# ming71/rotate-yolov3

Hardware: AMD Instinct MI355X
Metric: images/sec fwd+bwd at 608^2 (train step, backend=hip) (higher is better)
Workload: dtype bf16; 1 GPU; configs[3]: Darknet-53 train step (fwd + riou loss + bwd + grad all-reduce + SGD), bs=64/GPU 608x608, synthetic HRSC-shaped targets; global_batch=64, parallelism=dp1, gradients=250 MB fp32 in 4 flat buckets, fp32 on the wire

## Files before the change

include/ryolo.h:

```cpp
#ifndef RYOLO_H
#define RYOLO_H

#include <stddef.h>
#include <stdint.h>

#ifdef __cplusplus
extern "C" {
#endif

#define RYOLO_OK 0
#define RYOLO_EINVAL -1
#define RYOLO_ELAUNCH -2
#define RYOLO_ETOOBIG -3

#define RYOLO_RNMS_MAX_BOXES 262144

const char *ryolo_strerror(int code);
int ryolo_abi_version(void);
const char *ryolo_build_id(void);
int ryolo_set_tuning(const char *name, const char *value);

size_t ryolo_rnms_workspace_bytes(int n);
int ryolo_rnms(const float *dets, int n, int row_stride, float thr, int64_t *keep_out, int32_t *num_keep,
               void *workspace, size_t workspace_bytes, void *stream);

size_t ryolo_rnms_segmented_workspace_bytes(int m, int num_segments, int max_seg_len);
int ryolo_rnms_segmented(const float *dets, int m, int row_stride, const int32_t *seg_offsets, int num_segments,
                         int max_seg_len, float thr, unsigned char *keep_flags, void *workspace, size_t workspace_bytes,
                         void *stream);

void ryolo_rnms_count_pairs(uint64_t *device_counter);

int ryolo_riou_pairs(const float *b1, int stride1, const float *b2, int stride2, int n, float *out, void *stream);
int ryolo_riou_matrix(const float *b1, int n1, int stride1, const float *b2, int n2, int stride2, float *out,
                      void *stream);

int ryolo_skew_iou_pairs(const float *b1, int stride1, const float *b2, int stride2, int n, float *out, void *stream);
int ryolo_skew_iou_matrix(const float *b1, int n1, int stride1, const float *b2, int n2, int stride2, float *out,
                          void *stream);

size_t ryolo_eval_match_workspace_bytes(int n_det, int n_lab);
int ryolo_eval_match(const float *det, int det_stride, const int32_t *det_off, const float *lab, int lab_stride, const int32_t *lab_off,
                     int n_img, int n_det, int n_lab, float iou_thres, uint8_t *correct, int32_t *matched , void *ws,
                     size_t ws_bytes, void *stream);


#define RYOLO_ACT_LINEAR 0
#define RYOLO_ACT_LEAKY 1
#define RYOLO_ACT_MISH 2

typedef struct ryolo_conv_desc {
    int N, H, W;
    int Cin, Cout;
    int ksize, stride, pad;
    int in_cstride, out_cstride, res_cstride;
    int act;
    float slope;
    int upsample;
    int tile;
} ryolo_conv_desc;

size_t ryolo_conv_packed_weight_bytes(int Cout, int Cin_pad, int ksize);
int ryolo_conv_pack_weights(const float *w_oihw, int Cout, int Cin, int ksize, int Cin_pad, void *packed,
                            void *stream);
int ryolo_conv2d_bn_act(const ryolo_conv_desc *desc , const void *x, const void *w_packed,
                        const float *scale, const float *shift, const void *residual , void *y,
                        void *stream);
int ryolo_conv_pair_supported(const ryolo_conv_desc *first, const ryolo_conv_desc *second, int shortcut_from_input);
int ryolo_conv2d_bn_act_pair(const ryolo_conv_desc *first, const ryolo_conv_desc *second, const void *x, const void *w_first,
                             const float *scale_first, const float *shift_first, const void *w_second, const float *scale_second,
                             const float *shift_second, int shortcut_from_input, void *y, void *stream);
#define RYOLO_CONV_KERNEL_MP256 1
#define RYOLO_CONV_KERNEL_MP192 2
#define RYOLO_CONV_KERNEL_MQ 3
#define RYOLO_CONV_KERNEL_DIRECT8 4
#define RYOLO_CONV_KERNEL_STEM 5
#define RYOLO_CONV_KERNEL_PW 6
#define RYOLO_CONV_KERNEL_STEM0 8
#define RYOLO_CONV_KERNEL_STEM_DGRAD 7
#define RYOLO_CONV_KERNEL_STEM64 11
#define RYOLO_CONV_KERNEL_MQ128 9
#define RYOLO_CONV_KERNEL_MQ64 10
#define RYOLO_CONV_KERNEL_IGEMM 16
int ryolo_conv_kernel_choice(const ryolo_conv_desc *desc, int with_residual, int with_statistics);
#define RYOLO_WGRAD_KERNEL_TAPS 1000
int ryolo_conv_dgrad_kernel_choice(const ryolo_conv_desc *forward_desc, int with_bn_reduce );
int ryolo_conv_wgrad_kernel_choice(const ryolo_conv_desc *forward_desc);
int ryolo_nchw_f32_to_nhwc_bf16(const float *x, int N, int C, int H, int W, int Cpad, void *y, void *stream);
int ryolo_nhwc_bf16_to_nchw_f32(const void *x, int N, int C, int H, int W, int cstride, float *y, void *stream);


int ryolo_yolo_decode_filter(const void *head, int head_cstride, int bs, int ny, int nx, int na, int no,
                             const float *anchors, float stride, float context_factor, int arc, float conf_thres,
                             float min_wh, long long io_rows_per_image, long long io_row_offset, float *cand,
                             long long *cand_row, int *counter, int capacity, void *stream);

int ryolo_yolo_decode(const void *head, int head_cstride, int bs, int ny, int nx, int na, int no,
                      const float *anchors, float stride, float context_factor, int arc, float *io,
                      long long io_rows_per_image, long long io_row_offset, float *p, void *stream);

int ryolo_conv_head_decode_supported(const ryolo_conv_desc *desc, int na, int no);
int ryolo_conv_head_decode(const ryolo_conv_desc *desc, const void *x, const void *w_packed, const float *scale, const float *shift,
                           const float *anchors, int na, int no, float stride, float context_factor, int arc, float *io,
                           long long io_rows_per_image, long long io_row_offset, float *p, void *stream);

int ryolo_add_nhwc(const void *a, int a_cstride, const void *b, int b_cstride, void *y, int y_cstride,
                   long long npix, int C, void *stream);
int ryolo_upsample_nhwc(const void *x, int x_cstride, void *y, int y_cstride, int N, int H, int W, int C, int scale,
                        void *stream);
int ryolo_maxpool_nhwc(const void *x, int x_cstride, void *y, int y_cstride, int N, int H, int W, int C, int ksize,
                       int stride, void *stream);

size_t ryolo_se_workspace_bytes(int N, int H, int W, int C);
int ryolo_se_nhwc(const void *x, int x_cstride, const float *w1 , const float *w2 ,
                  int hidden, void *y, int y_cstride, int N, int H, int W, int C,
                  float *gate_out , void *workspace, size_t workspace_bytes, void *stream);


int ryolo_conv0_recompute_supported(const ryolo_conv_desc *desc);
int ryolo_conv0_bn_act_fwd(const ryolo_conv_desc *desc, const void *x, const void *w_packed, const float *scale, const float *shift,
                           int act, const float *slope, void *y, void *stream);
size_t ryolo_conv0_bn_bwd_workspace_bytes(void);
int ryolo_conv0_bn_bwd(const ryolo_conv_desc *desc, const void *x, const void *w_packed, const void *dy, int dy_cstride,
                       const float *scale, const float *shift, const float *mean, const float *invstd, int act, const float *slope,
                       void *dz, int dz_cstride, float *dgamma, float *dbeta, float *dslope, void *workspace, size_t workspace_bytes,
                       int workspace_is_zero, void *stream);
size_t ryolo_conv0_bn_bwd_wgrad_workspace_bytes(void);
int ryolo_conv0_bn_bwd_wgrad(const ryolo_conv_desc *desc, const void *x, const void *w_packed, const void *dy, int dy_cstride,
                             const float *scale, const float *shift, const float *mean, const float *invstd, int act, const float *slope,
                             float *dgamma, float *dbeta, float *dslope, float *grad_oihw, int cin_real, int accumulate, void *workspace,
                             size_t workspace_bytes, void *stream);
int ryolo_conv_stat_rows(const ryolo_conv_desc *desc);
int ryolo_conv2d_bn_act_stats(const ryolo_conv_desc *desc, const void *x, const void *w_packed, const float *scale,
                              const float *shift, const void *residual, void *y,
                              double *stat_part ,
                              void *stream);
int ryolo_bn_finalize(double *stat_part, int rows, int cpad, int C, long long count, float eps, float momentum,
                      const float *gamma, const float *beta, float *mean, float *invstd, float *scale, float *shift,
                      float *running_mean , float *running_var, void *stream);
int ryolo_bn_act_fwd(const void *z, int z_cstride, const float *scale, const float *shift, int act,
                     const float *slope , const void *residual, int res_cstride, void *y,
                     int y_cstride, long long npix, int C, void *stream);
size_t ryolo_bn_act_bwd_workspace_bytes(long long npix, int C);
int ryolo_bn_act_bwd(const void *z, int z_cstride, const void *dy, int dy_cstride, const float *scale, const float *shift,
                     const float *mean, const float *invstd, int act, const float *slope, void *dz, int dz_cstride,
                     long long npix, int C, float *dgamma, float *dbeta, float *dslope, void *workspace,
                     size_t workspace_bytes, void *stream);
size_t ryolo_conv_packed_dgrad_bytes(int Cout, int Cin, int ksize, int stride);
int ryolo_conv_dgrad_tap_table(int ksize, int stride, int *host_out );
int ryolo_conv_pack_weights_dgrad(const float *w_oihw, int Cout, int Cin, int ksize, int stride, void *packed,
                                  const int *taps_table ,
                                  void *stream);
int ryolo_conv2d_dgrad(const ryolo_conv_desc *forward_desc, const void *dz, int dz_cstride, const void *packed_dgrad,
                       const float *ones, const float *zeros , void *dx, int accumulate, void *stream);
int ryolo_conv2d_dgrad_bnreduce_rows(const ryolo_conv_desc *forward_desc);
int ryolo_conv2d_dgrad_bnreduce(const ryolo_conv_desc *forward_desc, const void *dz, int dz_cstride, const void *packed_dgrad,
                                const float *ones, const float *zeros, void *dx, int accumulate,
                                const void *z , int z_cstride,
                                const float *scale, const float *shift, const float *mean, const float *invstd ,
                                const float *slope , float *part , void *stream);
int ryolo_bn_act_bwd_reduced(const void *z, int z_cstride, const void *dy, int dy_cstride, const float *scale, const float *shift,
                             const float *mean, const float *invstd, int act , const float *slope, void *dz,
                             int dz_cstride, long long npix, int C, float *dgamma, float *dbeta, float *dslope, const float *part,
                             int rows, void *workspace , size_t workspace_bytes, void *stream);
size_t ryolo_conv_wgrad_workspace_bytes(const ryolo_conv_desc *forward_desc);
int ryolo_conv2d_wgrad_partials(const ryolo_conv_desc *forward_desc, const void *x, const void *dz, int dz_cstride, int Cin_real,
                                float *grad_oihw, int accumulate, void *workspace, size_t workspace_bytes, void *stream);
int ryolo_conv2d_wgrad_reduce(const ryolo_conv_desc *forward_desc, const void *x, const void *dz, int dz_cstride, int Cin_real,
                              float *grad_oihw, int accumulate, void *workspace, size_t workspace_bytes, void *stream);

typedef struct ryolo_wgrad_reduce_job {
    const float *part;
    float *g;
    int S, Cout, Cin_real, Cin_k, ks, Kpad, Cout_pad, accumulate;
    int kind;
    int block_begin, block_end;
    int wide;
} ryolo_wgrad_reduce_job;
int ryolo_conv_wgrad_reduce_job_fill(ryolo_wgrad_reduce_job *host_job, const ryolo_conv_desc *forward_desc, int Cin_real, const void *workspace,
                                     float *grad_oihw, int accumulate);
int ryolo_conv_wgrad_reduce_batch(const ryolo_wgrad_reduce_job *device_jobs, int njobs, int total_blocks, void *stream);
int ryolo_conv2d_wgrad(const ryolo_conv_desc *forward_desc, const void *x, const void *dz, int dz_cstride, int Cin_real,
                       float *grad_oihw , int accumulate, void *workspace,
                       size_t workspace_bytes, void *stream);
int ryolo_upsample2x_bwd(const void *dy, int dy_cstride, void *dx, int dx_cstride, int N, int H, int W, int C,
                         int accumulate, void *stream);
int ryolo_pgrad_to_nhwc(const float *pgrad, int bs, int na, int ny, int nx, int no, void *out, int out_cstride,
                        void *stream);

typedef struct ryolo_pack_job {
    const void *src;
    void *dst;
    int kind, Cout, Cin, KS, Cin_pad, ntaps, Kpad, rows;
    int khs[9], kws[9];
    int block_begin, block_end;
} ryolo_pack_job;
int ryolo_conv_pack_job_fill(ryolo_pack_job *host_jobs, const float *w_oihw, int Cout, int Cin, int ksize, int stride,
                             int Cin_pad, void *packed_fwd, void *packed_dgrad);
int ryolo_conv_pack_batch(const ryolo_pack_job *device_jobs, int njobs, int total_blocks, void *stream);

#define RYOLO_MAX_HEADS 4
int ryolo_build_targets(const float *tpad, const unsigned char *valid, int NT, int nheads, int na, const float *const *ng,
                        const float *const *anchor_vec, float iou_t, float ang_t, float context_factor, float *const *w,
                        long long *const *idx, float *const *box, float *const *npos, void *stream);
size_t ryolo_yolo_loss_bitmap_bytes(long long cells);
int ryolo_yolo_loss(const float *p, int bs, int na, int ny, int nx, int no, int nc, const float *w, int NT,
                    const long long *b, const long long *gj, const long long *gi, const long long *cls, const float *txy,
                    const float *twh, const float *ta, const float *anchor_vec , const float *npos, float giou,
                    float reg_w, float cls_w, float cls_pw, float obj_w, float obj_pw,
                    int iou_mode ,
                    unsigned *bitmap, float *dp, float *items , void *stream);

int ryolo_yolo_loss_nhwc(const void *head, int head_cstride, const float *p, int bs, int na, int ny, int nx, int no, int nc,
                         const float *w, int NT, const long long *b, const long long *gj, const long long *gi,
                         const long long *cls, const float *txy, const float *twh, const float *ta, const float *anchor_vec,
                         const float *npos, float giou, float reg_w, float cls_w, float cls_pw, float obj_w, float obj_pw,
                         int iou_mode, unsigned *bitmap, float *dp_sparse, void *head_grad, int head_grad_cstride, float *items,
                         void *stream);
#define RYOLO_ARC_FOCAL 1
#define RYOLO_ARC_UBCE 2
#define RYOLO_ARC_UCE 4
size_t ryolo_yolo_loss_bitmap_bytes_arc(long long cells, int nc, int arc);
int ryolo_yolo_loss_arc(const float *p, int bs, int na, int ny, int nx, int no, int nc, const float *w, int NT,
                        const long long *b, const long long *gj, const long long *gi, const long long *cls, const float *txy,
                        const float *twh, const float *ta, const float *anchor_vec, const float *npos, float giou, float reg_w,
                        float cls_w, float cls_pw, float obj_w, float obj_pw, int iou_mode, int arc, float fl_gamma, unsigned *bitmap,
                        float *dp, float *items, void *stream);
int ryolo_yolo_loss_nhwc_arc(const void *head, int head_cstride, const float *p, int bs, int na, int ny, int nx, int no, int nc,
                             const float *w, int NT, const long long *b, const long long *gj, const long long *gi,
                             const long long *cls, const float *txy, const float *twh, const float *ta, const float *anchor_vec,
                             const float *npos, float giou, float reg_w, float cls_w, float cls_pw, float obj_w, float obj_pw,
                             int iou_mode, int arc, float fl_gamma, unsigned *bitmap, float *dp_sparse, void *head_grad,
                             int head_grad_cstride, float *items, void *stream);
int ryolo_scale_bf16_if(const float *g, void *buf, int cstride, long long npix, int C, void *stream);

int ryolo_riou_loss_pairs(const float *pbox, const float *tbox, int n, float *iou, float *grad, void *stream);

// ... 15 lines not shown
```

rotate-yolov3_amd/_lib.py:

```python
import ctypes as C
import os

_HERE = os.path.dirname(os.path.abspath(__file__))
LIB_PATH = os.environ.get("RYOLO_HIP_LIB") or os.path.join(_HERE, "libryolo_hip.so")

_lib = None

ACT_LINEAR, ACT_LEAKY, ACT_MISH = 0, 1, 2


class ConvDesc(C.Structure):
    _fields_ = [("N", C.c_int), ("H", C.c_int), ("W", C.c_int), ("Cin", C.c_int), ("Cout", C.c_int),
                ("ksize", C.c_int), ("stride", C.c_int), ("pad", C.c_int),
                ("in_cstride", C.c_int), ("out_cstride", C.c_int), ("res_cstride", C.c_int),
                ("act", C.c_int), ("slope", C.c_float), ("upsample", C.c_int), ("tile", C.c_int)]


_vp = C.c_void_p
_dp = C.POINTER(ConvDesc)
_sigs = {
    "ryolo_strerror": (C.c_char_p, [C.c_int]),
    "ryolo_abi_version": (C.c_int, []),
    "ryolo_build_id": (C.c_char_p, []),
    "ryolo_set_tuning": (C.c_int, [C.c_char_p, C.c_char_p]),
    "ryolo_rnms_workspace_bytes": (C.c_size_t, [C.c_int]),
    "ryolo_rnms": (C.c_int, [_vp, C.c_int, C.c_int, C.c_float, _vp, _vp, _vp, C.c_size_t, _vp]),
    "ryolo_rnms_segmented_workspace_bytes": (C.c_size_t, [C.c_int, C.c_int, C.c_int]),
    "ryolo_rnms_segmented": (C.c_int, [_vp, C.c_int, C.c_int, _vp, C.c_int, C.c_int, C.c_float, _vp, _vp, C.c_size_t, _vp]),
    "ryolo_riou_pairs": (C.c_int, [_vp, C.c_int, _vp, C.c_int, C.c_int, _vp, _vp]),
    "ryolo_riou_matrix": (C.c_int, [_vp, C.c_int, C.c_int, _vp, C.c_int, C.c_int, _vp, _vp]),
    "ryolo_rnms_count_pairs": (None, [_vp]),
    "ryolo_skew_iou_pairs": (C.c_int, [_vp, C.c_int, _vp, C.c_int, C.c_int, _vp, _vp]),
    "ryolo_skew_iou_matrix": (C.c_int, [_vp, C.c_int, C.c_int, _vp, C.c_int, C.c_int, _vp, _vp]),
    "ryolo_eval_match_workspace_bytes": (C.c_size_t, [C.c_int, C.c_int]),
    "ryolo_eval_match": (C.c_int, [_vp, C.c_int, _vp, _vp, C.c_int, _vp, C.c_int, C.c_int, C.c_int, C.c_float, _vp, _vp, _vp, C.c_size_t, _vp]),
    "ryolo_conv_pair_supported": (C.c_int, [_dp, _dp, C.c_int]),
    "ryolo_conv_head_decode_supported": (C.c_int, [_dp, C.c_int, C.c_int]),
    "ryolo_conv0_recompute_supported": (C.c_int, [_dp]),
    "ryolo_conv2d_dgrad_bnreduce_rows": (C.c_int, [_dp]),
    "ryolo_se_workspace_bytes": (C.c_size_t, [C.c_int, C.c_int, C.c_int, C.c_int]),
    "ryolo_se_nhwc": (C.c_int, [_vp, C.c_int, _vp, _vp, C.c_int, _vp, C.c_int, C.c_int, C.c_int, C.c_int, C.c_int, _vp, _vp, C.c_size_t, _vp]),
}


def declare(name, restype, argtypes):
    _sigs[name] = (restype, argtypes)
    if _lib is not None:
        fn = getattr(getattr(_lib, "_real", _lib), name)
        fn.restype, fn.argtypes = restype, argtypes


def lib():
    global _lib
    if _lib is None:
        if not os.path.exists(LIB_PATH):
            raise RuntimeError(
                "rotate-yolov3_amd: %s is missing -- run `python -c 'import __graft_entry__ as g; g.build()'` "
                "(hipcc --offload-arch=gfx950).  There is no CPU fallback for the HIP hot path." % LIB_PATH)
        import torch
        _lib = C.CDLL(LIB_PATH)
        for name, (restype, argtypes) in _sigs.items():
            fn = getattr(_lib, name)
            fn.restype, fn.argtypes = restype, argtypes
    return _lib


TUNING_SWITCHES = ("RYOLO_CONV3X3", "RYOLO_CONV1X1", "RYOLO_RNMS_TILES", "RYOLO_MQ_KORDER", "RYOLO_BN_REDUCE_TILES", "RYOLO_STEM_DGRAD")


def set_tuning(name, value):
    rc = getattr(lib(), "_real", lib()).ryolo_set_tuning(name.encode(), None if value is None else str(value).encode())
    if rc != 0:
        raise RuntimeError("ryolo_set_tuning(%s): unknown switch" % name)


class _CallTracer(object):

    def __init__(self, real, log):
        self._real, self._log = real, log

    def __getattr__(self, name):
        fn = getattr(self._real, name)
        if not name.startswith("ryolo_") or not callable(fn):
            return fn
        log = self._log

        def traced(*args):
            import torch
            e0, e1 = torch.cuda.Event(enable_timing=True), torch.cuda.Event(enable_timing=True)
            e0.record()
            rc = fn(*args)
            e1.record()
            log.append((name, args, e0, e1))
            return rc
        return traced


class trace_calls(object):

    def __enter__(self):
        global _lib
        lib()
        self._saved = _lib
        self.log = []
        _lib = _CallTracer(self._saved, self.log)
        return self.log

    def __exit__(self, *exc):
        global _lib
        _lib = self._saved
        return False


def check(rc, what):
    if rc != 0:
        msg = lib().ryolo_strerror(rc)
        raise RuntimeError("%s failed: %s (code %d)" % (what, msg.decode() if msg else "?", rc))


def stream_ptr(device=None):
# ... 3 lines not shown
```

rotate-yolov3_amd/csrc/conv.hip:

```cpp
#include <cstring>

#include <mutex>

#include "conv_common.h"

using namespace ryolo_detail;

namespace {

template <int KS, int BM, int BN, int WGM, int WGN, int NSTAGE, bool FAST, bool GEN, bool BNRED = false>
__global__ void __launch_bounds__(WGM *WGN * 64) conv_igemm_kernel(const ConvParams p, const BnRed br = BnRed()) {
    constexpr int NW = WGM * WGN, NT = NW * 64;
    constexpr int WPIX = BM / WGM, WCH = BN / WGN, PF = WPIX / 16, CF = WCH / 16;
    constexpr int A_BYTES = BM * BK * 2, B_BYTES = BN * BK * 2, STAGE = A_BYTES + B_BYTES;
    constexpr int A_PPW = (BM / 8) / NW, B_PPW = (BN / 8) / NW;
    static_assert(A_PPW >= 1 && B_PPW >= 1, "tile too small for the wave count");
    constexpr int SROW = BN * 2 + 16;
    static_assert(BM * SROW + WGM * 2 * BN * 4 <= NSTAGE * STAGE, "staging tile + statistics slots must fit in the operand buffers");
    constexpr int LOADS_PER_STAGE = A_PPW + B_PPW;

    extern __shared__ __attribute__((aligned(16))) char smem[];

    const int tid = threadIdx.x;
    const int lane = tid & 63;
// ... 1475 lines not shown
        unsigned nblk;
        if (!conv0_params(d, d->out_cstride, p, gpw, &nblk)) return RYOLO_EINVAL;
        p.cin_log2 = 3;
        p.stat_cpad = 128;
        const bool staged = conv0_halo_on() && !(d->tile >> 16) && y && !stat_part;
        RYOLO_CONV_DRY_RUN(lc, (staged ? RYOLO_CONV_KERNEL_STEM0 : RYOLO_CONV_KERNEL_DIRECT8));
        if (staged) return launch_conv0_halo(p, nullptr, 0, lc);
        return stat_part ? launch_c8_direct<true>(p, gpw, nblk, lc.stream) : launch_c8_direct<false>(p, gpw, nblk, lc.stream);
    }
    if (!conv_shape(d, p)) return RYOLO_EINVAL;
    p.cin_log2 = ilog2_exact(d->Cin);
    if (d->ksize == 3 && p.cin_log2 < 0 && (d->Cin % BK)) return RYOLO_EINVAL;
    p.taps2 = (d->Cin == 32 && d->ksize == 3) ? 1 : 0;
    p.fast = (d->Cin % BK == 0 || p.taps2) && !(d->tile & 0x100) && buffer_extent((unsigned long long)d->N * d->H * d->W, d->in_cstride, d->Cin, &p.x_bytes) &&
             buffer_extent((d->Cout + 127) / 128 * 128, p.Kpad, p.Kpad + 128, &p.w_bytes);
    if (!p.fast) p.taps2 = p.x_bytes = p.w_bytes = 0;
    p.no_persist = (d->tile & 0x200) ? 1 : 0;
    p.force_persist = (d->tile & 0x800) ? 1 : 0;
    p.pw_grid_cap = (d->tile & 0xff) == 13 ? (d->tile >> 16) & 0xff : 0;
#ifdef RYOLO_MP_ABLATION
    if ((d->tile & 0x400) && p.fast) p.x_bytes = p.w_bytes = 0;
#endif
    p.nt_out = (long long)p.M * d->upsample * d->upsample * d->Cout * 2 >= nt_out_min_bytes() ? 1 : 0;
    p.stat_cpad = (d->Cout + 127) / 128 * 128;
    return dispatch(p, d->ksize, pick_tile(d), lc);
}

static bool head_params(const ryolo_conv_desc *d, ConvParams &p) {
    if (conv_validate(d) != RYOLO_OK || d->ksize != 1 || d->stride != 1 || d->pad != 0 || d->upsample != 1 || (d->Cin % BK)) return false;
    if (!conv_shape(d, p)) return false;
    p.out_cs = d->Cout; p.res_cs = 0; p.Kpad = d->Cin;
    if (!buffer_extent(p.M, d->in_cstride, d->Cin, &p.x_bytes) || !buffer_extent((d->Cout + 127) / 128 * 128, p.Kpad, p.Kpad + 128, &p.w_bytes)) return false;
    p.fast = 1; p.use_magic = 1;
    return true;
}

extern "C" {

int ryolo_conv_stat_rows(const ryolo_conv_desc *d) {
    if (conv_validate(d) != RYOLO_OK) return 0;
    return STAT_ROWS;
}

int ryolo_conv2d_bn_act_stats(const ryolo_conv_desc *d, const void *x, const void *w_packed, const float *scale,
                              const float *shift, const void *residual, void *y, double *stat_part, void *stream_) {
    if (!x || !w_packed || !scale || !shift) return RYOLO_EINVAL;
    if (!y && !(stat_part && ryolo_conv0_recompute_supported(d))) return RYOLO_EINVAL;
    if (((uintptr_t)x | (uintptr_t)y | (uintptr_t)w_packed | (uintptr_t)residual | (uintptr_t)scale | (uintptr_t)shift) & 15)
        return RYOLO_EINVAL;
    ConvLaunch lc;
    lc.stream = (hipStream_t)stream_;
    return conv_forward(d, x, w_packed, scale, shift, residual, y, stat_part, lc);
}

int ryolo_conv2d_bn_act(const ryolo_conv_desc *d, const void *x, const void *w_packed, const float *scale,
                        const float *shift, const void *residual, void *y, void *stream_) {
    return ryolo_conv2d_bn_act_stats(d, x, w_packed, scale, shift, residual, y, nullptr, stream_);
}

int ryolo_conv_kernel_choice(const ryolo_conv_desc *d, int with_residual, int with_statistics) {
    int choice = -1;
    ConvLaunch lc;
    lc.choice = &choice;
    void *fake = (void *)(uintptr_t)4096;
    const int rc = conv_forward(d, fake, fake, (const float *)fake, (const float *)fake, with_residual ? fake : nullptr, fake,
                                with_statistics ? (double *)fake : nullptr, lc);
    return rc == RYOLO_OK ? choice : -1;
}

int ryolo_conv_head_decode_supported(const ryolo_conv_desc *d, int na, int no) {
    ConvParams p{};
    return head_params(d, p) && conv_pw_decode_supported(p, na, no) ? 1 : 0;
}

int ryolo_conv_head_decode(const ryolo_conv_desc *d, const void *x, const void *w_packed, const float *scale, const float *shift,
                           const float *anchors, int na, int no, float stride, float context_factor, int arc, float *io,
                           long long io_rows_per_image, long long io_row_offset, float *pout, void *stream_) {
    ConvParams p{};
    if (!x || !w_packed || !scale || !shift || !anchors || !io || !head_params(d, p) || !conv_pw_decode_supported(p, na, no)) return RYOLO_EINVAL;
    if (arc < 0 || arc > 2 || !(stride > 0.f) || !(context_factor > 0.f)) return RYOLO_EINVAL;
    if (((uintptr_t)x | (uintptr_t)w_packed) & 15) return RYOLO_EINVAL;
    p.x = (const __bf16 *)x; p.w = (const __bf16 *)w_packed; p.scale = scale; p.shift = shift;
    return launch_conv_pw_decode(p, io, io_rows_per_image, io_row_offset, pout, anchors, na, no, stride, context_factor, arc, (hipStream_t)stream_);
}

int ryolo_conv_pair_supported(const ryolo_conv_desc *first, const ryolo_conv_desc *second, int shortcut_from_input) {
    if (conv_validate(first) != RYOLO_OK || conv_validate(second) != RYOLO_OK) return 0;
    return conv_stem_pair_kind(first, second, shortcut_from_input) != 0 ? 1 : 0;
}

int ryolo_conv2d_bn_act_pair(const ryolo_conv_desc *a, const ryolo_conv_desc *b, const void *x, const void *w_first, const float *scale_first,
                             const float *shift_first, const void *w_second, const float *scale_second, const float *shift_second,
                             int shortcut_from_input, void *y, void *stream_) {
    if (conv_validate(a) != RYOLO_OK || conv_validate(b) != RYOLO_OK || !x || !w_first || !scale_first || !shift_first || !w_second || !scale_second ||
        !shift_second || !y)
        return RYOLO_EINVAL;
    const int kind = conv_stem_pair_kind(a, b, shortcut_from_input);
    if (!kind) return RYOLO_EINVAL;
    if (((uintptr_t)x | (uintptr_t)y | (uintptr_t)w_first | (uintptr_t)w_second) & 15) return RYOLO_EINVAL;
    ConvParams p{};
    if (!conv_shape(b, p)) return RYOLO_EINVAL;
    p.w = (const __bf16 *)w_second; p.scale = scale_second; p.shift = shift_second; p.y = (__bf16 *)y;
    p.in_cs = b->Cin; p.res_cs = 0;
    p.nt_out = (long long)p.M * b->Cout * 2 >= nt_out_min_bytes() ? 1 : 0;
    const unsigned long long xb = (((unsigned long long)a->N * a->H * a->W - 1) * a->in_cstride + a->Cin) * 2ull;
    const int kpad_first = (a->ksize * a->ksize * a->Cin + BK - 1) / BK * BK;
    return launch_conv_stem_pair(kind, p, x, (unsigned)xb, a->in_cstride, a->H, a->W, w_first, kpad_first, scale_first, shift_first, a->act,
                                 a->slope, (hipStream_t)stream_);
}

int ryolo_conv0_recompute_supported(const ryolo_conv_desc *d) {
    return conv_validate(d) == RYOLO_OK && conv0_shape(d, d->out_cstride) ? 1 : 0;
}

int ryolo_conv0_bn_act_fwd(const ryolo_conv_desc *d, const void *x, const void *w_packed, const float *scale, const float *shift,
                           int act, const float *slope, void *y, void *stream_) {
    if (!ryolo_conv0_recompute_supported(d) || !x || !w_packed || !scale || !shift || !y) return RYOLO_EINVAL;
    if (act < 0 || act > 2 || (act == RYOLO_ACT_LEAKY && !slope)) return RYOLO_EINVAL;
    if (((uintptr_t)x | (uintptr_t)y | (uintptr_t)w_packed) & 15) return RYOLO_EINVAL;
    ConvParams p{};
    const int gpw = 32;
    unsigned nblk;
    if (!conv0_params(d, d->out_cstride, p, gpw, &nblk)) return RYOLO_EINVAL;
    p.x = (const __bf16 *)x; p.w = (const __bf16 *)w_packed; p.scale = scale; p.shift = shift; p.y = (__bf16 *)y;
    p.act = act; p.slope = 0.f;
    C8Bwd bw;
    bw.slope = act == RYOLO_ACT_LEAKY ? slope : nullptr;
    bw.round_z = 1;
    ConvLaunch lc;
    lc.stream = (hipStream_t)stream_;
    if (conv0_halo_on()) return launch_conv0_halo(p, bw.slope, 1, lc);
    return launch_c8_mode(act, p, gpw, nblk, bw, 0, lc.stream);
}

size_t ryolo_conv0_bn_bwd_workspace_bytes(void) { return (size_t)STAT_ROWS * 96 * 8 + 64 * 4; }

int ryolo_conv0_bn_bwd(const ryolo_conv_desc *d, const void *x, const void *w_packed, const void *dy, int dy_cstride,
                       const float *scale, const float *shift, const float *mean, const float *invstd, int act, const float *slope,
                       void *dz, int dz_cstride, float *dgamma, float *dbeta, float *dslope, void *workspace, size_t workspace_bytes,
                       int workspace_is_zero, void *stream_) {
    if (!ryolo_conv0_recompute_supported(d) || !x || !w_packed || !dy || !scale || !shift || !mean || !invstd || !dz || !workspace)
        return RYOLO_EINVAL;
    if (workspace_bytes < ryolo_conv0_bn_bwd_workspace_bytes() || (dy_cstride & 7) || (dz_cstride & 7) || dy_cstride < 32 || dz_cstride < 32)
        return RYOLO_EINVAL;
    if (act < 0 || act > 2 || (act == RYOLO_ACT_LEAKY && !slope)) return RYOLO_EINVAL;
    if (((uintptr_t)x | (uintptr_t)dy | (uintptr_t)dz | (uintptr_t)w_packed | (uintptr_t)workspace) & 15) return RYOLO_EINVAL;
    hipStream_t stream = (hipStream_t)stream_;
    ConvParams p{};
    const int gpw = 32;
    unsigned nblk;
    C8Bwd bw;
    if (!conv0_params(d, dz_cstride, p, gpw, &nblk) || !buffer_extent(p.M, dy_cstride, 32, &bw.dy_bytes)) return RYOLO_EINVAL;
    p.x = (const __bf16 *)x; p.w = (const __bf16 *)w_packed; p.scale = scale; p.shift = shift; p.y = (__bf16 *)dz;
    p.act = act; p.slope = 0.f;
    bw.slope = act == RYOLO_ACT_LEAKY ? slope : nullptr;
    bw.dy = (const __bf16 *)dy; bw.dy_cs = dy_cstride; bw.mean = mean;
    double *part = (double *)workspace;
    float *kb = (float *)(part + (size_t)STAT_ROWS * 96), *kd = kb + 32;
    bw.part = part; bw.kb = kb; bw.kd = kd;
    if (!workspace_is_zero && hipMemsetAsync(part, 0, (size_t)STAT_ROWS * 96 * 8, stream) != hipSuccess) return RYOLO_ELAUNCH;
    int rc = launch_c8_mode(act, p, gpw, nblk, bw, 2, stream);
    if (rc != RYOLO_OK) return rc;
    rc = launch_kernel<conv0_bwd_finalize_kernel>(dim3(1), dim3(32), 0, stream, part, scale, mean, invstd, 1.0f / (float)p.M, kb, kd, dgamma, dbeta,
                                                  act == RYOLO_ACT_LEAKY ? dslope : nullptr);
    if (rc != RYOLO_OK) return rc;
    return launch_c8_mode(act, p, gpw, nblk, bw, 3, stream);
// ... 4 lines not shown
```

rotate-yolov3_amd/csrc/conv_common.h:

```cpp
#pragma once
#include <hip/hip_runtime.h>
#include <stdint.h>
#include <stdlib.h>

#include "../../include/ryolo.h"

namespace ryolo_detail {

typedef __attribute__((ext_vector_type(8))) __bf16 bf16x8;
typedef __attribute__((ext_vector_type(4))) __bf16 bf16x4;
typedef __attribute__((ext_vector_type(2))) __bf16 bf16x2;
typedef __attribute__((ext_vector_type(4))) float f32x4;
typedef __attribute__((ext_vector_type(4))) unsigned int u32x4;
typedef __attribute__((address_space(3))) void *lds_vp;
typedef const __attribute__((address_space(1))) void *glb_vp;

constexpr int BK = 64;
constexpr long long NT_OUT_MIN_BYTES = 128ll << 20;
constexpr int STAT_ROWS = 128;

struct ConvParams {
    const __bf16 *x;
    const __bf16 *w;
    const float *scale;
// ... 135 lines not shown
        }                             \
    } while (0)

inline int cu_count() {
    static const int cus = [] {
        int dev = 0, n = 0;
        return hipGetDevice(&dev) == hipSuccess && hipDeviceGetAttribute(&n, hipDeviceAttributeMultiprocessorCount, dev) == hipSuccess && n > 0 ? n : 256;
    }();
    return cus;
}

template <auto KFN, typename... Args>
int launch_kernel(dim3 grid, dim3 block, size_t smem, hipStream_t stream, Args... args) {
    if (smem > 64 * 1024) {
        static const hipError_t raised = hipFuncSetAttribute((const void *)KFN, hipFuncAttributeMaxDynamicSharedMemorySize, (int)smem);
        if (raised != hipSuccess) return RYOLO_ELAUNCH;
    }
    hipLaunchKernelGGL(KFN, grid, block, smem, stream, args...);
    return hipGetLastError() == hipSuccess ? RYOLO_OK : RYOLO_ELAUNCH;
}

inline bool buffer_extent(unsigned long long npix, long long cs, long long c, unsigned *bytes = nullptr) {
    const unsigned long long b = ((npix - 1) * (unsigned long long)cs + (unsigned long long)c) * 2ull;
    if (b >= 0x7fffff00ull) return false;
    if (bytes) *bytes = (unsigned)b;
    return true;
}

struct PersistGrid {
    int grid, nt;
    long long tiles;
    bool deep, exact;
};
inline PersistGrid persist_grid(long long M, int BM, int Cout, int BN, int Ho, int Wo, bool force = false, int rounds2 = 5) {
    const long long mt = (M + BM - 1) / BM, nt = (Cout + BN - 1) / BN, dmax = Wo > Ho ? Wo : Ho;
    PersistGrid g;
    g.grid = (2 * cu_count()) & ~7;
    g.nt = (int)nt;
    g.tiles = mt * nt;
    g.deep = force ? g.tiles > g.grid : 2 * g.tiles >= (long long)rounds2 * g.grid;
    g.exact = g.grid >= 8 && mt * BM * dmax < 0x100000000ll && g.tiles * nt < 0x100000000ll;
    return g;
}

inline int grid_for(long long total, int tb = 256, int cap = 32768) {
    long long nb = (total + tb - 1) / tb;
    return (int)(nb < 1 ? 1 : (nb > cap ? cap : nb));
}

inline int ilog2_exact(int v) {
    int l = 0;
    while ((1 << l) < v) l++;
    return (1 << l) == v ? l : -1;
}

int conv_validate(const ryolo_conv_desc *d);
int dispatch(ConvParams &p, int ksize, int pick, const ConvLaunch &lc);
long long nt_out_min_bytes();
bool conv_pw_disabled();
int mq128_knob();

int launch_conv_mp(ConvParams &p, int bm , int variant, const ConvLaunch &lc);
int conv_mp_pick_bm(const ConvParams &p);
bool conv_mp_eligible(const ConvParams &p);
int launch_conv_mq(ConvParams &p, int variant, const ConvLaunch &lc);
bool conv_mq128_eligible(const ConvParams &p);
int conv_mq128_grid(const ConvParams &p, int bm);
int launch_conv_mq128(ConvParams &p, int bm, const ConvLaunch &lc);
bool conv_stem_eligible(const ConvParams &p, int ksize);
int launch_conv_stem(ConvParams &p, const ConvLaunch &lc);
bool conv_stem64_eligible(const ConvParams &p, int ksize);
int launch_conv_stem64(ConvParams &p, const ConvLaunch &lc);
int launch_conv0_halo(ConvParams &p, const float *slope_dev, int round_z, const ConvLaunch &lc);
int launch_conv_stem_dgrad(int cdz, int stride, const void *dz, int dz_cs, const void *w_classes, void *dx, int dx_cs, int accumulate, int N,
                           int H, int W, int nt_out, const ConvLaunch &lc);
int conv_stem_pair_kind(const ryolo_conv_desc *first, const ryolo_conv_desc *second, int shortcut_from_input);
int launch_conv_stem_pair(int kind, ConvParams &p , const void *x, unsigned x_bytes, int in_cs, int H, int W,
                          const void *w_first, int kpad_first, const float *scale_first, const float *shift_first, int act_first,
                          float slope_first, hipStream_t stream);
bool conv_pw_eligible(const ConvParams &p, int ksize);
bool conv_pw_preferred(const ConvParams &p);
int conv_pw_grid(const ConvParams &p);
int launch_conv_pw(ConvParams &p, const ConvLaunch &lc);
bool conv_pw_decode_supported(const ConvParams &p, int na, int no);
int launch_conv_pw_decode(ConvParams &p, float *io, long long io_img_rows, long long io_row0, float *pout, const float *anchors, int na, int no,
                          float stride, float cf, int arc, hipStream_t stream);
#ifdef RYOLO_MP_ABLATION
int ryolo_mp_ablation_variant(int slot);
#endif

enum TuneKey { TUNE_CONV3X3 = 0, TUNE_CONV1X1, TUNE_RNMS_TILES, TUNE_MQ_KORDER, TUNE_BN_REDUCE_TILES, TUNE_STEM_DGRAD, TUNE_COUNT };
const char *tune(TuneKey k);
#ifdef RYOLO_MP_ABLATION
inline const char *abl_env(const char *name) { return getenv(name); }
#else
inline const char *abl_env(const char *) { return nullptr; }
#endif

}
```

rotate-yolov3_amd/csrc/conv_dgrad.hip:

```cpp
#include <cstring>

#include "conv_common.h"

using namespace ryolo_detail;

extern "C" {

static int dgrad_classes(int ks, int stride, int pad, int cls, int *dy, int *dx, int *khs, int *kws) {
    if (stride == 1) {
        int n = 0;
        for (int kh = 0; kh < ks; kh++)
            for (int kw = 0; kw < ks; kw++) {
                dy[n] = kh; dx[n] = kw; khs[n] = ks - 1 - kh; kws[n] = ks - 1 - kw;
                n++;
            }
        return n;
    }
    const int a = cls >> 1, b = cls & 1;
    int n = 0;
    for (int kh = ks - 1; kh >= 0; kh--) {
        if (((a + pad - kh) & 1) != 0) continue;
        for (int kw = ks - 1; kw >= 0; kw--) {
            if (((b + pad - kw) & 1) != 0) continue;
            dy[n] = (a + pad - kh) / 2; dx[n] = (b + pad - kw) / 2; khs[n] = kh; kws[n] = kw;
// ... 246 lines not shown
        for (int cls = 0; cls < (stride == 1 ? 1 : 4); cls++) {
            int dy[9], dx[9], khs[9], kws[9];
            const int nt = dgrad_classes(ksize, stride, (ksize - 1) / 2, cls, dy, dx, khs, kws);
            ryolo_pack_job &j = host_jobs[n++];
            j = ryolo_pack_job{};
            j.src = w_oihw; j.dst = dst; j.kind = 1; j.Cout = Cout; j.Cin = Cin; j.KS = ksize; j.ntaps = nt;
            for (int t = 0; t < nt; t++) { j.khs[t] = khs[t]; j.kws[t] = kws[t]; }
            j.Kpad = (nt * Cout + BK - 1) / BK * BK;
            j.rows = (Cin + 127) / 128 * 128;
            j.block_begin = 0; j.block_end = (j.rows / PK_CI) * ((Cout + PK_CO - 1) / PK_CO);
            dst += ((size_t)j.rows * j.Kpad + 128) * 2;
        }
        if (dgrad_xfusable(Cin, ksize, stride)) {
            for (int a = 0; a < 2; a++) {
                int dy[9], dx[9], khs[9], k0[9], k1[9];
                const int nt = dgrad_xfused_class(a, dy, dx, khs, k0, k1);
                ryolo_pack_job &j = host_jobs[n++];
                j = ryolo_pack_job{};
                j.src = w_oihw; j.dst = dst; j.kind = 2; j.Cout = Cout; j.Cin = Cin; j.KS = ksize; j.ntaps = nt;
                for (int t = 0; t < nt; t++) { j.khs[t] = khs[t]; j.kws[t] = (k0[t] + 1) | ((k1[t] + 1) << 4); }
                j.Kpad = (nt * Cout + BK - 1) / BK * BK;
                j.rows = (2 * Cin + 127) / 128 * 128;
                j.block_begin = 0; j.block_end = (j.rows / PK_CI) * ((Cout + PK_CO - 1) / PK_CO);
                dst += ((size_t)j.rows * j.Kpad + 128) * 2;
            }
        }
    }
    return n;
}

int ryolo_conv_pack_batch(const ryolo_pack_job *device_jobs, int njobs, int total_blocks, void *stream) {
    if (!device_jobs || njobs <= 0 || total_blocks <= 0) return RYOLO_EINVAL;
    hipLaunchKernelGGL(pack_batch_kernel, dim3((unsigned)total_blocks), dim3(256), 0, (hipStream_t)stream, device_jobs, njobs);
    return hipGetLastError() == hipSuccess ? RYOLO_OK : RYOLO_ELAUNCH;
}

int ryolo_conv_dgrad_tap_table(int ksize, int stride, int *host_out ) {
    if (!host_out || (ksize != 1 && ksize != 3) || (stride != 1 && stride != 2)) return RYOLO_EINVAL;
    for (int i = 0; i < 72; i++) host_out[i] = 0;
    for (int cls = 0; cls < (stride == 1 ? 1 : 4); cls++) {
        int dy[9], dx[9];
        dgrad_classes(ksize, stride, (ksize - 1) / 2, cls, dy, dx, host_out + cls * 18, host_out + cls * 18 + 9);
    }
    return RYOLO_OK;
}

int ryolo_conv_pack_weights_dgrad(const float *w_oihw, int Cout, int Cin, int ksize, int stride, void *packed,
                                  const int *taps_table , void *stream_) {
    if (!w_oihw || !packed || !taps_table || ryolo_conv_packed_dgrad_bytes(Cout, Cin, ksize, stride) == 0) return RYOLO_EINVAL;
    hipStream_t stream = (hipStream_t)stream_;
    const int rows = (Cin + 127) / 128 * 128;
    char *dst = (char *)packed;
    for (int cls = 0; cls < (stride == 1 ? 1 : 4); cls++) {
        int dy[9], dx[9], kk[18];
        const int nt = dgrad_classes(ksize, stride, (ksize - 1) / 2, cls, dy, dx, kk, kk + 9);
        const int Kpad = (nt * Cout + BK - 1) / BK * BK;
        const size_t total = (size_t)rows * Kpad + 128;
        const int nb = (int)((total + 255) / 256 < 4096 ? (total + 255) / 256 : 4096);
        hipLaunchKernelGGL(pack_dgrad_kernel, dim3(nb), dim3(256), 0, stream, w_oihw, Cout, Cin, ksize, nt,
                           taps_table + cls * 18, Kpad, rows, (__bf16 *)dst);
        dst += total * 2;
    }
    if (dgrad_xfusable(Cin, ksize, stride)) {
        const int rows2 = (2 * Cin + 127) / 128 * 128;
        for (int a = 0; a < 2; a++) {
            int dy[9], dx[9];
            XfTaps tp;
            const int nt = dgrad_xfused_class(a, dy, dx, tp.khs, tp.kw0, tp.kw1);
            for (int t = nt; t < 9; t++) { tp.khs[t] = 0; tp.kw0[t] = -1; tp.kw1[t] = -1; }
            const int Kpad = (nt * Cout + BK - 1) / BK * BK;
            const size_t total = (size_t)rows2 * Kpad + 128;
            const int nb = (int)((total + 255) / 256 < 4096 ? (total + 255) / 256 : 4096);
            hipLaunchKernelGGL(pack_dgrad_xfused_kernel, dim3(nb), dim3(256), 0, stream, w_oihw, Cout, Cin, nt, tp, Kpad, rows2,
                               (__bf16 *)dst);
            dst += total * 2;
        }
    }
    return hipGetLastError() == hipSuccess ? RYOLO_OK : RYOLO_ELAUNCH;
}

}

static int conv_dgrad(const ryolo_conv_desc *d , const void *dz, int dz_cstride, const void *packed_dgrad, const float *ones,
                      const float *zeros, void *dx, int accumulate, const ConvLaunch &lc) {
    if (conv_validate(d) != RYOLO_OK) return RYOLO_EINVAL;
    if (d->stride != 1 && !(d->stride == 2 && d->ksize == 3 && d->pad == 1)) return RYOLO_EINVAL;
    if ((dz_cstride & 7) || dz_cstride < d->Cout) return RYOLO_EINVAL;
    const int Ho = (d->H + 2 * d->pad - d->ksize) / d->stride + 1, Wo = (d->W + 2 * d->pad - d->ksize) / d->stride + 1;
    const int rows = (d->Cin + 127) / 128 * 128;
    const unsigned long long dz_pix = (unsigned long long)d->N * Ho * Wo;
    const int nt_out = (long long)d->N * d->H * d->W * d->Cin * 2 >= nt_out_min_bytes() ? 1 : 0;
    const char *wsrc = (const char *)packed_dgrad;
    const bool xfuse = dgrad_xfusable(d->Cin, d->ksize, d->stride) && d->pad == 1 && (d->W & 1) == 0 &&
                       d->in_cstride == d->Cin && !(d->tile & 0x8000);
    if (xfuse) wsrc += dgrad_classic_bytes(d->Cout, d->Cin, d->ksize, d->stride);
    if (!lc.bnred && d->ksize == 3 && d->pad == 1 && ((d->Cin == 32 && d->Cout == 64) || (d->Cin == 64 && d->Cout == 128 && d->stride == 2)) &&
        !(d->tile & 0x80ff)) {
        const char *e = tune(TUNE_STEM_DGRAD);
        const int knob = e ? atoi(e) : 3;
        if (knob & (d->Cout == 64 ? 1 : 2)) {
            if (buffer_extent(dz_pix, dz_cstride, d->Cout) && buffer_extent((unsigned long long)d->N * d->H * d->W, d->in_cstride, d->Cin)) {
                RYOLO_CONV_DRY_RUN(lc, RYOLO_CONV_KERNEL_STEM_DGRAD);
                const int rc = launch_conv_stem_dgrad(d->Cout, d->stride, dz, dz_cstride, packed_dgrad, dx, d->in_cstride, accumulate, d->N, d->H,
                                                      d->W, nt_out, lc);
                if (rc != RYOLO_EINVAL) return rc;
            }
        }
    }
    const int ncls = d->stride == 1 ? 1 : (xfuse ? 2 : 4);
    const int wrows = xfuse ? (2 * d->Cin + 127) / 128 * 128 : rows;
    for (int cls = 0; cls < ncls; cls++) {
        int dy[9], dxx[9], khs[9], kws[9];
        const int nt = xfuse ? dgrad_xfused_class(cls, dy, dxx, khs, kws, kws)
                             : dgrad_classes(d->ksize, d->stride, d->pad, cls, dy, dxx, khs, kws);
        ConvParams p{};
        p.x = (const __bf16 *)dz;
        p.w = (const __bf16 *)wsrc;
        p.scale = ones; p.shift = zeros;
        p.res = accumulate ? (const __bf16 *)dx : nullptr;
        p.y = (__bf16 *)dx;
        p.N = d->N; p.H = Ho; p.W = Wo; p.Cin = d->Cout; p.in_cs = dz_cstride;
        p.Cout = d->Cin; p.out_cs = d->in_cstride; p.res_cs = d->in_cstride;
        p.K = nt * d->Cout;
        p.Kpad = (p.K + BK - 1) / BK * BK;
        p.act = RYOLO_ACT_LINEAR; p.ups = 1;
        p.cin_log2 = ilog2_exact(d->Cout);
        p.ntaps = nt;
        for (int t = 0; t < nt; t++) { p.tap_dy[t] = dy[t]; p.tap_dx[t] = dxx[t]; }
        p.stride = 1; p.OH = d->H;
        if (d->stride == 1) {
            p.pad = d->ksize - 1 - d->pad;
            p.Ho = d->H; p.Wo = d->W;
            p.os = 1; p.osx = 1; p.OW = d->W;
        } else if (xfuse) {
            p.Cout = 2 * d->Cin; p.out_cs = 2 * d->in_cstride; p.res_cs = 2 * d->in_cstride;
            p.Ho = (d->H - cls + 1) / 2; p.Wo = d->W / 2;
            p.os = 2; p.osx = 1; p.ooy = cls; p.OW = d->W / 2;
        } else {
            const int a = cls >> 1, b = cls & 1;
            p.Ho = (d->H - a + 1) / 2; p.Wo = (d->W - b + 1) / 2;
            p.os = 2; p.osx = 2; p.ooy = a; p.oox = b; p.OW = d->W;
        }
        const size_t wbytes = ((size_t)wrows * p.Kpad + 128) * 2;
        wsrc += wbytes;
        if (p.Ho <= 0 || p.Wo <= 0) continue;
        p.M = (int)((long long)d->N * p.Ho * p.Wo);
        p.fast = (d->Cout % BK == 0) && buffer_extent(dz_pix, dz_cstride, d->Cout, &p.x_bytes) && buffer_extent(wrows, p.Kpad, p.Kpad + 128, &p.w_bytes);
        if (!p.fast) p.x_bytes = p.w_bytes = 0;
        if (!p.fast && (d->stride != 1 || (d->ksize == 3 && p.cin_log2 < 0))) return RYOLO_EINVAL;
        p.no_persist = (d->tile & 0x200) ? 1 : 0;
        p.pw_grid_cap = (d->tile & 0xff) == 13 ? (d->tile >> 16) & 0xff : 0;
        p.nt_out = nt_out;
        const int pick = (d->tile & 0xff);
        const int rc = dispatch(p, d->ksize, pick, lc);
        if (rc != RYOLO_OK) return rc;
    }
    return RYOLO_OK;
}

static int dgrad_choice(const ryolo_conv_desc *d, const BnRed *bnred = nullptr, int mode = 0) {
    int choice = -1;
    ConvLaunch lc;
    lc.bnred = bnred; lc.bnred_mode = mode; lc.choice = &choice;
    void *fake = (void *)(uintptr_t)4096;
    return conv_dgrad(d, fake, d ? d->Cout : 0, fake, (const float *)fake, (const float *)fake, fake, 1, lc) == RYOLO_OK ? choice : -1;
}

static int bnreduce_plan_tiles(const ryolo_conv_desc *d) {
    if (d->stride != 1 || (d->tile & 0xff) || d->in_cstride != d->Cin || (d->Cin & 7)) return 0;
    int knob = 1;
    {
        const char *e = tune(TUNE_BN_REDUCE_TILES);
        if (e) knob = atoi(e);
        if (knob == 0) return 0;
    }
    const BnRed br{};
    const int natural = dgrad_choice(d), fused = natural < 0 ? -1 : dgrad_choice(d, &br, 3);
    if (fused < 0 || natural != fused) return 0;
    const int tile = fused - RYOLO_CONV_KERNEL_IGEMM;
    const int bm = tile == 1 ? 128 : ((tile == 2 || tile == 3) ? 256 : 0);
    if (!bm) return 0;
    if (tile == 3) return 0;
    if (tile == 1 && knob == 2) return 0;
    const long long M = (long long)d->N * d->H * d->W;
    return (int)((M + bm - 1) / bm);
}

static int bnreduce_plan_mq128(const ryolo_conv_desc *d) {
    if (d->stride != 1 || (d->tile & 0xff) || d->in_cstride != d->Cin || (d->Cin & 127) || mq128_knob() <= 0) return 0;
    const int natural = dgrad_choice(d);
    if (natural != RYOLO_CONV_KERNEL_MQ128 && natural != RYOLO_CONV_KERNEL_MQ64) return 0;
    ConvParams q{};
    q.M = (int)((long long)d->N * d->H * d->W);
    q.Cout = d->Cin;
    return conv_mq128_grid(q, natural == RYOLO_CONV_KERNEL_MQ128 ? 128 : 64);
}

static int bnreduce_plan(const ryolo_conv_desc *d, int *mode) {
    *mode = 0;
    if (conv_validate(d) != RYOLO_OK) return 0;
    {
        const int r = bnreduce_plan_mq128(d);
        if (r > 0) {
            *mode = 4;
            return r;
        }
    }
    auto tiles = [&]() {
        const int r = bnreduce_plan_tiles(d);
        if (r > 0) *mode = 3;
        return r;
    };
    if (d->ksize != 1 || d->stride != 1 || d->pad != 0) return tiles();
    if ((d->Cin & 127) || (d->Cout & 63) || (d->tile & 0xff)) return tiles();
    const long long M = (long long)d->N * d->H * d->W;
    int g_pw = 0;
    {
        ConvParams q{};
        q.Cin = d->Cout; q.Kpad = (d->Cout + BK - 1) / BK * BK; q.Cout = d->Cin;
        const int g = conv_pw_disabled() ? 0 : conv_pw_grid(q);
        if (g > 0 && d->in_cstride == d->Cin && buffer_extent(M + 1024 * 128, d->Cout, d->Cout) && buffer_extent(M, d->Cin, d->Cin)) g_pw = g;
    }
    const PersistGrid pg = persist_grid(M, 128, d->Cin, 128, d->H, d->W);
    const bool persist_ok = pg.deep && pg.exact && buffer_extent(M, d->Cout, d->Cout);
    if (g_pw > 0 && (d->Cout == 128 || !persist_ok)) {
        *mode = 1;
        return g_pw;
    }
    if (persist_ok) {
        *mode = 2;
        return pg.grid;
    }
    return tiles();
}

extern "C" {

int ryolo_conv2d_dgrad_bnreduce_rows(const ryolo_conv_desc *d) {
    int mode;
    return bnreduce_plan(d, &mode);
}

int ryolo_conv2d_dgrad(const ryolo_conv_desc *d , const void *dz, int dz_cstride,
                       const void *packed_dgrad, const float *ones, const float *zeros, void *dx, int accumulate,
                       void *stream_) {
    if (!dz || !packed_dgrad || !ones || !zeros || !dx) return RYOLO_EINVAL;
    ConvLaunch lc;
    lc.stream = (hipStream_t)stream_;
    return conv_dgrad(d, dz, dz_cstride, packed_dgrad, ones, zeros, dx, accumulate, lc);
}

int ryolo_conv2d_dgrad_bnreduce(const ryolo_conv_desc *d, const void *dz, int dz_cstride, const void *packed_dgrad, const float *ones,
                                const float *zeros, void *dx, int accumulate, const void *z, int z_cstride, const float *scale,
                                const float *shift, const float *mean, const float *invstd, const float *slope, float *part,
                                void *stream_) {
    ConvLaunch lc;
    if (!bnreduce_plan(d, &lc.bnred_mode) || !z || (z_cstride & 7) || z_cstride < d->Cin || !scale || !shift || !mean || !invstd ||
        !slope || !part || d->in_cstride != d->Cin || !dz || !packed_dgrad || !ones || !zeros || !dx)
        return RYOLO_EINVAL;
    BnRed br;
    br.z = (const __bf16 *)z; br.z_cs = z_cstride; br.scale = scale; br.shift = shift; br.mean = mean; br.invstd = invstd;
    br.slope = slope; br.part = part;
    lc.bnred = &br;
    lc.stream = (hipStream_t)stream_;
    return conv_dgrad(d, dz, dz_cstride, packed_dgrad, ones, zeros, dx, accumulate, lc);
}

int ryolo_conv_dgrad_kernel_choice(const ryolo_conv_desc *d, int with_bn_reduce) {
    if (!with_bn_reduce) return dgrad_choice(d);
    const BnRed br{};
    int mode = 0;
    return bnreduce_plan(d, &mode) ? dgrad_choice(d, &br, mode) : -1;
}

}
```

rotate-yolov3_amd/csrc/conv_pw.hip:

```cpp
#include <type_traits>
#include <utility>

#include "conv_common.h"
#include "yolo_decode.h"

using namespace ryolo_detail;

namespace {

template <int N> using ic = std::integral_constant<int, N>;

template <class F, int... I>
__device__ __forceinline__ void static_for_impl(F &&f, std::integer_sequence<int, I...>) {
    (f(ic<I>{}), ...);
}
template <int N, class F>
__device__ __forceinline__ void static_for(F &&f) {
    static_for_impl(f, std::make_integer_sequence<int, N>{});
}

__device__ __forceinline__ void issue_order_fence() { asm volatile("" ::: "memory"); }

template <int N>
__device__ __forceinline__ void wait_vmcnt() {
    asm volatile("s_waitcnt vmcnt(%0)" ::"n"(N > 63 ? 63 : (N < 0 ? 0 : N)) : "memory");
}

constexpr int pw_first_block_younger(int kt, int KT, int RING, int LPU, int WL, int NREQ, int D) {
    int after = 0;
    bool seen = false;
    for (int u = 0; u < RING - 1; u++) {
        if (seen) after += LPU;
        if (u == kt) seen = true;
    }
    for (int j = 0; j < D && j < KT; j++)
        if (seen) after += WL;
    for (int t = 0; t < kt; t++) {
        if (t == 0 && seen) after += NREQ;
        if (seen) after += LPU;
        if (t + RING - 1 == kt) seen = true;
        if (t + D < KT && seen) after += WL;
    }
    return after;
}

struct PwBnRed {
    const __bf16 *z;
    int z_cs;
    unsigned z_bytes;
    const float *scale, *shift, *mean, *invstd, *slope;
    float *part;
};

#ifdef RYOLO_MP_ABLATION
#define PW_DBG(bit) ((p.dbg0 >> (bit)) & 1)
#else
#define PW_DBG(bit) 0
#endif

struct PwDecode {
    float *io, *p;
    const float *anchors;
    long long io_img_rows, io_row0;
    int na, no, ny, nx;
    float stride, cf;
    int arc;
    int apb;
};

template <int KT, int NW, int CF, int PF, int RING, int MODE>
__global__ void __launch_bounds__(NW * 64, 2) conv_pw_kernel(const ConvParams p, const PwBnRed br, const PwDecode dc) {
    constexpr int BMS = PF * 16;
    constexpr int UNIT = BMS * 128;
    constexpr int LPU = (BMS / 8) / NW;
    constexpr int NCB = NW * CF * 16;
    constexpr bool HAS_RES = MODE == 2 || MODE == 3, BNRED = MODE == 3, STATS = MODE == 1, DEC = MODE == 4;
    constexpr int TROW = NCB * 2 + 16;
    constexpr int NSTG = DEC ? 0 : (CF == 2 ? PF : PF / 2);
    constexpr int NREQ = (HAS_RES ? NSTG : 0) + (BNRED ? NSTG : 0);
    static_assert(LPU >= 1 && (BMS / 8) % NW == 0, "a unit must split into whole pieces per wave");
    static_assert(CF == 1 || CF == 2, "one or two channel fragments per wave");
    static_assert(PF % 2 == 0, "row fragments are paired by the CF == 1 epilogue");
    static_assert(RING >= 3, "at least one unit in flight behind the one being read");
    static_assert((RING - 2) * LPU + 2 * (NSTG + NREQ) <= 63, "the counted waits must be encodable");
    extern __shared__ __attribute__((aligned(16))) char smem[];

    if (PW_DBG(6)) return;
    const int tid = threadIdx.x, lane = tid & 63;
    const int wave = __builtin_amdgcn_readfirstlane(tid >> 6);
    const int fr = lane & 15, g = lane >> 4;
#ifdef RYOLO_MP_ABLATION
    unsigned *trace_row = nullptr;
    if (PW_DBG(9) && p.trace && (wave == 0 || wave == NW - 1) && (blockIdx.x == 0 || blockIdx.x == 8 || blockIdx.x == 1001 % gridDim.x))
        trace_row = p.trace + ((blockIdx.x == 0 ? 0 : (blockIdx.x == 8 ? 1 : 2)) * 2 + (wave == 0 ? 0 : 1)) * 64;
    int trace_n = 0;
#define PW_STAMP()                                                                                              \
    do {                                                                                                        \
        if (trace_row && trace_n < 64) {                                                                        \
            if (lane == 0) trace_row[trace_n] = (unsigned)__builtin_readcyclecounter();                         \
            trace_n++;                                                                                          \
        }                                                                                                       \
    } while (0)
#else
#define PW_STAMP() do { } while (0)
#endif
    PW_STAMP();

    const int xcd = blockIdx.x & 7, loc = blockIdx.x >> 3, nloc = gridDim.x >> 3;
    const int NB = p.pw_nb;
    const int nb = loc % NB, ms = loc / NB, nms = nloc / NB;
    const int MB = p.pw_mb, q = MB >> 3, r = MB & 7;
    const int start = xcd < r ? xcd * (q + 1) : r * (q + 1) + (xcd - r) * q;
    const int len = q + (xcd < r ? 1 : 0);
    const int n0 = DEC ? nb * dc.apb * dc.no : nb * NCB;
    if constexpr (BNRED) {
        for (int t = tid; t < 3 * p.Cout; t += NW * 64) br.part[(size_t)blockIdx.x * 3 * p.Cout + t] = 0.f;
        __syncthreads();
    }
    if (ms >= len) return;
    const int cnt = (len - ms + nms - 1) / nms;
    const int rb0 = start + ms;

    int iss_off[LPU];
#pragma unroll
    for (int j = 0; j < LPU; j++) {
        const int row = (wave * LPU + j) * 8 + (lane >> 3);
        const int slot = (lane & 7) ^ ((row >> 1) & 7);
        iss_off[j] = ((rb0 * BMS + row) * p.in_cs) * 2 + slot * 16;
    }
    const int iss_delta = nms * BMS * p.in_cs * 2;
    int iss_i = 0, iss_kt = 0, iss_slot = 0;
    auto fill = [&]() __attribute__((always_inline)) {
        const bool live = iss_i < cnt && !PW_DBG(1);
        char *dst = smem + iss_slot * UNIT + wave * LPU * 1024;
#pragma unroll
        for (int j = 0; j < LPU; j++)
            buffer_load_lds16(p.x, p.x_bytes, dst + j * 1024, live ? iss_off[j] : (int)0x80000000, iss_kt * 128);
        iss_slot = iss_slot + 1 == RING ? 0 : iss_slot + 1;
        if (++iss_kt == KT) {
            iss_kt = 0;
            iss_i++;
            if (iss_i < cnt) {
#pragma unroll
                for (int j = 0; j < LPU; j++) iss_off[j] += iss_delta;
            }
        }
    };

    int a_rd[2];
#pragma unroll
    for (int ks = 0; ks < 2; ks++) a_rd[ks] = fr * 128 + (((ks * 4 + g) ^ ((fr >> 1) & 7)) << 4);

    f32x4 sc[CF], sh[CF];
#pragma unroll
    for (int cf = 0; cf < CF; cf++) {
        const int ch = n0 + wave * CF * 16 + cf * 16 + g * 4;
        if constexpr (DEC) {
            sc[cf] = *(const f32x4_u4 *)(p.scale + ch);
            sh[cf] = *(const f32x4_u4 *)(p.shift + ch);
// ... 61 lines not shown
    constexpr int I0 = (RING - 1 + KT - 1) / KT;

    auto row_block = [&](int i, auto FIRSTc) __attribute__((always_inline)) {
        constexpr bool FIRST = decltype(FIRSTc)::value != 0;
        const int m0 = (rb0 + i * nms) * BMS;
#pragma unroll
        for (int cf = 0; cf < CF; cf++)
#pragma unroll
            for (int f = 0; f < PF; f++) acc[cf][f] = f32x4{0.f, 0.f, 0.f, 0.f};
        const bool steady = !FIRST && i >= I0;
        static_for<KT>([&](auto ktc) __attribute__((always_inline)) {
            constexpr int kt = decltype(ktc)::value;
            constexpr int BASE = (RING - 2) * LPU;
            constexpr int own_rq = (kt >= 1 && kt <= RING - 2) ? NREQ : 0;
            constexpr int ALL_ST = []() { int n = 0; for (int d = 1; d <= RING - 1; d++) if ((((kt - d) % KT) + KT) % KT == KT - 1) n++; return n; }();
            constexpr int ALL_RQ = []() { int n = 0; for (int d = 1; d <= RING - 2; d++) if ((((kt - d) % KT) + KT) % KT == 0) n++; return n; }();
            if constexpr (FIRST) wait_vmcnt<pw_first_block_younger(kt, KT, RING, LPU, WL, NREQ, WD)>();
            else if (steady) wait_vmcnt<BASE + ALL_ST * NSTG + ALL_RQ * NREQ>();
            else wait_vmcnt<BASE + own_rq>();
            PW_STAMP();
            if (!PW_DBG(4)) __builtin_amdgcn_s_barrier();
            PW_STAMP();
            if constexpr (kt == 0 && NREQ > 0) {
#if defined(__HIP_DEVICE_COMPILE__)
#pragma unroll
                for (int s = 0; s < NSTG; s++) {
                    const int m = m0 + (CF == 2 ? s : 2 * s + (g & 1)) * 16 + fr;
                    const bool ok = m < p.M && och_ok;
                    if constexpr (HAS_RES) rv[s] = __builtin_amdgcn_raw_buffer_load_b128(rrs, ok ? (m * p.res_cs + och) * 2 : (int)0x80000000, 0, 0);
                    if constexpr (BNRED) zv[s] = __builtin_amdgcn_raw_buffer_load_b128(zrs, ok ? (m * br.z_cs + och) * 2 : (int)0x80000000, 0, 0);
                }
#endif
            }
            issue_order_fence();
            fill();
            issue_order_fence();
            if constexpr (FIRST && kt + WD < KT) {
                load_w(ic<kt + WD>{});
                issue_order_fence();
            }
            const char *ub = smem + rd_slot * UNIT;
#pragma unroll
            for (int ks = 0; ks < 2; ks++) {
                bf16x8 xf[PF];
#pragma unroll
                for (int f = 0; f < PF; f++) xf[f] = PW_DBG(5) ? wreg[kt][ks][0] : *(const bf16x8 *)(ub + a_rd[ks] + f * 2048);
                if (!PW_DBG(2)) {
#pragma unroll
                    for (int cf = 0; cf < CF; cf++)
#pragma unroll
                        for (int f = 0; f < PF; f++)
                            acc[cf][f] = __builtin_amdgcn_mfma_f32_16x16x32_bf16(wreg[kt][ks][cf], xf[f], acc[cf][f], 0, 0, 0);
                }
            }
            rd_slot = rd_slot + 1 == RING ? 0 : rd_slot + 1;
#ifdef RYOLO_MP_ABLATION
            if (trace_row) asm volatile("s_nop 0" ::"v"(acc[0][0]), "v"(acc[CF - 1][PF - 1]));
#endif
            PW_STAMP();
        });

        auto run_epilogue = [&](auto ACTc) __attribute__((always_inline)) {
            constexpr int ACT = decltype(ACTc)::value;
            if constexpr (DEC) {
                char *tile = smem + RING * UNIT;
#pragma unroll
                for (int cf = 0; cf < CF; cf++)
#pragma unroll
                    for (int f = 0; f < PF; f++) {
                        bf16x4 o;
#pragma unroll
                        for (int rr = 0; rr < 4; rr++) {
                            float v = acc[cf][f][rr] * sc[cf][rr] + sh[cf][rr];
                            if constexpr (ACT == RYOLO_ACT_LEAKY) v = v > 0.f ? v : v * slope;
                            else if constexpr (ACT == RYOLO_ACT_MISH) v = mish(v);
                            o[rr] = (__bf16)v;
                        }
                        *(bf16x4 *)(tile + (f * 16 + fr) * TROW + (wave * CF * 16 + cf * 16 + g * 4) * 2) = o;
                    }
                __syncthreads();
                const int a0 = nb * dc.apb, na_here = min(dc.apb, dc.na - a0);
                const int nrows = BMS * na_here;
                const long long hw = (long long)dc.ny * dc.nx;
                for (int rw = tid; rw < nrows; rw += NW * 64) {
                    const int al = rw / BMS, pxl = rw - al * BMS;
                    const int a = a0 + al;
                    const int m = m0 + pxl;
                    if (m >= p.M) continue;
                    const int t1 = udiv_magic(m, p.magic_wo);
                    const int x = m - t1 * p.Wo;
                    const int n = udiv_magic(t1, p.magic_ho);
                    const int y = t1 - n * p.Ho;
                    const __bf16 *src = (const __bf16 *)(tile + pxl * TROW) + al * dc.no;
                    float v[8];
#pragma unroll
                    for (int k = 0; k < 8; k++)
                        if (k < dc.no) v[k] = (float)src[k];
                    const long long row = (long long)a * hw + (long long)y * dc.nx + x;
                    if (dc.p) store_row(dc.p + (((long long)n * dc.na * hw) + row) * dc.no, v, dc.no);
                    const float aw = dc.anchors[a * 3 + 0] / dc.stride, ah = dc.anchors[a * 3 + 1] / dc.stride, aa = dc.anchors[a * 3 + 2];
                    decode_row<8>(v, dc.no, x, y, aw, ah, aa, dc.stride, dc.cf, dc.arc, dc.io + (((long long)n * dc.io_img_rows) + dc.io_row0 + row) * dc.no);
                }
                return;
            }
            unsigned R[CF][PF][2];
#pragma unroll
            for (int cf = 0; cf < CF; cf++)
#pragma unroll
                for (int f = 0; f < PF; f++) {
                    const bool ok = m0 + f * 16 + fr < p.M;
                    bf16x4 o;
#pragma unroll
                    for (int rr = 0; rr < 4; rr++) {
                        float v = acc[cf][f][rr] * sc[cf][rr] + sh[cf][rr];
                        if constexpr (ACT == RYOLO_ACT_LEAKY) v = v > 0.f ? v : v * slope;
                        else if constexpr (ACT == RYOLO_ACT_MISH) v = mish(v);
                        o[rr] = (__bf16)v;
                        if constexpr (STATS) {
                            const float qv = ok ? (float)o[rr] : 0.f;
                            st_sum[cf][rr] += qv;
                            st_sq[cf][rr] += qv * qv;
                        }
                    }
                    const uint2 u2 = __builtin_bit_cast(uint2, o);
                    R[cf][f][0] = u2.x;
                    R[cf][f][1] = u2.y;
                }
#if defined(__HIP_DEVICE_COMPILE__)
#pragma unroll
            for (int s = 0; s < (DEC ? 0 : NSTG); s++) {
                unsigned a0, a1, b0, b1;
                if constexpr (CF >= 2) { a0 = R[0][s][0]; a1 = R[0][s][1]; b0 = R[1][s][0]; b1 = R[1][s][1]; }
                else { a0 = R[0][2 * s][0]; a1 = R[0][2 * s][1]; b0 = R[0][2 * s + 1][0]; b1 = R[0][2 * s + 1][1]; }
                auto s0 = __builtin_amdgcn_permlane16_swap(a0, b0, false, false);
                auto s1 = __builtin_amdgcn_permlane16_swap(a1, b1, false, false);
                u32x4 out = u32x4{s0[0], s1[0], s0[1], s1[1]};
                const int m = m0 + (CF == 2 ? s : 2 * s + (g & 1)) * 16 + fr;
                const bool ok = m < p.M && och_ok;
                if constexpr (HAS_RES) {
                    bf16x8 a = __builtin_bit_cast(bf16x8, out);
                    const bf16x8 b = __builtin_bit_cast(bf16x8, rv[s]);
#pragma unroll
                    for (int e = 0; e < 8; e++) a[e] = (__bf16)((float)a[e] + (float)b[e]);
                    out = __builtin_bit_cast(u32x4, a);
                }
                if constexpr (BNRED) {
                    const bf16x8 dv = __builtin_bit_cast(bf16x8, out), zq = __builtin_bit_cast(bf16x8, zv[s]);
                    if (ok) {
#pragma unroll
                        for (int e = 0; e < 8; e++) {
                            const float zf = (float)zq[e], d = (float)dv[e];
                            const float u = zf * bn_sc[e] + bn_sh[e];
                            float gg = d;
                            if (u <= 0.f) { gg = d * bn_slope; bs3[e] += d * u; }
                            bs2[e] += gg * (zf - bn_mu[e]);
                            bs1[e] += gg;
                        }
                    }
                }
                if (PW_DBG(3)) {
                    asm volatile("" ::"v"(out));
                } else if (p.ups == 1) {
                    const int voff = ok ? (m * p.out_cs + och) * 2 : (int)0x80000000;
                    if (p.nt_out) __builtin_amdgcn_raw_buffer_store_b128(out, yrs, voff, 0, 2);
                    else __builtin_amdgcn_raw_buffer_store_b128(out, yrs, voff, 0, 0);
                } else {
                    const int mm = m < p.M ? m : 0;
                    const int t = udiv_magic(mm, p.magic_wo);
                    const int wo = mm - t * p.Wo;
                    const int img = udiv_magic(t, p.magic_ho);
                    const int ho = t - img * p.Ho;
                    const int W2 = p.Wo * 2;
                    const int o00 = ok ? ((((img * p.Ho * 2 + ho * 2) * W2 + wo * 2) * p.out_cs) + och) * 2 : (int)0x80000000;
                    buffer_store16_soff<0>(out, yrs, o00, 0);
                    buffer_store16_soff<0>(out, yrs, o00, p.out_cs * 2);
                    buffer_store16_soff<0>(out, yrs, o00, W2 * p.out_cs * 2);
                    buffer_store16_soff<0>(out, yrs, o00, (W2 + 1) * p.out_cs * 2);
                }
            }
#endif
        };
        if (p.act == RYOLO_ACT_LEAKY) run_epilogue(ic<RYOLO_ACT_LEAKY>{});
        else if (p.act == RYOLO_ACT_MISH) run_epilogue(ic<RYOLO_ACT_MISH>{});
        else run_epilogue(ic<RYOLO_ACT_LINEAR>{});
        PW_STAMP();
    };
    PW_STAMP();
    if (PW_DBG(7)) {
        asm volatile("s_waitcnt vmcnt(0)" ::: "memory");
        return;
    }
    row_block(0, ic<1>{});
    if (!PW_DBG(8))
        for (int i = 1; i < cnt; i++) row_block(i, ic<0>{});
    asm volatile("s_waitcnt vmcnt(0)" ::: "memory");
    PW_STAMP();

    if constexpr (STATS) {
        float ta = 0.f, tb = 0.f;
#pragma unroll
        for (int cf = 0; cf < CF; cf++)
#pragma unroll
            for (int rr = 0; rr < 4; rr++) {
                const float a = row16_sum(st_sum[cf][rr]), b = row16_sum(st_sq[cf][rr]);
                if (fr == cf * 4 + rr) {
                    ta = a;
                    tb = b;
                }
            }
        if (fr < CF * 4) {
            const int ch = n0 + wave * CF * 16 + (fr >> 2) * 16 + g * 4 + (fr & 3);
            if (ch < p.Cout) {
                double *row = p.stat_part + (size_t)(blockIdx.x % STAT_ROWS) * 2 * p.stat_cpad;
                atomicAdd(row + ch, (double)ta);
                atomicAdd(row + p.stat_cpad + ch, (double)tb);
            }
        }
    }
    if constexpr (BNRED) {
        float t1 = 0.f, t2 = 0.f, t3 = 0.f;
#pragma unroll
        for (int e = 0; e < 8; e++) {
            float a = row16_sum(bs1[e]), b = row16_sum(bs2[e]), d = row16_sum(bs3[e]);
            if constexpr (CF == 1) {
                a += __shfl_xor(a, 16); b += __shfl_xor(b, 16); d += __shfl_xor(d, 16);
            }
            if (fr == e) { t1 = a; t2 = b; t3 = d; }
        }
        const bool writer = fr < 8 && (CF == 2 || (g & 1) == 0);
        const int ch = och + fr;
        if (writer && ch < p.Cout) {
            float *row = br.part + (size_t)blockIdx.x * 3 * p.Cout;
            row[ch] = t1;
            row[p.Cout + ch] = t2 * br.invstd[ch];
            row[2 * p.Cout + ch] = t3;
        }
    }
}

struct PwCfg { int kt, ncb, nw, cf, pf, ring; };

static thread_local const PwDecode *g_pw_decode = nullptr;

template <int KT, int NW, int CF, int PF, int RING, int MODE>
int pw_launch(ConvParams &p, const PwBnRed &br, int grid, hipStream_t stream) {
    constexpr int LDS = RING * PF * 16 * 128 + (MODE == 4 ? PF * 16 * (NW * CF * 16 * 2 + 16) : 0);
    const PwDecode dc = g_pw_decode ? *g_pw_decode : PwDecode{};
    return launch_kernel<conv_pw_kernel<KT, NW, CF, PF, RING, MODE>>(dim3((unsigned)grid), dim3(NW * 64), LDS, stream, p, br, dc);
}

template <int KT, int NW, int CF, int PF, int RING, int MODES>
int pw_launch_mode(ConvParams &p, const PwBnRed *br, int grid, hipStream_t stream) {
    PwBnRed none{};
    const int mode = g_pw_decode ? 4 : (br ? 3 : (p.stat_part ? 1 : (p.res ? 2 : 0)));
    if constexpr ((MODES & 16) != 0) if (mode == 4) return pw_launch<KT, NW, CF, PF, RING, 4>(p, none, grid, stream);
    if constexpr ((MODES & 8) != 0) if (mode == 3) return pw_launch<KT, NW, CF, PF, RING, 3>(p, *br, grid, stream);
    if constexpr ((MODES & 2) != 0) if (mode == 1) return pw_launch<KT, NW, CF, PF, RING, 1>(p, none, grid, stream);
    if constexpr ((MODES & 4) != 0) if (mode == 2) return pw_launch<KT, NW, CF, PF, RING, 2>(p, none, grid, stream);
    if constexpr ((MODES & 1) != 0) if (mode == 0) return pw_launch<KT, NW, CF, PF, RING, 0>(p, none, grid, stream);
    return RYOLO_EINVAL;
}

inline unsigned pw_magic_u32(int d) { return d <= 1 ? 0u : (unsigned)((0x100000000ull + (unsigned)d - 1) / (unsigned)d); }

bool pw_pick(const ConvParams &p, bool bnred, PwCfg &c, int &NB, int &grid) {
    if (p.Kpad != p.Cin || (p.Cin & 63)) return false;
    const int kt = p.Cin / 64;
    const int cus = cu_count() & ~7;
    if (cus < 8) return false;
    int wgpc;
    if (g_pw_decode) {
        if (bnred) return false;
        if (kt == 4) c = PwCfg{4, 256, 8, 2, 4, 12};
        else if (kt == 8) c = PwCfg{8, 256, 8, 2, 4, 12};
        else if (kt == 16) c = PwCfg{16, 128, 8, 1, 4, 12};
        else return false;
        NB = (g_pw_decode->na + g_pw_decode->apb - 1) / g_pw_decode->apb;
        grid = cus;
        return NB >= 1 && (grid / 8) % NB == 0;
    }
    else if (kt == 4 && p.Cout <= 128 && !bnred) { c = PwCfg{4, 128, 4, 2, 8, 4}; wgpc = 2; }
    else if (kt == 6 && p.Cout <= 128 && !bnred) { c = PwCfg{6, 128, 4, 2, 4, 8}; wgpc = 2; }
    else if (kt == 2 && p.Cout % 256 == 0) { c = PwCfg{2, 256, 8, 2, 4, 12}; wgpc = 1; }
    else if (kt == 4 && bnred) { c = PwCfg{4, 128, 8, 1, 4, 12}; wgpc = 1; }
    else if (kt == 4) { c = PwCfg{4, 256, 8, 2, 4, 12}; wgpc = 1; }
    else if (kt == 8 && bnred) { c = PwCfg{8, 128, 8, 1, 4, 12}; wgpc = 1; }
    else if (kt == 8) { c = PwCfg{8, 256, 8, 2, 4, 12}; wgpc = 1; }
    else if (kt == 12 && !bnred) { c = PwCfg{12, 128, 8, 1, 4, 12}; wgpc = 1; }
    else if (kt == 16 && !bnred) { c = PwCfg{16, 128, 8, 1, 4, 12}; wgpc = 1; }
    else return false;
    NB = (p.Cout + c.ncb - 1) / c.ncb;
    grid = wgpc * cus;
    if (p.pw_grid_cap > 0 && p.pw_grid_cap * 8 < grid) grid = p.pw_grid_cap * 8;
    const int nloc = grid / 8;
    if (NB < 1 || nloc % NB) return false;
    if (NB * c.ncb > ((p.Cout + 127) / 128) * 128) return false;
    return true;
}

}

namespace ryolo_detail {

bool conv_pw_eligible(const ConvParams &p, int ksize) {
    if (ksize != 1 || !p.fast || p.os != 1 || p.stride != 1 || p.taps2) return false;
    if (p.stat_part && (p.res || p.ups != 1)) return false;
    if (p.res && p.ups != 1) return false;
    PwCfg c;
    int NB, grid;
    if (!pw_pick(p, false, c, NB, grid)) return false;
    return !(p.res && c.kt == 4 && c.nw == 4);
}

bool conv_pw_preferred(const ConvParams &p) {
    PwCfg c;
    int NB, grid;
    if (!pw_pick(p, false, c, NB, grid)) return false;
    const long long mb = ((long long)p.M + c.pf * 16 - 1) / (c.pf * 16);
    return c.kt <= 12 && 2 * p.Cout <= 3 * p.Cin && mb * NB >= 2ll * grid;
}

int conv_pw_grid(const ConvParams &p) {
    PwCfg c;
    int NB, grid;
    return pw_pick(p, true, c, NB, grid) ? grid : 0;
}

static int pw_decode_apb(int na, int no, int ncb = 256) {
    const int apb = ncb / no;
    return apb < na ? apb : na;
}

int launch_conv_pw_decode(ConvParams &p, float *io, long long io_img_rows, long long io_row0, float *pout, const float *anchors, int na, int no,
                          float stride, float cf, int arc, hipStream_t stream) {
    if (!io || !anchors || na <= 0 || no < 7 || no > 8 || na * no != p.Cout || p.ups != 1 || p.res || p.stat_part) return RYOLO_EINVAL;
    const long long dmax = p.Wo > p.Ho ? p.Wo : p.Ho;
    if (((long long)p.M + 64) * dmax >= 0x100000000ll) return RYOLO_EINVAL;
    PwDecode dc;
    dc.io = io; dc.p = pout; dc.anchors = anchors; dc.io_img_rows = io_img_rows; dc.io_row0 = io_row0;
    dc.na = na; dc.no = no; dc.ny = p.Ho; dc.nx = p.Wo; dc.stride = stride; dc.cf = cf; dc.arc = arc;
    dc.apb = pw_decode_apb(na, no, p.Cin == 1024 ? 128 : 256);
    g_pw_decode = &dc;
    ConvLaunch lc;
    lc.stream = stream;
    const int rc = launch_conv_pw(p, lc);
    g_pw_decode = nullptr;
    return rc;
}

bool conv_pw_decode_supported(const ConvParams &p, int na, int no) {
    if (no < 7 || no > 8 || na * no != p.Cout || p.Kpad != p.Cin || (p.Cin != 256 && p.Cin != 512 && p.Cin != 1024)) return false;
    const int ncb = p.Cin == 1024 ? 128 : 256;
    const int apb = pw_decode_apb(na, no, ncb);
    const int nb = apb > 0 ? (na + apb - 1) / apb : 0;
    if (!(apb > 0 && (nb == 1 || nb == 2 || nb == 4) && (nb - 1) * apb * no + ncb <= ((p.Cout + 127) / 128) * 128)) return false;
    PwDecode dc{};
    dc.na = na; dc.no = no; dc.apb = apb;
    const PwDecode *saved = g_pw_decode;
    g_pw_decode = &dc;
    PwCfg c;
    int NB, grid;
    const bool ok = pw_pick(p, false, c, NB, grid);
    g_pw_decode = saved;
    return ok;
}

#ifdef RYOLO_MP_ABLATION
static int g_pw_dbg = 0;
static unsigned *g_pw_trace = nullptr;
#endif

int launch_conv_pw(ConvParams &p, const ConvLaunch &lc) {
#ifdef RYOLO_MP_ABLATION
    p.dbg0 = g_pw_dbg;
    p.trace = g_pw_trace;
#endif
    PwCfg c;
    int NB, grid;
    if (!pw_pick(p, lc.bnred != nullptr, c, NB, grid)) return RYOLO_EINVAL;
    const int bms = c.pf * 16;
    const long long mb = ((long long)p.M + bms - 1) / bms;
    const unsigned long long yb = (((unsigned long long)p.M * p.ups * p.ups - 1) * p.out_cs + p.Cout) * 2ull;
    const unsigned long long rb = p.res ? (((unsigned long long)p.M - 1) * p.res_cs + p.Cout) * 2ull : 0ull;
    const unsigned long long xmax = ((unsigned long long)(mb + grid) * bms) * p.in_cs * 2ull + 4096;
    if (yb >= 0x7fffff00ull || rb >= 0x7fffff00ull || xmax >= 0x7fffff00ull || mb > 0x7fffffffll) return RYOLO_EINVAL;
    if (p.ups != 1 && (long long)mb * bms * (p.Wo > p.Ho ? p.Wo : p.Ho) >= 0x100000000ll) return RYOLO_EINVAL;
    p.y_bytes = (unsigned)yb;
    p.res_bytes = (unsigned)rb;
    p.pw_nb = NB;
    p.pw_mb = (int)mb;
    p.magic_wo = pw_magic_u32(p.Wo);
    p.magic_ho = pw_magic_u32(p.Ho);
    PwBnRed br{};
    const PwBnRed *brp = nullptr;
    if (const BnRed *b = lc.bnred) {
        if (p.stat_part || p.ups != 1) return RYOLO_EINVAL;
        br.z = b->z; br.z_cs = b->z_cs; br.scale = b->scale; br.shift = b->shift; br.mean = b->mean; br.invstd = b->invstd;
        br.slope = b->slope; br.part = b->part;
        const unsigned long long zb = (((unsigned long long)p.M - 1) * b->z_cs + p.Cout) * 2ull;
        if (zb >= 0x7fffff00ull) return RYOLO_EINVAL;
        br.z_bytes = (unsigned)zb;
        brp = &br;
    }
    RYOLO_CONV_DRY_RUN(lc, RYOLO_CONV_KERNEL_PW);
#define PW_CASE(KT_, NW_, CF_, PF_, RING_, MODES_)                                               \
    if (c.kt == KT_ && c.nw == NW_ && c.cf == CF_ && c.pf == PF_ && c.ring == RING_)              \
        return pw_launch_mode<KT_, NW_, CF_, PF_, RING_, MODES_>(p, brp, grid, lc.stream);
    PW_CASE(4, 4, 2, 8, 4, 3)
    PW_CASE(6, 4, 2, 4, 8, 7)
    PW_CASE(2, 8, 2, 4, 12, 15)
    PW_CASE(4, 8, 2, 4, 12, 23)
    PW_CASE(4, 8, 1, 4, 12, 8)
    PW_CASE(8, 8, 2, 4, 12, 23)
    PW_CASE(8, 8, 1, 4, 12, 8)
    PW_CASE(12, 8, 1, 4, 12, 7)
    PW_CASE(16, 8, 1, 4, 12, 23)
#undef PW_CASE
    return RYOLO_EINVAL;
}

}

#ifdef RYOLO_MP_ABLATION
extern "C" void ryolo_debug_convpw_set(int flags) { ryolo_detail::g_pw_dbg = flags; }
extern "C" void ryolo_debug_convpw_trace(void *buf ) { ryolo_detail::g_pw_trace = (unsigned *)buf; }
#endif
```

rotate-yolov3_amd/csrc/train.hip:

```cpp
#include "conv_common.h"

using namespace ryolo_detail;

namespace {

__global__ void __launch_bounds__(1024) bn_finalize_kernel(double *__restrict__ part, int R, int cpad, int C, float count, float eps,
                                   float momentum, const float *__restrict__ gamma, const float *__restrict__ beta,
                                   float *__restrict__ mean, float *__restrict__ invstd, float *__restrict__ scale,
                                   float *__restrict__ shift, float *__restrict__ run_mean, float *__restrict__ run_var) {
    __shared__ double red[2][32][33];
    const int cx = threadIdx.x & 31, ry = threadIdx.x >> 5;
    const int c = blockIdx.x * 32 + cx;
    double s = 0.0, q = 0.0;
    if (c < C) {
        for (int r0 = ry; r0 < R; r0 += 32 * 8) {
            double a[8], b[8];
#pragma unroll
            for (int u = 0; u < 8; u++) {
                const int r = r0 + 32 * u;
                a[u] = r < R ? part[(size_t)r * 2 * cpad + c] : 0.0;
                b[u] = r < R ? part[(size_t)r * 2 * cpad + cpad + c] : 0.0;
            }
#pragma unroll
            for (int u = 0; u < 8; u++) {
// ... 20 lines not shown
    invstd[c] = is;
    scale[c] = gamma[c] * is;
    shift[c] = beta[c] - (float)mu * gamma[c] * is;
    if (run_mean) {
        const double unb = count > 1.f ? var * count / (count - 1.0) : var;
        run_mean[c] = (1.f - momentum) * run_mean[c] + momentum * (float)mu;
        run_var[c] = (1.f - momentum) * run_var[c] + momentum * (float)unb;
    }
}

__device__ __forceinline__ float mish_f(float x) {
    const float e = __expf(fminf(x, 20.f));
    const float n = (1.f + e) * (1.f + e);
    return x * (n - 1.f) / (n + 1.f);
}
__device__ __forceinline__ float mish_grad(float x) {
    const float e = __expf(fminf(x, 20.f));
    const float n = (1.f + e) * (1.f + e);
    const float t = (n - 1.f) / (n + 1.f);
    return t + x * (1.f - t * t) * (e / (1.f + e));
}

constexpr long long NT_MIN_BYTES = 128ll << 20;
#ifdef RYOLO_MP_ABLATION
static int g_nt[3] = {-1, -1, -1};
inline bool nt_pass(int kind, long long npix, int C) { return g_nt[kind] < 0 ? npix * C * 2 >= NT_MIN_BYTES : g_nt[kind] != 0; }
#else
inline bool nt_pass(int, long long npix, int C) { return npix * C * 2 >= NT_MIN_BYTES; }
#endif
template <bool NTL>
__device__ __forceinline__ bf16x8 ld8(const __bf16 *p) {
    if constexpr (NTL) return __builtin_nontemporal_load((const bf16x8 *)p);
    else return *(const bf16x8 *)p;
}
template <bool NTL>
__device__ __forceinline__ void st8(__bf16 *p, const bf16x8 &v) {
    if constexpr (NTL) __builtin_nontemporal_store(v, (bf16x8 *)p);
    else *(bf16x8 *)p = v;
}

template <int ACT, bool NTL = false>
__global__ void bn_act_fwd_kernel(const __bf16 *__restrict__ z, int z_cs, const float *__restrict__ scale,
                                  const float *__restrict__ shift, const float *__restrict__ slope_p,
                                  const __bf16 *__restrict__ res, int res_cs, __bf16 *__restrict__ y, int y_cs,
                                  long long npix, int C) {
    const int cpr = C / 8;
    const long long total = npix * cpr;
    const float slope = slope_p ? slope_p[0] : 0.f;
    for (long long i = (long long)blockIdx.x * blockDim.x + threadIdx.x; i < total;
         i += (long long)gridDim.x * blockDim.x) {
        const long long pix = i / cpr;
        const int c = (int)(i % cpr) * 8;
        const bf16x8 v = ld8<NTL>(z + pix * z_cs + c);
        bf16x8 o;
#pragma unroll
        for (int e = 0; e < 8; e++) {
            float u = (float)v[e] * scale[c + e] + shift[c + e];
            if (ACT == 1) u = u > 0.f ? u : u * slope;
            else if (ACT == 2) u = mish_f(u);
            o[e] = (__bf16)u;
        }
        if (res) {
            const bf16x8 r = ld8<NTL>(res + pix * res_cs + c);
#pragma unroll
            for (int e = 0; e < 8; e++) o[e] = (__bf16)((float)o[e] + (float)r[e]);
        }
        st8<NTL>(y + pix * y_cs + c, o);
    }
}

constexpr int BWD_SLAB_MIN = 128;
#ifdef RYOLO_MP_ABLATION
static int g_bwd_slabs = 1024, g_bwd_slab_min = BWD_SLAB_MIN;
inline long long bwd_slab(long long npix) {
    long long s = (npix + g_bwd_slabs - 1) / g_bwd_slabs;
    return s < g_bwd_slab_min ? g_bwd_slab_min : s;
}
#else
inline long long bwd_slab(long long npix) {
    const long long s = (npix + 1023) / 1024;
    return s < BWD_SLAB_MIN ? BWD_SLAB_MIN : s;
}
#endif
template <int ACT, bool NTL = false>
__global__ void __launch_bounds__(256)
bn_act_bwd_reduce_kernel(const __bf16 *__restrict__ z, int z_cs, const __bf16 *__restrict__ dy, int dy_cs,
                         const float *__restrict__ scale, const float *__restrict__ shift,
                         const float *__restrict__ mean, const float *__restrict__ invstd,
                         const float *__restrict__ slope_p, long long npix, int C, int CT, float *__restrict__ part, long long SL) {
    __shared__ float red[256][25];
    const int cl = threadIdx.x % CT, pl = threadIdx.x / CT, npl = 256 / CT;
    const int c = (blockIdx.x * CT + cl) * 8;
    const int slab = blockIdx.y;
    const long long p0 = (long long)slab * SL;
    const long long p1 = p0 + SL < npix ? p0 + SL : npix;
    const float slope = slope_p ? slope_p[0] : 0.f;
    float s1[8], s2[8], s3[8];
#pragma unroll
    for (int e = 0; e < 8; e++) s1[e] = s2[e] = s3[e] = 0.f;
    if (c < C) {
        float sc[8], sh[8], mu[8], is[8];
#pragma unroll
        for (int e = 0; e < 8; e++) {
            sc[e] = scale ? scale[c + e] : 1.f; sh[e] = scale ? shift[c + e] : 0.f;
            mu[e] = scale ? mean[c + e] : 0.f; is[e] = scale ? invstd[c + e] : 0.f;
        }
        auto accum = [&](const bf16x8 &zv, const bf16x8 &gv) {
#pragma unroll
            for (int e = 0; e < 8; e++) {
                const float zf = (float)zv[e], d = (float)gv[e];
                float g = d;
                if (scale) {
                    const float u = zf * sc[e] + sh[e];
                    if (ACT == 1 && u <= 0.f) { g = d * slope; s3[e] += d * u; }
                    else if (ACT == 2) g = d * mish_grad(u);
                    s2[e] += g * (zf - mu[e]);
                }
                s1[e] += g;
            }
        };
        long long pix = p0 + pl;
        for (; pix + 3 * npl < p1; pix += 4 * npl) {
            bf16x8 zv[4], gv[4];
#pragma unroll
            for (int k = 0; k < 4; k++) {
                zv[k] = ld8<NTL>(z + (pix + k * npl) * z_cs + c);
                gv[k] = ld8<NTL>(dy + (pix + k * npl) * dy_cs + c);
            }
#pragma unroll
            for (int k = 0; k < 4; k++) accum(zv[k], gv[k]);
        }
        for (; pix < p1; pix += npl) accum(*(const bf16x8 *)(z + pix * z_cs + c), *(const bf16x8 *)(dy + pix * dy_cs + c));
#pragma unroll
        for (int e = 0; e < 8; e++) s2[e] *= is[e];
    }
#pragma unroll
    for (int e = 0; e < 8; e++) { red[threadIdx.x][e] = s1[e]; red[threadIdx.x][8 + e] = s2[e]; red[threadIdx.x][16 + e] = s3[e]; }
    __syncthreads();
    for (int t = threadIdx.x; t < CT * 24; t += 256) {
        const int l = t / 24, k = t % 24;
        float v = 0.f;
        for (int q = 0; q < npl; q++) v += red[q * CT + l][k];
        const int ch = (blockIdx.x * CT + l) * 8 + (k & 7);
        if (ch < C) part[((size_t)slab * 3 + (k >> 3)) * C + ch] = v;
    }
}

__global__ void __launch_bounds__(1024)
bn_act_bwd_finalize_kernel(const float *__restrict__ part, int nslab, int C, float *__restrict__ s1o,
                           float *__restrict__ s2o, float *__restrict__ dgamma, float *__restrict__ dbeta,
                           float *__restrict__ s3o) {
    __shared__ float red[3][32][33];
    const int cx = threadIdx.x & 31, ry = threadIdx.x >> 5;
    const int c = blockIdx.x * 32 + cx;
    float a = 0.f, b = 0.f, d = 0.f;
    if (c < C) {
        for (int s0 = ry; s0 < nslab; s0 += 32 * 8) {
            float va[8], vb[8], vd[8];
#pragma unroll
            for (int u = 0; u < 8; u++) {
                const int s = s0 + 32 * u;
                va[u] = s < nslab ? part[((size_t)s * 3 + 0) * C + c] : 0.f;
                vb[u] = s < nslab ? part[((size_t)s * 3 + 1) * C + c] : 0.f;
                vd[u] = s < nslab ? part[((size_t)s * 3 + 2) * C + c] : 0.f;
            }
#pragma unroll
            for (int u = 0; u < 8; u++) { a += va[u]; b += vb[u]; d += vd[u]; }
        }
    }
    red[0][ry][cx] = a; red[1][ry][cx] = b; red[2][ry][cx] = d;
    __syncthreads();
    if (ry != 0) return;
    for (int k = 1; k < 32; k++) { a += red[0][k][cx]; b += red[1][k][cx]; d += red[2][k][cx]; }
    if (c < C) {
        s1o[c] = a;
        s2o[c] = b;
        if (dgamma) dgamma[c] += b;
        if (dbeta) dbeta[c] += a;
        if (s3o) s3o[c] = d;
    }
}

constexpr int BWD_FOLD = 64, BWD_FOLD_MIN_ROWS = 2048;
__global__ void __launch_bounds__(1024)
bn_act_bwd_fold_kernel(const float *__restrict__ part, int nrows, int C, int per, float *__restrict__ out) {
    __shared__ float red[3][32][33];
    const int cx = threadIdx.x & 31, ry = threadIdx.x >> 5;
    const int c = blockIdx.x * 32 + cx, g = blockIdx.y;
    const int r0 = g * per, r1 = min(nrows, r0 + per);
    float a = 0.f, b = 0.f, d = 0.f;
    if (c < C) {
        for (int s0 = r0 + ry; s0 < r1; s0 += 32 * 4) {
            float va[4], vb[4], vd[4];
#pragma unroll
            for (int u = 0; u < 4; u++) {
                const int s = s0 + 32 * u;
                va[u] = s < r1 ? part[((size_t)s * 3 + 0) * C + c] : 0.f;
                vb[u] = s < r1 ? part[((size_t)s * 3 + 1) * C + c] : 0.f;
                vd[u] = s < r1 ? part[((size_t)s * 3 + 2) * C + c] : 0.f;
            }
#pragma unroll
            for (int u = 0; u < 4; u++) { a += va[u]; b += vb[u]; d += vd[u]; }
        }
    }
    red[0][ry][cx] = a; red[1][ry][cx] = b; red[2][ry][cx] = d;
    __syncthreads();
    if (ry != 0 || c >= C) return;
    for (int k = 1; k < 32; k++) { a += red[0][k][cx]; b += red[1][k][cx]; d += red[2][k][cx]; }
    out[((size_t)g * 3 + 0) * C + c] = a;
    out[((size_t)g * 3 + 1) * C + c] = b;
    out[((size_t)g * 3 + 2) * C + c] = d;
}

template <int ACT, bool NTL = false>
__global__ void __launch_bounds__(256) bn_act_bwd_apply_kernel(const __bf16 *__restrict__ z, int z_cs, const __bf16 *__restrict__ dy, int dy_cs,
// ... 155 lines not shown
extern "C" {

int ryolo_bn_finalize(double *stat_part, int rows, int cpad, int C, long long count, float eps, float momentum,
                      const float *gamma, const float *beta, float *mean, float *invstd, float *scale, float *shift,
                      float *running_mean, float *running_var, void *stream) {
    if (!stat_part || !gamma || !beta || !mean || !invstd || !scale || !shift || rows <= 0 || C <= 0 || count <= 0)
        return RYOLO_EINVAL;
    hipLaunchKernelGGL(bn_finalize_kernel, dim3((C + 31) / 32), dim3(1024), 0, (hipStream_t)stream, stat_part, rows, cpad, C,
                       (float)count, eps, momentum, gamma, beta, mean, invstd, scale, shift, running_mean, running_var);
    return ok_launch();
}

int ryolo_bn_act_fwd(const void *z, int z_cstride, const float *scale, const float *shift, int act, const float *slope,
                     const void *residual, int res_cstride, void *y, int y_cstride, long long npix, int C, void *stream) {
    if (!z || !scale || !shift || !y || npix <= 0 || C <= 0 || (C & 7) || (z_cstride & 7) || (y_cstride & 7))
        return RYOLO_EINVAL;
    if (act < 0 || act > 2) return RYOLO_EINVAL;
    const bool ntl = nt_pass(0, npix, C);
#define RYOLO_BN_FWD(A)                                                                                                   \
    hipLaunchKernelGGL((ntl ? bn_act_fwd_kernel<A, true> : bn_act_fwd_kernel<A, false>), dim3(grid_for(npix * (C / 8))), dim3(256), 0, (hipStream_t)stream,           \
                       (const __bf16 *)z, z_cstride, scale, shift, slope, (const __bf16 *)residual, res_cstride,          \
                       (__bf16 *)y, y_cstride, npix, C)
    if (act == 0) RYOLO_BN_FWD(0); else if (act == 1) RYOLO_BN_FWD(1); else RYOLO_BN_FWD(2);
#undef RYOLO_BN_FWD
    return ok_launch();
}

size_t ryolo_bn_act_bwd_workspace_bytes(long long npix, int C) {
    const long long nslab = (npix + bwd_slab(npix) - 1) / bwd_slab(npix);
    return (size_t)nslab * 3 * C * 4 + (size_t)3 * C * 4;
}

static int bn_act_bwd_impl(const void *z, int z_cstride, const void *dy, int dy_cstride, const float *scale, const float *shift,
                           const float *mean, const float *invstd, int act, const float *slope, void *dz, int dz_cstride,
                           long long npix, int C, float *dgamma, float *dbeta, float *dslope, void *workspace,
                           size_t workspace_bytes, const float *pre_part, int pre_rows, void *stream_);

int ryolo_bn_act_bwd(const void *z, int z_cstride, const void *dy, int dy_cstride, const float *scale, const float *shift,
                     const float *mean, const float *invstd, int act, const float *slope, void *dz, int dz_cstride,
                     long long npix, int C, float *dgamma, float *dbeta, float *dslope, void *workspace,
                     size_t workspace_bytes, void *stream_) {
    return bn_act_bwd_impl(z, z_cstride, dy, dy_cstride, scale, shift, mean, invstd, act, slope, dz, dz_cstride, npix, C, dgamma, dbeta,
                           dslope, workspace, workspace_bytes, nullptr, 0, stream_);
}

int ryolo_bn_act_bwd_reduced(const void *z, int z_cstride, const void *dy, int dy_cstride, const float *scale, const float *shift,
                             const float *mean, const float *invstd, int act, const float *slope, void *dz, int dz_cstride,
                             long long npix, int C, float *dgamma, float *dbeta, float *dslope, const float *part, int rows,
                             void *workspace, size_t workspace_bytes, void *stream_) {
    if (!part || rows <= 0 || !scale || act != 1) return RYOLO_EINVAL;
    return bn_act_bwd_impl(z, z_cstride, dy, dy_cstride, scale, shift, mean, invstd, act, slope, dz, dz_cstride, npix, C, dgamma, dbeta,
                           dslope, workspace, workspace_bytes, part, rows, stream_);
}

static int bn_act_bwd_impl(const void *z, int z_cstride, const void *dy, int dy_cstride, const float *scale, const float *shift,
                           const float *mean, const float *invstd, int act, const float *slope, void *dz, int dz_cstride,
                           long long npix, int C, float *dgamma, float *dbeta, float *dslope, void *workspace,
                           size_t workspace_bytes, const float *pre_part, int pre_rows, void *stream_) {
    if (!z || !dy || npix <= 0 || C <= 0 || (C & 7) || (z_cstride & 7) || (dy_cstride & 7) || !workspace) return RYOLO_EINVAL;
    if (workspace_bytes < (pre_part ? (size_t)3 * C * 4 : ryolo_bn_act_bwd_workspace_bytes(npix, C))) return RYOLO_EINVAL;
    if (scale && (!shift || !mean || !invstd || !dz || (dz_cstride & 7))) return RYOLO_EINVAL;
    hipStream_t stream = (hipStream_t)stream_;
    int nslab = pre_part ? pre_rows : (int)((npix + bwd_slab(npix) - 1) / bwd_slab(npix));
    float *part = pre_part ? const_cast<float *>(pre_part) : (float *)workspace;
    float *s1 = pre_part ? (float *)workspace : part + (size_t)nslab * 3 * C, *s2 = s1 + C, *s3 = s2 + C;
    if (pre_part && pre_rows >= BWD_FOLD_MIN_ROWS && workspace_bytes >= (size_t)(3 + 3 * BWD_FOLD) * C * 4) {
        float *folded = s3 + C;
        const int per = (pre_rows + BWD_FOLD - 1) / BWD_FOLD;
        hipLaunchKernelGGL(bn_act_bwd_fold_kernel, dim3((C + 31) / 32, BWD_FOLD), dim3(1024), 0, stream, part, pre_rows, C, per, folded);
        part = folded;
        nslab = (pre_rows + per - 1) / per;
    }
    float *dsl = (scale && act == 1) ? dslope : nullptr;
    int CT = 32;
    while (CT > 1 && CT > C / 8) CT >>= 1;
    if (act < 0 || act > 2) return RYOLO_EINVAL;
    const bool nt_red = nt_pass(1, npix, C), nt_app = nt_pass(2, npix, C);
#define RYOLO_BN_REDK(A) (nt_red ? bn_act_bwd_reduce_kernel<A, true> : bn_act_bwd_reduce_kernel<A, false>)
#define RYOLO_BN_RED(A)                                                                                                   \
    hipLaunchKernelGGL(RYOLO_BN_REDK(A), dim3((C / 8 + CT - 1) / CT, nslab), dim3(256), 0, stream,             \
                       (const __bf16 *)z, z_cstride, (const __bf16 *)dy, dy_cstride, scale, shift, mean, invstd, slope,   \
                       npix, C, CT, part, bwd_slab(npix))
    if (pre_part) {  }
    else if (act == 0) RYOLO_BN_RED(0); else if (act == 1) RYOLO_BN_RED(1); else RYOLO_BN_RED(2);
#undef RYOLO_BN_RED
    hipLaunchKernelGGL(bn_act_bwd_finalize_kernel, dim3((C + 31) / 32), dim3(1024), 0, stream, part, nslab, C, s1, s2,
                       scale ? dgamma : nullptr, dbeta, dsl ? s3 : nullptr);
#define RYOLO_BN_APP(A)                                                                                                   \
    hipLaunchKernelGGL((nt_app ? bn_act_bwd_apply_kernel<A, true> : bn_act_bwd_apply_kernel<A, false>), dim3(grid_for(npix * (C / 8), 256, ELEM_BLOCKS)), dim3(256), 0, stream,                  \
                       (const __bf16 *)z, z_cstride, (const __bf16 *)dy, dy_cstride, scale, shift, mean, invstd, s1, s2,  \
                       1.0f / (float)npix, slope, (__bf16 *)dz, dz_cstride, npix, C, s3, dsl)
    if (scale) {
        if (act == 0) RYOLO_BN_APP(0); else if (act == 1) RYOLO_BN_APP(1); else RYOLO_BN_APP(2);
    }
#undef RYOLO_BN_APP
    return ok_launch();
}

#ifdef RYOLO_MP_ABLATION
void ryolo_debug_bn_set(int slabs, int slab_min, int nt_fwd, int nt_red, int nt_app) {
    g_bwd_slabs = slabs; g_bwd_slab_min = slab_min; g_nt[0] = nt_fwd; g_nt[1] = nt_red; g_nt[2] = nt_app;
}
#endif

int ryolo_upsample2x_bwd(const void *dy, int dy_cstride, void *dx, int dx_cstride, int N, int H, int W, int C,
                         int accumulate, void *stream) {
    if (!dy || !dx || N <= 0 || H <= 0 || W <= 0 || C <= 0 || (C & 7) || (dy_cstride & 7) || (dx_cstride & 7))
        return RYOLO_EINVAL;
    hipLaunchKernelGGL(upsample2x_bwd_kernel, dim3(grid_for((long long)N * H * W * (C / 8))), dim3(256), 0,
                       (hipStream_t)stream, (const __bf16 *)dy, dy_cstride, (__bf16 *)dx, dx_cstride, N, H, W, C, accumulate);
    return ok_launch();
}

int ryolo_pgrad_to_nhwc(const float *pgrad, int bs, int na, int ny, int nx, int no, void *out, int out_cstride,
                        void *stream) {
    if (!pgrad || !out || bs <= 0 || na <= 0 || ny <= 0 || nx <= 0 || no <= 0 || out_cstride < na * no) return RYOLO_EINVAL;
    const long long npix = (long long)bs * ny * nx;
    const size_t smem = (size_t)PG_PIX * na * no * 2;
    if ((na * no) % 8 == 0 && (out_cstride & 7) == 0 && (((uintptr_t)out) & 15) == 0 && smem <= 64 * 1024 && npix < 0x7fffffffll) {
        hipLaunchKernelGGL(pgrad_to_nhwc_tiled_kernel, dim3((unsigned)((npix + PG_PIX - 1) / PG_PIX)), dim3(256), smem,
                           (hipStream_t)stream, pgrad, na, ny * nx, no, (__bf16 *)out, out_cstride, (int)npix);
        return ok_launch();
    }
    hipLaunchKernelGGL(pgrad_to_nhwc_kernel, dim3(grid_for((long long)bs * na * ny * nx * no)), dim3(256), 0,
                       (hipStream_t)stream, pgrad, bs, na, ny, nx, no, (__bf16 *)out, out_cstride);
    return ok_launch();
}

}
```

rotate-yolov3_amd/model/hip_train_ops.py:

```python
import ctypes as C

import torch

from .. import _lib
from .hip_ops import ConvDesc, _check_nhwc, cpad

_vp = C.c_void_p
_P = C.POINTER(ConvDesc)
_lib.declare("ryolo_conv_stat_rows", C.c_int, [_P])
_lib.declare("ryolo_conv2d_bn_act_stats", C.c_int, [_P, _vp, _vp, _vp, _vp, _vp, _vp, _vp, _vp])
_lib.declare("ryolo_bn_finalize", C.c_int, [_vp, C.c_int, C.c_int, C.c_int, C.c_longlong, C.c_float, C.c_float, _vp, _vp, _vp,
                                            _vp, _vp, _vp, _vp, _vp, _vp])
_lib.declare("ryolo_bn_act_fwd", C.c_int, [_vp, C.c_int, _vp, _vp, C.c_int, _vp, _vp, C.c_int, _vp, C.c_int, C.c_longlong,
                                           C.c_int, _vp])
_lib.declare("ryolo_bn_act_bwd_workspace_bytes", C.c_size_t, [C.c_longlong, C.c_int])
_lib.declare("ryolo_bn_act_bwd", C.c_int, [_vp, C.c_int, _vp, C.c_int, _vp, _vp, _vp, _vp, C.c_int, _vp, _vp, C.c_int,
                                           C.c_longlong, C.c_int, _vp, _vp, _vp, _vp, C.c_size_t, _vp])
_lib.declare("ryolo_conv_packed_dgrad_bytes", C.c_size_t, [C.c_int, C.c_int, C.c_int, C.c_int])
_lib.declare("ryolo_conv_pack_weights_dgrad", C.c_int, [_vp, C.c_int, C.c_int, C.c_int, C.c_int, _vp, _vp, _vp])
_lib.declare("ryolo_conv_dgrad_tap_table", C.c_int, [C.c_int, C.c_int, _vp])
_lib.declare("ryolo_conv2d_dgrad", C.c_int, [_P, _vp, C.c_int, _vp, _vp, _vp, _vp, C.c_int, _vp])
_lib.declare("ryolo_conv2d_dgrad_bnreduce", C.c_int, [_P, _vp, C.c_int, _vp, _vp, _vp, _vp, C.c_int, _vp, C.c_int, _vp, _vp, _vp, _vp, _vp,
                                                      _vp, _vp])
_lib.declare("ryolo_bn_act_bwd_reduced", C.c_int, [_vp, C.c_int, _vp, C.c_int, _vp, _vp, _vp, _vp, C.c_int, _vp, _vp, C.c_int,
                                                   C.c_longlong, C.c_int, _vp, _vp, _vp, _vp, C.c_int, _vp, C.c_size_t, _vp])
_lib.declare("ryolo_conv_wgrad_workspace_bytes", C.c_size_t, [_P])
_lib.declare("ryolo_conv2d_wgrad", C.c_int, [_P, _vp, _vp, C.c_int, C.c_int, _vp, C.c_int, _vp, C.c_size_t, _vp])
_lib.declare("ryolo_conv2d_wgrad_partials", C.c_int, [_P, _vp, _vp, C.c_int, C.c_int, _vp, C.c_int, _vp, C.c_size_t, _vp])
_lib.declare("ryolo_conv2d_wgrad_reduce", C.c_int, [_P, _vp, _vp, C.c_int, C.c_int, _vp, C.c_int, _vp, C.c_size_t, _vp])
_lib.declare("ryolo_upsample2x_bwd", C.c_int, [_vp, C.c_int, _vp, C.c_int, C.c_int, C.c_int, C.c_int, C.c_int, C.c_int, _vp])
_lib.declare("ryolo_pgrad_to_nhwc", C.c_int, [_vp, C.c_int, C.c_int, C.c_int, C.c_int, C.c_int, _vp, C.c_int, _vp])


_lib.declare("ryolo_yolo_loss_bitmap_bytes", C.c_size_t, [C.c_longlong])
_lib.declare("ryolo_yolo_loss", C.c_int, [_vp, C.c_int, C.c_int, C.c_int, C.c_int, C.c_int, C.c_int, _vp, C.c_int, _vp, _vp, _vp,
                                          _vp, _vp, _vp, _vp, _vp, _vp, C.c_float, C.c_float, C.c_float, C.c_float, C.c_float,
                                          C.c_float, C.c_int, _vp, _vp, _vp, _vp])
_lib.declare("ryolo_yolo_loss_nhwc", C.c_int, [_vp, C.c_int, _vp, C.c_int, C.c_int, C.c_int, C.c_int, C.c_int, C.c_int, _vp, C.c_int, _vp,
                                               _vp, _vp, _vp, _vp, _vp, _vp, _vp, _vp, C.c_float, C.c_float, C.c_float, C.c_float,
                                               C.c_float, C.c_float, C.c_int, _vp, _vp, _vp, C.c_int, _vp, _vp])
_lib.declare("ryolo_scale_bf16_if", C.c_int, [_vp, _vp, C.c_int, C.c_longlong, C.c_int, _vp])
_lib.declare("ryolo_yolo_loss_bitmap_bytes_arc", C.c_size_t, [C.c_longlong, C.c_int, C.c_int])
_lib.declare("ryolo_yolo_loss_arc", C.c_int, [_vp] + [C.c_int] * 6 + [_vp, C.c_int] + [_vp] * 9 + [C.c_float] * 6 +
             [C.c_int, C.c_int, C.c_float] + [_vp] * 4)
_lib.declare("ryolo_yolo_loss_nhwc_arc", C.c_int, [_vp, C.c_int, _vp] + [C.c_int] * 6 + [_vp, C.c_int] + [_vp] * 9 + [C.c_float] * 6 +
             [C.c_int, C.c_int, C.c_float] + [_vp, _vp, _vp, C.c_int, _vp, _vp])
ARC_FOCAL, ARC_UBCE, ARC_UCE = 1, 2, 4


def arc_flags(arc):
    f = ARC_FOCAL if 'F' in arc else 0
    if 'default' in arc:
        return f
    if 'BCE' in arc:
        return f | ARC_UBCE
    if 'CE' in arc:
        return f | ARC_UCE
    raise ValueError("unknown arc %r" % (arc,))
_lib.declare("ryolo_riou_loss_pairs", C.c_int, [_vp, _vp, C.c_int, _vp, _vp, _vp])


class PackJob(C.Structure):
    _fields_ = [("src", C.c_void_p), ("dst", C.c_void_p), ("kind", C.c_int), ("Cout", C.c_int), ("Cin", C.c_int),
                ("KS", C.c_int), ("Cin_pad", C.c_int), ("ntaps", C.c_int), ("Kpad", C.c_int), ("rows", C.c_int),
                ("khs", C.c_int * 9), ("kws", C.c_int * 9), ("block_begin", C.c_int), ("block_end", C.c_int)]


_lib.declare("ryolo_conv_pack_job_fill", C.c_int, [C.POINTER(PackJob), _vp, C.c_int, C.c_int, C.c_int, C.c_int, C.c_int, _vp, _vp])
_lib.declare("ryolo_conv_pack_batch", C.c_int, [_vp, C.c_int, C.c_int, _vp])


class WgradReduceJob(C.Structure):
    _fields_ = [("part", C.c_void_p), ("g", C.c_void_p), ("S", C.c_int), ("Cout", C.c_int), ("Cin_real", C.c_int), ("Cin_k", C.c_int),
                ("ks", C.c_int), ("Kpad", C.c_int), ("Cout_pad", C.c_int), ("accumulate", C.c_int), ("kind", C.c_int),
                ("block_begin", C.c_int), ("block_end", C.c_int), ("wide", C.c_int)]


_lib.declare("ryolo_conv_wgrad_reduce_job_fill", C.c_int, [C.POINTER(WgradReduceJob), _P, C.c_int, _vp, _vp, C.c_int])
_lib.declare("ryolo_conv_wgrad_reduce_batch", C.c_int, [_vp, C.c_int, C.c_int, _vp])


class WgradReduceBatch(object):

    def __init__(self, device):
        self.device = device
        self.jobs = []
        self.keep = []

    def add(self, d, cin_real, ws, grad, accumulate):
        j = WgradReduceJob()
        n = _lib.lib().ryolo_conv_wgrad_reduce_job_fill(C.byref(j), C.byref(d), cin_real, ws.data_ptr(), grad.data_ptr(), 1 if accumulate else 0)
        if n <= 0:
            raise RuntimeError("ryolo_conv_wgrad_reduce_job_fill failed")
        self.jobs.append(j)
        self.keep.append((ws, grad))

    def finalize(self):
        arr = (WgradReduceJob * len(self.jobs))()
        blk = 0
        for q, j in enumerate(self.jobs):
            nb = j.block_end
            j.block_begin, j.block_end = blk, blk + nb
            blk += nb
            arr[q] = j
# ... 54 lines not shown

def stat_rows():
    d = ConvDesc(1, 8, 8, 8, 8, 1, 1, 0, 8, 8, 0, 0, 0.0, 1, 0)
    rows = _lib.lib().ryolo_conv_stat_rows(C.byref(d))
    if rows <= 0:
        raise RuntimeError("ryolo_conv_stat_rows failed")
    return rows


def conv_fwd_stats(d, x, packed_w, ones, shift, z, part=None, clear=True):
    L = _lib.lib()
    rows = L.ryolo_conv_stat_rows(C.byref(d))
    cp = cpad(d.Cout)
    if part is None:
        part = torch.zeros((rows, 2, cp), dtype=torch.float64, device=x.device)
    else:
        part = part.view(-1)[:rows * 2 * cp].view(rows, 2, cp)
        if clear:
            part.zero_()
    if z is not None:
        d.out_cstride = _check_nhwc(z, "z")
    _lib.check(L.ryolo_conv2d_bn_act_stats(C.byref(d), x.data_ptr(), packed_w.data_ptr(), ones.data_ptr(), shift.data_ptr(),
                                           None, z.data_ptr() if z is not None else None, part.data_ptr(), _s(x.device)),
               "ryolo_conv2d_bn_act_stats")
    return part


_lib.declare("ryolo_conv0_bn_act_fwd", C.c_int, [C.POINTER(ConvDesc), _vp, _vp, _vp, _vp, C.c_int, _vp, _vp, _vp])
_lib.declare("ryolo_conv0_bn_bwd_workspace_bytes", C.c_size_t, [])
_lib.declare("ryolo_conv0_bn_bwd", C.c_int, [C.POINTER(ConvDesc), _vp, _vp, _vp, C.c_int, _vp, _vp, _vp, _vp, C.c_int, _vp, _vp, C.c_int,
                                             _vp, _vp, _vp, _vp, C.c_size_t, C.c_int, _vp])


def conv0_recompute_supported(d):
    return bool(_lib.lib().ryolo_conv0_recompute_supported(C.byref(d)))


def conv0_bn_act_fwd(d, x, packed_w, scale, shift, act, slope, y):
    d.out_cstride = _check_nhwc(y, "y")
    _lib.check(_lib.lib().ryolo_conv0_bn_act_fwd(C.byref(d), x.data_ptr(), packed_w.data_ptr(), scale.data_ptr(), shift.data_ptr(), act,
                                                 slope.data_ptr() if slope is not None else None, y.data_ptr(), _s(x.device)),
               "ryolo_conv0_bn_act_fwd")
    return y


def conv0_bn_bwd_ws(device):
    return torch.zeros(_lib.lib().ryolo_conv0_bn_bwd_workspace_bytes(), dtype=torch.uint8, device=device)


def conv0_bn_bwd(d, x, packed_w, dy, stats, act, slope, dz, dgamma, dbeta, dslope, ws, ws_is_zero=True):
    mean, invstd, scale, shift = stats
    _lib.check(_lib.lib().ryolo_conv0_bn_bwd(C.byref(d), x.data_ptr(), packed_w.data_ptr(), dy.data_ptr(), dy.stride(2),
                                             scale.data_ptr(), shift.data_ptr(), mean.data_ptr(), invstd.data_ptr(), act,
                                             slope.data_ptr() if slope is not None else None, dz.data_ptr(), dz.stride(2),
                                             dgamma.data_ptr(), dbeta.data_ptr(), dslope.data_ptr() if dslope is not None else None,
                                             ws.data_ptr(), ws.numel(), 1 if ws_is_zero else 0, _s(x.device)), "ryolo_conv0_bn_bwd")
    return dz


_lib.declare("ryolo_conv0_bn_bwd_wgrad_workspace_bytes", C.c_size_t, [])
_lib.declare("ryolo_conv0_bn_bwd_wgrad", C.c_int, [C.POINTER(ConvDesc), _vp, _vp, _vp, C.c_int, _vp, _vp, _vp, _vp, C.c_int, _vp, _vp, _vp, _vp,
                                                  _vp, C.c_int, C.c_int, _vp, C.c_size_t, _vp])


def conv0_bn_bwd_wgrad_ws(device):
    return torch.empty(_lib.lib().ryolo_conv0_bn_bwd_wgrad_workspace_bytes(), dtype=torch.uint8, device=device)


def conv0_bn_bwd_wgrad(d, x, packed_w, dy, stats, act, slope, dgamma, dbeta, dslope, grad_w, cin_real, accumulate, ws):
    mean, invstd, scale, shift = stats
    _lib.check(_lib.lib().ryolo_conv0_bn_bwd_wgrad(C.byref(d), x.data_ptr(), packed_w.data_ptr(), dy.data_ptr(), dy.stride(2),
                                                   scale.data_ptr(), shift.data_ptr(), mean.data_ptr(), invstd.data_ptr(), act,
                                                   slope.data_ptr() if slope is not None else None, dgamma.data_ptr(), dbeta.data_ptr(),
                                                   dslope.data_ptr() if dslope is not None else None, grad_w.data_ptr(), int(cin_real),
                                                   1 if accumulate else 0, ws.data_ptr(), ws.numel(), _s(x.device)), "ryolo_conv0_bn_bwd_wgrad")


def conv_fwd_plain(d, x, packed_w, ones, shift, z):
    d.out_cstride = _check_nhwc(z, "z")
    _lib.check(_lib.lib().ryolo_conv2d_bn_act(C.byref(d), x.data_ptr(), packed_w.data_ptr(), ones.data_ptr(), shift.data_ptr(),
                                              None, z.data_ptr(), _s(x.device)), "ryolo_conv2d_bn_act")


def bn_finalize(part, C_, count, gamma, beta, eps=1e-5, momentum=0.1, running_mean=None, running_var=None, out=None):
    dev = part.device
    if out is None:
        out = [torch.empty(C_, dtype=torch.float32, device=dev) for _ in range(4)]
    _lib.check(_lib.lib().ryolo_bn_finalize(part.data_ptr(), part.shape[0], part.shape[2], C_, int(count), eps, momentum,
                                            gamma.data_ptr(), beta.data_ptr(), out[0].data_ptr(), out[1].data_ptr(),
                                            out[2].data_ptr(), out[3].data_ptr(),
                                            running_mean.data_ptr() if running_mean is not None else None,
                                            running_var.data_ptr() if running_var is not None else None, _s(dev)),
               "ryolo_bn_finalize")
    return out


def bn_act_fwd(z, scale, shift, act, slope, y, residual=None):
    n, h, w, c = z.shape
    _lib.check(_lib.lib().ryolo_bn_act_fwd(z.data_ptr(), z.stride(2), scale.data_ptr(), shift.data_ptr(), act,
                                           slope.data_ptr() if slope is not None else None,
                                           residual.data_ptr() if residual is not None else None,
                                           residual.stride(2) if residual is not None else 0, y.data_ptr(), y.stride(2),
                                           n * h * w, c, _s(z.device)), "ryolo_bn_act_fwd")
    return y


def bn_act_bwd(z, dy, stats, act, slope, dz, dgamma, dbeta, dslope, ws):
    n, h, w, c = z.shape
    mean, invstd, scale, shift = stats if stats is not None else (None, None, None, None)
    p = lambda t: t.data_ptr() if t is not None else None
    _lib.check(_lib.lib().ryolo_bn_act_bwd(z.data_ptr(), z.stride(2), dy.data_ptr(), dy.stride(2), p(scale), p(shift), p(mean),
                                           p(invstd), act, p(slope), p(dz), dz.stride(2) if dz is not None else 0,
                                           n * h * w, c, p(dgamma), p(dbeta), p(dslope), ws.data_ptr(), ws.numel(),
                                           _s(z.device)), "ryolo_bn_act_bwd")


def bn_bwd_ws_bytes(npix, c):
    return _lib.lib().ryolo_bn_act_bwd_workspace_bytes(npix, c)


_tap_tables = {}


def dgrad_tap_table(ksize, stride, device):
    key = (ksize, stride, device.index)
    t = _tap_tables.get(key)
    if t is None:
        host = (C.c_int * 72)()
        _lib.check(_lib.lib().ryolo_conv_dgrad_tap_table(ksize, stride, host), "ryolo_conv_dgrad_tap_table")
        t = torch.tensor(list(host), dtype=torch.int32, device=device)
        _tap_tables[key] = t
    return t


def pack_weights_dgrad(weight, stride, out=None):
    cout, cin, k, _ = weight.shape
    L = _lib.lib()
    nbytes = L.ryolo_conv_packed_dgrad_bytes(cout, cin, k, stride)
    if out is None:
        out = torch.empty(nbytes, dtype=torch.uint8, device=weight.device)
    w = weight.contiguous()
    table = dgrad_tap_table(k, stride, weight.device)
    _lib.check(L.ryolo_conv_pack_weights_dgrad(w.data_ptr(), cout, cin, k, stride, out.data_ptr(), table.data_ptr(),
                                               _s(weight.device)), "ryolo_conv_pack_weights_dgrad")
    return out


def conv_dgrad(d, dz, packed_dgrad, ones, zeros, dx, accumulate):
    _lib.check(_lib.lib().ryolo_conv2d_dgrad(C.byref(d), dz.data_ptr(), dz.stride(2), packed_dgrad.data_ptr(), ones.data_ptr(),
                                             zeros.data_ptr(), dx.data_ptr(), 1 if accumulate else 0, _s(dz.device)),
               "ryolo_conv2d_dgrad")


def dgrad_bnreduce_rows(d):
    return _lib.lib().ryolo_conv2d_dgrad_bnreduce_rows(C.byref(d))


def conv_dgrad_bnreduce(d, dz, packed_dgrad, ones, zeros, dx, accumulate, z, stats, slope, part):
    mean, invstd, scale, shift = stats
    _lib.check(_lib.lib().ryolo_conv2d_dgrad_bnreduce(C.byref(d), dz.data_ptr(), dz.stride(2), packed_dgrad.data_ptr(), ones.data_ptr(),
                                                      zeros.data_ptr(), dx.data_ptr(), 1 if accumulate else 0, z.data_ptr(), z.stride(2),
                                                      scale.data_ptr(), shift.data_ptr(), mean.data_ptr(), invstd.data_ptr(),
                                                      slope.data_ptr(), part.data_ptr(), _s(dz.device)), "ryolo_conv2d_dgrad_bnreduce")


def bn_act_bwd_reduced(z, dy, stats, act, slope, dz, dgamma, dbeta, dslope, part, ws):
    n, h, w, c = z.shape
    mean, invstd, scale, shift = stats
    p = lambda t: t.data_ptr() if t is not None else None
    _lib.check(_lib.lib().ryolo_bn_act_bwd_reduced(z.data_ptr(), z.stride(2), dy.data_ptr(), dy.stride(2), scale.data_ptr(), shift.data_ptr(),
                                                   mean.data_ptr(), invstd.data_ptr(), act, p(slope), dz.data_ptr(), dz.stride(2), n * h * w, c,
                                                   p(dgamma), p(dbeta), p(dslope), part.data_ptr(), part.shape[0], ws.data_ptr(), ws.numel(),
                                                   _s(z.device)), "ryolo_bn_act_bwd_reduced")


def wgrad_ws_bytes(d):
    return _lib.lib().ryolo_conv_wgrad_workspace_bytes(C.byref(d))


def conv_wgrad(d, x, dz, cin_real, grad, accumulate, ws):
    L = _lib.lib()
    args = (C.byref(d), x.data_ptr(), dz.data_ptr(), dz.stride(2), cin_real, grad.data_ptr(), 1 if accumulate else 0, ws.data_ptr(),
            ws.numel(), _s(x.device))
    if isinstance(L, _lib._CallTracer):
        _lib.check(L.ryolo_conv2d_wgrad_partials(*args), "ryolo_conv2d_wgrad_partials")
        _lib.check(L.ryolo_conv2d_wgrad_reduce(*args), "ryolo_conv2d_wgrad_reduce")
        return
    _lib.check(L.ryolo_conv2d_wgrad(*args), "ryolo_conv2d_wgrad")


def conv_wgrad_partials(d, x, dz, cin_real, grad, accumulate, ws):
    _lib.check(_lib.lib().ryolo_conv2d_wgrad_partials(C.byref(d), x.data_ptr(), dz.data_ptr(), dz.stride(2), cin_real, grad.data_ptr(),
                                                      1 if accumulate else 0, ws.data_ptr(), ws.numel(), _s(x.device)),
               "ryolo_conv2d_wgrad_partials")


def upsample2x_bwd(dy, dx, accumulate):
    n, h, w, c = dx.shape
    _lib.check(_lib.lib().ryolo_upsample2x_bwd(dy.data_ptr(), dy.stride(2), dx.data_ptr(), dx.stride(2), n, h, w, c,
                                               1 if accumulate else 0, _s(dy.device)), "ryolo_upsample2x_bwd")


def pgrad_to_nhwc(pgrad, out):
    bs, na, ny, nx, no = pgrad.shape
    g = pgrad.contiguous()
    _lib.check(_lib.lib().ryolo_pgrad_to_nhwc(g.data_ptr(), bs, na, ny, nx, no, out.data_ptr(), out.stride(2), _s(g.device)),
               "ryolo_pgrad_to_nhwc")


def yolo_loss_bitmap(p, nc=1, arc=0):
    cells = p.numel() // p.shape[-1]
    return torch.zeros(_lib.lib().ryolo_yolo_loss_bitmap_bytes_arc(cells, nc, arc) // 4, dtype=torch.int32, device=p.device)


def yolo_loss_head(p, hd, nc, h, bitmap, dp, items, arc=0):
    bs, na, ny, nx, no = p.shape
    w = hd['w'].contiguous()
    n = hd['npos'] if 'npos' in hd else w.sum()
    c = lambda t: t.contiguous()
    b, gj, gi, cls = c(hd['b']), c(hd['gj']), c(hd['gi']), c(hd['cls'])
    txy, twh, ta, av = c(hd['gxy']), c(hd['gwh']), c(hd['ga']), c(hd['av'].float())
    _lib.check(_lib.lib().ryolo_yolo_loss_arc(p.data_ptr(), bs, na, ny, nx, no, nc, w.data_ptr(), w.shape[1], b.data_ptr(),
                                              gj.data_ptr(), gi.data_ptr(), cls.data_ptr(), txy.data_ptr(), twh.data_ptr(),
                                              ta.data_ptr(), av.data_ptr(), n.data_ptr(), float(h['giou']), float(h['reg']),
                                              float(h['cls']), float(h['cls_pw']), float(h['obj']), float(h['obj_pw']),
                                              1 if h.get('riou', 0) else 0, int(arc), float(h.get('fl_gamma', 0.0)),
                                              bitmap.data_ptr(), dp.data_ptr(), items.data_ptr(), _s(p.device)),
               "ryolo_yolo_loss_arc")


def yolo_loss_head_nhwc(head, p, hd, nc, h, bitmap, dp_sparse, head_g, items, arc=0):
    bs, na, ny, nx, no = p.shape
    w = hd['w'].contiguous()
    n = hd['npos'] if 'npos' in hd else w.sum()
# ... 75 lines not shown
```

rotate-yolov3_amd/model/plan.py:

```python
import ctypes as C
from collections import namedtuple

from .. import _lib
from .._lib import ACT_LINEAR, ConvDesc

View = namedtuple('View', 'buf off C H W cs')
EvalPlan = namedtuple('EvalPlan', 'shapes buffers x views ops')
TrainPlan = namedtuple('TrainPlan', 'shapes buffers x act grd forward blocks backward')


class Refused(RuntimeError):
    """the configuration is refused at plan time (as opposed to a bug in the planner)"""


def _abs(i, l):
    return l if l > 0 else i + l


def _sources(i, d):
    return [_abs(i, int(v)) for v in d['layers'].split(',')]


def _new(buffers, c, h, w):
    buffers.append((c, h, w))
# ... 115 lines not shown
        return home[i] if i in home else _new(buffers, *shp[i])

    ops = []
    pending = None
    pending_head = None
    for i, d in enumerate(defs):
        t = d['type']
        if i in fused_into:
            views[i] = views[fused_into[i]]
            continue
        if t == 'convolutional':
            cv = convs[i]
            if cv.get('refuse'):
                raise Refused(cv['refuse'])
            xin = x if i == 0 else views[i - 1]
            cin_k = convs[pending['layer']]['cout'] if pending is not None else xin.C
            res = views[conv_res[i]] if i in conv_res else None
            ups = 2 if i in conv_ups else 1
            final = i + 1 if (i in conv_res or i in conv_ups) else i
            if cv['cout'] % 8 or cin_k % 8:
                raise Refused("conv %d: channel counts must be multiples of 8 for the HIP path" % i)
            if pending is not None:
                first, pending = pending, None
                fc = convs[first['layer']]
                views[i] = out = view_for(final)
                ops.append(dict(kind='pair', layer=i, first=first['layer'], xin=first['xin'], out=out, shortcut=res is not None,
                                descs=pair_descs(N, first['xin'], fc, cv, out.cs),
                                name='conv_stem_pair<k%ds%d+k%ds%d%s>' % (fc['k'], fc['s'], cv['k'], cv['s'], '+res' if res is not None else '')))
                continue
            alone = readers[i] == [i + 1] and i not in home and res is None and ups == 1
            if (head_decode and alone and not cv['bn'] and cv['act'] == ACT_LINEAR and cv['k'] == 1 and cv['s'] == 1 and
                    defs[i + 1]['type'] == 'yolo'):
                na, no = yolos[i + 1]
                ht = (N, xin.H, xin.W, xin.C, cv['cout'], 1, 1, 0, xin.cs, cv['cout'], 0, ACT_LINEAR, 0.0, 1, 0)
                if _query('ryolo_conv_head_decode_supported', ht, int(na), int(no)):
                    pending_head = dict(kind='head', conv=i, xin=xin, desc=ht, na=na, no=no, name='conv_pw<k1,K%d>+decode' % xin.C)
                    continue
            if (stem_pair and alone and i not in conv_res and defs[i + 1]['type'] == 'convolutional' and (i + 1) not in conv_ups
                    and convs[i + 1]['bn']):
                nx = convs[i + 1]
                if nx.get('refuse'):
                    raise Refused(nx['refuse'])
                if (i + 1) not in conv_res or views[conv_res[i + 1]] == xin:
                    a, b = pair_descs(N, xin, cv, nx)
                    if _query('ryolo_conv_pair_supported', a, b, 1 if (i + 1) in conv_res else 0):
                        pending = dict(layer=i, xin=xin)
                        continue
            views[i] = out = view_for(final)
            desc = (N, xin.H, xin.W, xin.C, cv['cout'], cv['k'], cv['s'], cv['pad'], xin.cs, out.cs, res.cs if res is not None else 0,
                    cv['act'], cv['slope'], ups, 0)
            ops.append(dict(kind='conv', layer=i, xin=xin, out=out, res=res, res_layer=conv_res.get(i), ups=ups, desc=desc))
        elif t == 'shortcut':
            views[i] = view_for(i)
            ops.append(dict(kind='add', layer=i, a=views[i - 1], b=views[_abs(i, int(d['from']))], out=views[i]))
        elif t == 'upsample':
            views[i] = view_for(i)
            ops.append(dict(kind='upsample', layer=i, xin=views[i - 1], out=views[i], stride=int(d['stride'])))
        elif t == 'maxpool':
            views[i] = view_for(i)
            ops.append(dict(kind='maxpool', layer=i, xin=views[i - 1], out=views[i], size=int(d['size']), stride=int(d['stride'])))
        elif t == 'se':
            c = shp[i][0]
            if c % 8 or c < 16 or c > 2048:
                raise Refused("se %d: %d channels (the HIP path serves multiples of 8 from 16 to 2048)" % (i, c))
            views[i] = view_for(i)
            ops.append(dict(kind='se', layer=i, xin=views[i - 1], out=views[i], C=c))
        elif t == 'route':
            if i in alias:
                views[i] = views[alias[i]]
            for src, off in copies.get(i, ()):
                ops.append(dict(kind='copy', layer=i, xin=views[src], out=_slice(views[i], off, shp[src][0])))
        elif t == 'yolo':
            if pending_head is not None:
                ops.append(dict(pending_head, layer=i))
                pending_head = None
            else:
                views[i] = views[i - 1]
                ops.append(dict(kind='decode', layer=i, xin=views[i]))
        elif t == 'reorg3d':
            views[i] = views[i - 1]
    return EvalPlan(shp, buffers, x, views, ops)


def plan_train(defs, convs, N, H, W, conv0_recompute=True, conv0_one_pass=True, cin=3):
    n = len(defs)
    shp = _shapes(defs, convs, cin, H, W)
    for i, d in enumerate(defs):
        if d['type'] == 'upsample' and int(d['stride']) != 2:
            raise Refused("training path: only x2 upsampling")
        if d['type'] == 'se':
            raise Refused("training path: se layers have no HIP training kernels (use model.backend = 'torch')")
        if d['type'] == 'maxpool':
            raise Refused("training path: maxpool graphs (yolov3-tiny) cannot train in the reference either "
                          "(model/loss.py:248 hard-codes three heads)")
    readers = _readers(defs)
    fused_into, conv_res = {}, {}
    for i, d in enumerate(defs):
        if d['type'] == 'shortcut' and i > 0 and defs[i - 1]['type'] == 'convolutional' and readers[i - 1] == [i] \
                and _abs(i, int(d['from'])) != i - 1 and convs[i - 1]['bn']:
            fused_into[i] = i - 1
            conv_res[i - 1] = _abs(i, int(d['from']))

    buffers = []
    x = _new(buffers, 8, H, W)

    def new_pair(c, h, w):
        return _new(buffers, c, h, w), _new(buffers, c, h, w)

    act, grd = [None] * n, [None] * n
    alias, concat = _routes(defs, shp)
    home = {}
    children = {}
    for i, srcs in concat.items():
        act[i], grd[i] = new_pair(*shp[i])
        for src, off in srcs:
            if src in home or defs[src]['type'] not in ('convolutional', 'shortcut', 'upsample') or shp[src][0] % 8 or off % 8:
                raise Refused("training path: route %d needs a copy (unsupported graph)" % i)
            home[src] = (_slice(act[i], off, shp[src][0]), _slice(grd[i], off, shp[src][0]))
            children.setdefault(grd[i], []).append(home[src][1])

    def pair_for(i):
        return home[i] if i in home else new_pair(*shp[i])

    forward, blocks = [], []
    for i, d in enumerate(defs):
        t = d['type']
        if i in fused_into:
            act[i], grd[i] = act[fused_into[i]], grd[fused_into[i]]
            continue
        if t == 'convolutional':
            cv = convs[i]
            if cv.get('refuse'):
                raise Refused(cv['refuse'])
            xin, xin_g = (x, None) if i == 0 else (act[i - 1], grd[i - 1])
            final = i + 1 if i in conv_res else i
            y, dy = pair_for(final)
            res_alias = False
            if i in conv_res and final not in home:
                rg = grd[conv_res[i]]
                if rg is not None and rg[2:5] == dy[2:5] and rg.cs == rg.C:
                    dy, res_alias = rg, True
            act[i], grd[i] = y, dy
            c, h, w = shp[i]
            desc = (N, xin.H, xin.W, xin.C, c, cv['k'], cv['s'], cv['pad'], xin.cs, c, 0, 0, 0.0, 1, 0)
            recompute = bool(i == 0 and cv['bn'] and i not in conv_res and conv0_recompute
                             and _query('ryolo_conv0_recompute_supported', desc))
            blk = dict(layer=i, desc=desc, xin=xin, xin_g=xin_g, y=y, dy=dy, res=act[conv_res[i]] if i in conv_res else None,
                       res_g=grd[conv_res[i]] if i in conv_res else None, res_alias=res_alias, bn=cv['bn'], act=cv['act'], shape=shp[i],
                       recompute=recompute, one_pass=bool(recompute and xin_g is None and conv0_one_pass))
            blocks.append(blk)
            forward.append(('conv', i, blk))
        elif t == 'shortcut':
            a, b = i - 1, _abs(i, int(d['from']))
            act[i], grd[i] = pair_for(i)
            forward.append(('add', i, (act[a], act[b], act[i], grd[a], grd[b], grd[i])))
        elif t == 'upsample':
            act[i], grd[i] = pair_for(i)
            forward.append(('up', i, (act[i - 1], act[i], grd[i - 1], grd[i])))
        elif t == 'route':
            if i in alias:
                act[i], grd[i] = act[alias[i]], grd[alias[i]]
        elif t == 'yolo':
            act[i], grd[i] = act[i - 1], grd[i - 1]
            forward.append(('yolo', i, (act[i], grd[i])))

    init = set()

    def first(g):
        if g in init:
            return False
        init.add(g)
        init.update(children.get(g, ()))
        return True

    heads = [i for kind, i, _ in forward if kind == 'yolo']
    backward = []
    for kind, i, pl in reversed(forward):
        if kind == 'yolo':
            first(pl[1])
            backward.append((kind, i, heads.index(i)))
        elif kind == 'conv':
            res_first = first(pl['res_g']) if (pl['res_g'] is not None and not pl['res_alias']) else None
            backward.append((kind, i, (res_first, first(pl['xin_g']) if pl['xin_g'] is not None else None)))
        elif kind == 'add':
            backward.append((kind, i, (first(pl[3]), first(pl[4]))))
        elif kind == 'up':
            backward.append((kind, i, first(pl[2])))
    return TrainPlan(shp, buffers, x, act, grd, forward, blocks, backward)


def reduce_fusion_pairs(tp):
    by = {b['layer']: b for b in tp.blocks}
    pairs = []
    for (k0, i0, _), (k1, i1, _) in zip(tp.backward[:-1], tp.backward[1:]):
        if k0 != 'conv' or k1 != 'conv':
            continue
        x, y = by[i0], by[i1]
        g, dy = x['xin_g'], y['dy']
        if g is None or not y['bn'] or y['recompute'] or g != dy or dy[2:5] != y['shape'] or g.cs != g.C:
            continue
        rows = _query('ryolo_conv2d_dgrad_bnreduce_rows', x['desc'])
        if rows > 0:
            pairs.append((x, y, rows))
    return pairs
```

rotate-yolov3_amd/model/train_engine.py:

```python
import ctypes as C
import os

import torch
import torch.nn as nn

from .. import _lib
from . import hip_ops as ops
from . import hip_train_ops as tr
from . import plan
from .engine import HipEngine


class _Fn(torch.autograd.Function):
    @staticmethod
    def forward(ctx, engine, x, anchor):
        ctx.engine = engine
        outs = engine.forward(x)
        return tuple(outs)

    @staticmethod
    def backward(ctx, *grads):
        ctx.engine.backward(grads)
        return None, None, None


class TrainEngine(object):
    def __init__(self, model, x_shape, device, use_graph=True):
        _lib.lib()
        self.model = model
        self.no_graph_env = os.environ.get('RYOLO_NO_GRAPH', '0') == '1'
        self.use_graph = use_graph and not self.no_graph_env
        self.graph_fallback = None
        self.reduce_fallback = None
        self.force_eager = False
        self.g_fwd = self.g_bwd = None
        self._segs = None
        self._red_planned = False
        self.nbt = None
        self.packs = None
        self.steps = 0
        self.device = device
        self.bs, cin, self.H, self.W = [int(v) for v in x_shape]
        defs, mods = model.module_defs, model.module_list
        self.defs, self.mods = defs, mods

        convs = {i: self._conv_attrs(mods[i]) for i, d in enumerate(defs) if d['type'] == 'convolutional'}
        tp = self._tplan = plan.plan_train(defs, convs, self.bs, self.H, self.W,
                                           conv0_recompute=os.environ.get('RYOLO_CONV0_RECOMPUTE', '1') != '0',
                                           conv0_one_pass=os.environ.get('RYOLO_CONV0_ONE_PASS', '1') != '0', cin=cin)
        self.shp = tp.shapes

        def new_buf(c, h, w):
            return torch.empty((self.bs, h, w, c), dtype=torch.bfloat16, device=device)

        bufs = [new_buf(*b) for b in tp.buffers]
        tensors = {None: None}

        def tv(v):
            if v not in tensors:
                tensors[v] = bufs[v.buf][..., v.off:v.off + v.C]
            return tensors[v]

        self.x_nhwc = tv(tp.x)
        cmax = max(ops.cpad(max(c.out_channels, c.in_channels)) for c in (HipEngine._conv_of(mods[i]) for i in convs))
        self.ones = torch.ones(cmax, device=device)
        self.zeros = torch.zeros(cmax, device=device)
        self.stat_part = torch.zeros((tr.stat_rows(), 2, cmax), dtype=torch.float64, device=device)
        self.blocks = []
        self.p, self.p_src = [], []
        self.static_grad = {}
        self.direct = False
        self.static_flat = None
        wgrad_ws, bn_ws = 0, 0
        self.plan = fwd = []
        for kind, i, rec in tp.forward:
            if kind == 'conv':
                conv = HipEngine._conv_of(mods[i])
                bn = HipEngine._bn_of(mods[i])
                actmod = [s_ for s_ in mods[i] if isinstance(s_, (nn.PReLU, nn.LeakyReLU))]
                xin, y, dy = tv(rec['xin']), tv(rec['y']), tv(rec['dy'])
                c, h, w = rec['shape']
                desc = ops.ConvDesc(*rec['desc'])
                if bn is not None:
                    z = None if rec['recompute'] else new_buf(c, h, w)
                    dz = None if rec['one_pass'] else new_buf(c, h, w)
                else:
                    z, dz = y, dy
                blk = dict(i=i, conv=conv, bn=bn, act=actmod[-1] if actmod else None, mish=any(type(s_).__name__ == 'Mish' for s_ in mods[i]),
                           xin=xin, xin_g=tv(rec['xin_g']), z=z, dz=dz, y=y, dy=dy, desc=desc, res=tv(rec['res']), res_g=tv(rec['res_g']),
                           res_alias=rec['res_alias'], cin_k=xin.shape[-1], k=desc.ksize, s=desc.stride, pad=desc.pad,
                           npix=self.bs * h * w, C=c, recompute=rec['recompute'])
                wgrad_ws = max(wgrad_ws, tr.wgrad_ws_bytes(desc))
                bn_ws = max(bn_ws, tr.bn_bwd_ws_bytes(blk['npix'], c))
                self.blocks.append(blk)
                fwd.append(('conv', i, blk))
            elif kind in ('add', 'up'):
                fwd.append((kind, i, tuple(tv(v) for v in rec)))
            elif kind == 'yolo':
                m = mods[i]
                c, h, w = tp.shapes[i]
                anchors = m.anchors.to(device=device, dtype=torch.float32).contiguous()
                pbuf = torch.empty((self.bs, m.na, h, w, model.nc + 6), dtype=torch.float32, device=device)
                io = None
                if model.nc + 6 > 96 or m.na * (model.nc + 6) > 1024:
                    io = torch.empty((self.bs, m.na * h * w, model.nc + 6), dtype=torch.float32, device=device)
                self.p.append(pbuf)
                fwd.append(('yolo', i, (tv(rec[0]), tv(rec[1]), m, anchors, pbuf, io, h, w)))
        self.head_pairs = [(pl[0], pl[1]) for kind, _, pl in fwd if kind == 'yolo']
        self.fused_nhwc = False
        self.head_g_ready = False
        self.batch_reduce = os.environ.get('RYOLO_WGRAD_BATCH_REDUCE', '1') != '0'
        self._wr_batches = {}
        self._ws_w_bytes = max(wgrad_ws, 256)
        self._ws_w = None
        self.ws_b = torch.empty(max(bn_ws, 256), dtype=torch.uint8, device=device)

        self.bplan = [(kind, i, pl, flags) for (kind, i, pl), (_, _, flags) in zip(reversed(fwd), tp.backward)]

    @staticmethod
    def _conv_attrs(m):
        conv = HipEngine._conv_of(m)
        other = [type(s_).__name__ for s_ in m if not isinstance(s_, (nn.Conv2d, nn.BatchNorm2d, nn.PReLU, nn.LeakyReLU))
                 and type(s_).__name__ != 'Mish']
        return dict(cout=conv.out_channels, k=conv.kernel_size[0], s=conv.stride[0], pad=conv.padding[0],
                    bn=HipEngine._bn_of(m) is not None, act=None,
                    refuse="activation %s has no HIP training kernels (use model.backend = 'torch')" % other[0] if other else None)

    def _build_grad_sink(self):
        plist = [q for q in self.model.parameters()]
        views = getattr(self.model, '_dp_grad_views', None)
        ok = views is not None and os.environ.get("RYOLO_DIRECT_GRADS", "1") != "0"
        if ok:
            for q in plist:
                v = views.get(q)
                if (v is None or v.dtype != torch.float32 or not v.is_contiguous() or v.device != q.device or v.shape != q.shape
                        or q.grad is None or q.grad.data_ptr() != v.data_ptr()):
                    ok = False
                    break
        self.direct = bool(ok)
        if ok:
            self.static_flat = None
            self.static_grad = {q: views[q] for q in plist}
        else:
            self.static_flat = torch.zeros(sum(q.numel() for q in plist), dtype=torch.float32, device=self.device)
            off = 0
            for q in plist:
                self.static_grad[q] = self.static_flat[off:off + q.numel()].view_as(q)
                off += q.numel()

    def _reset_grad_sink(self):
        self.static_grad, self.static_flat, self.direct = {}, None, False
        self._segs, self.g_bwd = None, None
        self._wr_batches = {}

    def _check_direct_sink(self):
        if not self.direct:
            return
        rebound = 0
        for q, v in self.static_grad.items():
            g = q.grad
            if g is None:
                v.zero_()
            elif g.data_ptr() != v.data_ptr():
                v.copy_(g)
            else:
                continue
            q.grad = v
            rebound += 1
        if rebound and not getattr(self, '_warned_rebind', False):
            self._warned_rebind = True
            import warnings
            warnings.warn("TrainEngine: %d param.grad tensors had been replaced (zero_grad(set_to_none=True)?) while a GradientAllReducer "
                          "owns them; they were re-bound to the reducer's buckets.  Use reducer.zero_grad() to clear gradients." % rebound)

    def _grad_of(self, p):
        g = self.static_grad.get(p)
        if g is None:
            self._build_grad_sink()
            g = self.static_grad[p]
        return g

    def _flush_param_grads(self, params=None):
        add_to, add_from = [], []
        plist = list(self.static_grad.keys()) if params is None else params
        if not self.direct:
            views = getattr(self.model, '_dp_grad_views', None) or {}
            for p in plist:
                g = self.static_grad[p]
                v = views.get(p)
                if v is not None and (p.grad is None or p.grad.data_ptr() != v.data_ptr()):
# ... 86 lines not shown
            n, c, h, w = x.shape
            _lib.check(_lib.lib().ryolo_nchw_f32_to_nhwc_bf16(x.data_ptr(), n, c, h, w, 8, self.x_nhwc.data_ptr(), _lib.stream_ptr(dev)),
                       "ryolo_nchw_f32_to_nhwc_bf16")
            if not self.use_graph or self.steps < 2 or self.force_eager:
                self._forward_launch()
            else:
                if self.g_fwd is None:
                    self.g_fwd = self._capture(self._forward_launch)
                if self.g_fwd is not None:
                    self.g_fwd.replay()
        return [p for p in self.p]

    def _capture(self, launch):
        dev = self.device
        torch.cuda.synchronize(dev)
        g = torch.cuda.CUDAGraph()
        try:
            with torch.cuda.graph(g, capture_error_mode="thread_local"):
                launch()
            return g
        except Exception as e:
            self.use_graph = False
            self.graph_fallback = "%s: %s" % (type(e).__name__, str(e).splitlines()[0][:200] if str(e) else "")
            import warnings
            warnings.warn("TrainEngine: hipGraph capture failed (%s); continuing with eager launches" % self.graph_fallback)
            try:
                torch.cuda.synchronize(dev)
            except Exception:
                pass
            launch()
            return None

    def _forward_launch(self):
        dev = self.device
        L = _lib.lib()
        if self.nbt is None:
            self.nbt = [pl['bn'].num_batches_tracked for kind, i, pl in self.plan if kind == 'conv' and pl['bn'] is not None]
        if self.nbt:
            torch._foreach_add_(self.nbt, 1)
        if self.packs is None:
            self.packs = tr.WeightPackBatch(dev)
            for kind, i, pl in self.plan:
                if kind != 'conv':
                    continue
                w = pl['conv'].weight
                if w.dtype != torch.float32 or not w.is_contiguous():
                    raise RuntimeError("TrainEngine expects contiguous fp32 conv weights")
                cout, cin, k, _ = w.shape
                pl['packed'] = torch.empty(L.ryolo_conv_packed_weight_bytes(cout, pl['cin_k'], k), dtype=torch.uint8, device=dev)
                pl['packed_d'] = torch.empty(L.ryolo_conv_packed_dgrad_bytes(cout, cin, k, pl['s']), dtype=torch.uint8,
                                             device=dev) if pl['xin_g'] is not None else None
                self.packs.add(w.detach(), pl['s'], pl['cin_k'], pl['packed'], pl['packed_d'])
            self.packs.finalize()
        self.packs.run()
        for kind, i, pl in self.plan:
            if kind == 'conv':
                b = pl
                conv, bn = b['conv'], b['bn']
                if bn is not None:
                    part = tr.conv_fwd_stats(b['desc'], b['xin'], b['packed'], self.ones, self.zeros, b['z'], part=self.stat_part,
                                             clear=False)
                    b['stats'] = tr.bn_finalize(part, b['C'], b['npix'], bn.weight.detach(), bn.bias.detach(), eps=bn.eps,
                                                momentum=bn.momentum, running_mean=bn.running_mean,
                                                running_var=bn.running_var, out=b.get('stats'))
                    slope = b['act'].weight.detach() if isinstance(b['act'], nn.PReLU) else None
                    if isinstance(b['act'], nn.LeakyReLU):
                        if 'leaky' not in b:
                            b['leaky'] = torch.full((1,), b['act'].negative_slope, device=dev)
                        slope = b['leaky']
                    b['slope'] = slope
                    b['actcode'] = 2 if b['mish'] else (1 if slope is not None else 0)
                    if b['recompute']:
                        tr.conv0_bn_act_fwd(b['desc'], b['xin'], b['packed'], b['stats'][2], b['stats'][3], b['actcode'], slope, b['y'])
                    else:
                        tr.bn_act_fwd(b['z'], b['stats'][2], b['stats'][3], b['actcode'], slope, b['y'], residual=b['res'])
                else:
                    if conv.bias is not None:
                        if 'bias_pad' not in b:
                            b['bias_pad'] = torch.zeros(ops.cpad(b['C']), device=dev)
                        b['bias_pad'][:b['C']].copy_(conv.bias.detach())
                        bias = b['bias_pad']
                    else:
                        bias = self.zeros
                    tr.conv_fwd_plain(b['desc'], b['xin'], b['packed'], self.ones, bias, b['z'])
                    b['stats'] = None
            elif kind == 'add':
                a, bb, y = pl[0], pl[1], pl[2]
                nn_, hh, ww, cc = y.shape
                _lib.check(L.ryolo_add_nhwc(a.data_ptr(), a.stride(2), bb.data_ptr(), bb.stride(2), y.data_ptr(), y.stride(2),
                                            nn_ * hh * ww, cc, _lib.stream_ptr(dev)), "ryolo_add_nhwc")
            elif kind == 'up':
                xin, y = pl[0], pl[1]
                nn_, hh, ww, cc = xin.shape
                _lib.check(L.ryolo_upsample_nhwc(xin.data_ptr(), xin.stride(2), y.data_ptr(), y.stride(2), nn_, hh, ww, cc, 2,
                                                 _lib.stream_ptr(dev)), "ryolo_upsample_nhwc")
            elif kind == 'yolo':
                head, _, m, anchors, pbuf, io, hh, ww = pl
                stride = float(max(self.H, self.W)) / float(max(hh, ww))
                _lib.check(L.ryolo_yolo_decode(head.data_ptr(), head.stride(2), self.bs, hh, ww, m.na, self.model.nc + 6,
                                               anchors.data_ptr(), stride, 1.0, 0, io.data_ptr() if io is not None else None, m.na * hh * ww, 0,
                                               pbuf.data_ptr(), _lib.stream_ptr(dev)), "ryolo_yolo_decode")
                if (m.nx, m.ny) != (ww, hh):
                    from .models import create_grids
                    create_grids(m, (self.H, self.W), (ww, hh), dev)

    def backward(self, pgrads):
        dev = self.device
        with torch.cuda.device(dev), torch.no_grad():
            if not hasattr(self, "static_pg"):
                self.static_pg = [torch.zeros_like(p) for p in self.p]
            ready = self.head_g_ready
            self.head_g_ready = False
            for k, (buf, g) in enumerate(zip(self.static_pg, pgrads)):
                if g is not None and ready and g.data_ptr() == buf.data_ptr():
                    continue
                if g is None:
                    buf.zero_()
                elif g.data_ptr() != buf.data_ptr():
                    buf.copy_(g)
                tr.pgrad_to_nhwc(buf, self.head_pairs[k][1])
                if self.fused_nhwc and g is not None:
                    buf.zero_()
            self._check_direct_sink()
            self._grad_of(next(self.model.parameters()))
            segs = self._segments()
            if self.batch_reduce:
                self._ensure_reduce_batches(segs)
            if self.g_bwd is None:
                self.g_bwd = [None] * len(segs)
            for k, (lo, hi, params) in enumerate(segs):
                if not self.use_graph or self.steps < 2 or self.force_eager:
                    self._backward_launch(lo, hi)
                else:
                    if self.g_bwd[k] is None:
                        self.g_bwd[k] = self._capture(lambda lo=lo, hi=hi: self._backward_launch(lo, hi))
                    if self.g_bwd[k] is not None:
                        self.g_bwd[k].replay()
                self._flush_param_grads(params)
            self.steps += 1

    def _backward_launch(self, lo=0, hi=None):
        dev = self.device
        L = _lib.lib()
        pgrads = self.static_pg
        if lo == 0 and self.static_flat is not None:
            self.static_flat.zero_()
        if not self._red_planned:
            self._plan_reduce_fusion()
        hook = getattr(self, 'backward_hook', None)

        def entry(kind, i, pl, flags):
            if kind == 'yolo':
                pass
            elif kind == 'conv':
                b = pl
                conv, bn = b['conv'], b['bn']
                res_first, in_first = flags
                dy = b['dy']
                if b['res_g'] is not None and not b['res_alias']:
                    self._passthrough(dy, b['res_g'], res_first)
                if bn is not None:
                    dsl = self._grad_of(b['act'].weight) if isinstance(b['act'], nn.PReLU) else None
                    if b['recompute'] and b['xin_g'] is None and b['dz'] is None:
                        if 'ws0f' not in b:
                            b['ws0f'] = tr.conv0_bn_bwd_wgrad_ws(dev)
                        tr.conv0_bn_bwd_wgrad(b['desc'], b['xin'], b['packed'], dy, b['stats'], b['actcode'], b['slope'],
                                              self._grad_of(bn.weight), self._grad_of(bn.bias), dsl, self._grad_of(conv.weight),
                                              conv.in_channels, True, b['ws0f'])
                        return
                    elif b['recompute']:
                        if 'ws0' not in b:
                            b['ws0'] = tr.conv0_bn_bwd_ws(dev)
                        tr.conv0_bn_bwd(b['desc'], b['xin'], b['packed'], dy, b['stats'], b['actcode'], b['slope'], b['dz'],
                                        self._grad_of(bn.weight), self._grad_of(bn.bias), dsl, b['ws0'])
                    elif b.get('red_part') is not None:
                        tr.bn_act_bwd_reduced(b['z'], dy, b['stats'], 1, b['slope'], b['dz'],
                                              self._grad_of(bn.weight), self._grad_of(bn.bias), dsl, b['red_part'], self.ws_b)
                    else:
                        tr.bn_act_bwd(b['z'], dy, b['stats'], b['actcode'], b['slope'], b['dz'],
                                      self._grad_of(bn.weight), self._grad_of(bn.bias), dsl, self.ws_b)
                elif conv.bias is not None:
                    tr.bn_act_bwd(b['z'], dy, None, 0, None, None, None, self._grad_of(conv.bias), None, self.ws_b)
                if self.batch_reduce:
                    tr.conv_wgrad_partials(b['desc'], b['xin'], b['dz'], conv.in_channels, self._grad_of(conv.weight), True, b['ws_w'])
                else:
                    tr.conv_wgrad(b['desc'], b['xin'], b['dz'], conv.in_channels, self._grad_of(conv.weight), True, self.ws_w)
                if b['xin_g'] is not None:
                    y = b.get('red_for')
                    if y is not None:
                        tr.conv_dgrad_bnreduce(b['desc'], b['dz'], b['packed_d'], self.ones, self.zeros, b['xin_g'], not in_first,
                                               y['z'], y['stats'], y['slope'], y['red_part'])
                    else:
                        tr.conv_dgrad(b['desc'], b['dz'], b['packed_d'], self.ones, self.zeros, b['xin_g'], not in_first)
            elif kind == 'add':
                dyv = pl[5]
                self._passthrough(dyv, pl[3], flags[0])
                self._passthrough(dyv, pl[4], flags[1])
            elif kind == 'up':
                tr.upsample2x_bwd(pl[3], pl[2], not flags)

        for kind, i, pl, flags in self.bplan[lo:hi]:
            if hook is not None:
                hook('pre', kind, i, pl, flags)
            entry(kind, i, pl, flags)
            if hook is not None:
                hook('post', kind, i, pl, flags)
        if self.batch_reduce:
            wb = self._wr_batches[(lo, len(self.bplan) if hi is None else hi)]
            if wb is not None:
                wb.run()

    def _plan_reduce_fusion(self):
        self._red_planned = True
        if os.environ.get("RYOLO_BN_REDUCE_FUSION", "1") == "0":
            return
        blk = {b['i']: b for b in self.blocks}
        pairs = []
        for xr, yr, rows in plan.reduce_fusion_pairs(self._tplan):
            x, y = blk[xr['layer']], blk[yr['layer']]
            if y.get('actcode') == 1 and y.get('slope') is not None and y.get('stats') is not None:
                pairs.append((x, y, rows, x['xin_g'].shape[3]))
        if not pairs:
            return
        part = torch.empty(max(rows * 3 * c for _, _, rows, c in pairs), dtype=torch.float32, device=self.device)
        for x, y, rows, c in pairs:
            x['red_for'] = y
            y['red_part'] = part[:rows * 3 * c].view(rows, 3, c)

    def _passthrough(self, src, dst, is_first):
        L = _lib.lib()
        n, h, w, c = dst.shape
        if is_first:
            _lib.check(L.ryolo_upsample_nhwc(src.data_ptr(), src.stride(2), dst.data_ptr(), dst.stride(2), n, h, w, c, 1,
                                             _lib.stream_ptr(self.device)), "ryolo_upsample_nhwc")
        else:
            _lib.check(L.ryolo_add_nhwc(src.data_ptr(), src.stride(2), dst.data_ptr(), dst.stride(2), dst.data_ptr(),
                                        dst.stride(2), n * h * w, c, _lib.stream_ptr(self.device)), "ryolo_add_nhwc")

    def __call__(self, x):
        anchor = next(self.model.parameters())
        return list(_Fn.apply(self, x, anchor))
```

Baseline: 1349 images/s.

## Fuse YOLO head conv with raw-prediction write and pad head channels for dgrad

Adds a training-mode head kernel (new pointwise mode 5) that writes both the bf16 conv output and the fp32 per-anchor prediction buffer in one pass, so the separate yolo_decode launch and its re-read of the head tensor are skipped when fused. Head conv outputs are also allocated with a channel stride rounded up to 64 and zero-filled, so the head's 1x1 dgrad can take the fast path with K a multiple of BK. The cost is extra zeroed padding memory and extra template instantiations, and it relies on the padded lanes of dy staying zero.

```diff
diff --git a/include/ryolo.h b/include/ryolo.h
--- a/include/ryolo.h
+++ b/include/ryolo.h
@@ -103,6 +103,10 @@
 int ryolo_conv_head_decode(const ryolo_conv_desc *desc, const void *x, const void *w_packed, const float *scale, const float *shift,
                            const float *anchors, int na, int no, float stride, float context_factor, int arc, float *io,
                            long long io_rows_per_image, long long io_row_offset, float *p, void *stream);
+
+int ryolo_conv_head_train_supported(const ryolo_conv_desc *desc, int na, int no);
+int ryolo_conv_head_train(const ryolo_conv_desc *desc, const void *x, const void *w_packed, const float *scale, const float *shift,
+                          int na, int no, void *y, float *p, void *stream);
 
 int ryolo_add_nhwc(const void *a, int a_cstride, const void *b, int b_cstride, void *y, int y_cstride,
                    long long npix, int C, void *stream);
@@ -153,6 +157,9 @@
                                   void *stream);
 int ryolo_conv2d_dgrad(const ryolo_conv_desc *forward_desc, const void *dz, int dz_cstride, const void *packed_dgrad,
                        const float *ones, const float *zeros , void *dx, int accumulate, void *stream);
+int ryolo_conv2d_dgrad_zpad(const ryolo_conv_desc *forward_desc, const void *dz, int dz_cstride, const void *packed_dgrad,
+                            const float *ones, const float *zeros, void *dx, int accumulate, void *stream);
+int ryolo_conv_dgrad_zpad_kernel_choice(const ryolo_conv_desc *forward_desc);
 int ryolo_conv2d_dgrad_bnreduce_rows(const ryolo_conv_desc *forward_desc);
 int ryolo_conv2d_dgrad_bnreduce(const ryolo_conv_desc *forward_desc, const void *dz, int dz_cstride, const void *packed_dgrad,
                                 const float *ones, const float *zeros, void *dx, int accumulate,
diff --git a/rotate-yolov3_amd/_lib.py b/rotate-yolov3_amd/_lib.py
--- a/rotate-yolov3_amd/_lib.py
+++ b/rotate-yolov3_amd/_lib.py
@@ -36,6 +36,7 @@
     "ryolo_eval_match": (C.c_int, [_vp, C.c_int, _vp, _vp, C.c_int, _vp, C.c_int, C.c_int, C.c_int, C.c_float, _vp, _vp, _vp, C.c_size_t, _vp]),
     "ryolo_conv_pair_supported": (C.c_int, [_dp, _dp, C.c_int]),
     "ryolo_conv_head_decode_supported": (C.c_int, [_dp, C.c_int, C.c_int]),
+    "ryolo_conv_head_train_supported": (C.c_int, [_dp, C.c_int, C.c_int]),
     "ryolo_conv0_recompute_supported": (C.c_int, [_dp]),
     "ryolo_conv2d_dgrad_bnreduce_rows": (C.c_int, [_dp]),
     "ryolo_se_workspace_bytes": (C.c_size_t, [C.c_int, C.c_int, C.c_int, C.c_int]),
diff --git a/rotate-yolov3_amd/csrc/conv.hip b/rotate-yolov3_amd/csrc/conv.hip
--- a/rotate-yolov3_amd/csrc/conv.hip
+++ b/rotate-yolov3_amd/csrc/conv.hip
@@ -1581,6 +1581,21 @@
     if (((uintptr_t)x | (uintptr_t)w_packed) & 15) return RYOLO_EINVAL;
     p.x = (const __bf16 *)x; p.w = (const __bf16 *)w_packed; p.scale = scale; p.shift = shift;
     return launch_conv_pw_decode(p, io, io_rows_per_image, io_row_offset, pout, anchors, na, no, stride, context_factor, arc, (hipStream_t)stream_);
+}
+
+int ryolo_conv_head_train_supported(const ryolo_conv_desc *d, int na, int no) {
+    ConvParams p{};
+    return head_params(d, p) && d->act == RYOLO_ACT_LINEAR && conv_pw_decode_supported(p, na, no, true) ? 1 : 0;
+}
+
+int ryolo_conv_head_train(const ryolo_conv_desc *d, const void *x, const void *w_packed, const float *scale, const float *shift, int na, int no,
+                          void *y, float *pout, void *stream_) {
+    ConvParams p{};
+    if (!x || !w_packed || !scale || !shift || !y || !pout || !ryolo_conv_head_train_supported(d, na, no) || !head_params(d, p)) return RYOLO_EINVAL;
+    if (((uintptr_t)x | (uintptr_t)w_packed | (uintptr_t)y | (uintptr_t)pout) & 15) return RYOLO_EINVAL;
+    if (!buffer_extent(p.M, d->out_cstride, d->Cout)) return RYOLO_EINVAL;
+    p.x = (const __bf16 *)x; p.w = (const __bf16 *)w_packed; p.scale = scale; p.shift = shift;
+    return launch_conv_pw_decode(p, nullptr, 0, 0, pout, nullptr, na, no, 1.f, 1.f, 0, (hipStream_t)stream_, (__bf16 *)y, d->out_cstride);
 }
 
 int ryolo_conv_pair_supported(const ryolo_conv_desc *first, const ryolo_conv_desc *second, int shortcut_from_input) {
diff --git a/rotate-yolov3_amd/csrc/conv_common.h b/rotate-yolov3_amd/csrc/conv_common.h
--- a/rotate-yolov3_amd/csrc/conv_common.h
+++ b/rotate-yolov3_amd/csrc/conv_common.h
@@ -241,9 +241,9 @@
 bool conv_pw_preferred(const ConvParams &p);
 int conv_pw_grid(const ConvParams &p);
 int launch_conv_pw(ConvParams &p, const ConvLaunch &lc);
-bool conv_pw_decode_supported(const ConvParams &p, int na, int no);
+bool conv_pw_decode_supported(const ConvParams &p, int na, int no, bool with_y = false);
 int launch_conv_pw_decode(ConvParams &p, float *io, long long io_img_rows, long long io_row0, float *pout, const float *anchors, int na, int no,
-                          float stride, float cf, int arc, hipStream_t stream);
+                          float stride, float cf, int arc, hipStream_t stream, __bf16 *y = nullptr, int y_cs = 0);
 #ifdef RYOLO_MP_ABLATION
 int ryolo_mp_ablation_variant(int slot);
 #endif
diff --git a/rotate-yolov3_amd/csrc/conv_dgrad.hip b/rotate-yolov3_amd/csrc/conv_dgrad.hip
--- a/rotate-yolov3_amd/csrc/conv_dgrad.hip
+++ b/rotate-yolov3_amd/csrc/conv_dgrad.hip
@@ -352,12 +352,14 @@
 }
 
 static int conv_dgrad(const ryolo_conv_desc *d , const void *dz, int dz_cstride, const void *packed_dgrad, const float *ones,
-                      const float *zeros, void *dx, int accumulate, const ConvLaunch &lc) {
+                      const float *zeros, void *dx, int accumulate, const ConvLaunch &lc, int dz_pad_zero = 0) {
     if (conv_validate(d) != RYOLO_OK) return RYOLO_EINVAL;
     if (d->stride != 1 && !(d->stride == 2 && d->ksize == 3 && d->pad == 1)) return RYOLO_EINVAL;
     if ((dz_cstride & 7) || dz_cstride < d->Cout) return RYOLO_EINVAL;
     const int Ho = (d->H + 2 * d->pad - d->ksize) / d->stride + 1, Wo = (d->W + 2 * d->pad - d->ksize) / d->stride + 1;
     const int rows = (d->Cin + 127) / 128 * 128;
+    const int cout64 = (d->Cout + BK - 1) / BK * BK;
+    const int kch = (dz_pad_zero && d->ksize == 1 && d->stride == 1 && dz_cstride >= cout64) ? cout64 : d->Cout;
     const unsigned long long dz_pix = (unsigned long long)d->N * Ho * Wo;
     const int nt_out = (long long)d->N * d->H * d->W * d->Cin * 2 >= nt_out_min_bytes() ? 1 : 0;
     const char *wsrc = (const char *)packed_dgrad;
@@ -389,12 +391,12 @@
         p.scale = ones; p.shift = zeros;
         p.res = accumulate ? (const __bf16 *)dx : nullptr;
         p.y = (__bf16 *)dx;
-        p.N = d->N; p.H = Ho; p.W = Wo; p.Cin = d->Cout; p.in_cs = dz_cstride;
+        p.N = d->N; p.H = Ho; p.W = Wo; p.Cin = kch; p.in_cs = dz_cstride;
         p.Cout = d->Cin; p.out_cs = d->in_cstride; p.res_cs = d->in_cstride;
-        p.K = nt * d->Cout;
+        p.K = nt * kch;
         p.Kpad = (p.K + BK - 1) / BK * BK;
         p.act = RYOLO_ACT_LINEAR; p.ups = 1;
-        p.cin_log2 = ilog2_exact(d->Cout);
+        p.cin_log2 = ilog2_exact(kch);
         p.ntaps = nt;
         for (int t = 0; t < nt; t++) { p.tap_dy[t] = dy[t]; p.tap_dx[t] = dxx[t]; }
         p.stride = 1; p.OH = d->H;
@@ -415,7 +417,7 @@
         wsrc += wbytes;
         if (p.Ho <= 0 || p.Wo <= 0) continue;
         p.M = (int)((long long)d->N * p.Ho * p.Wo);
-        p.fast = (d->Cout % BK == 0) && buffer_extent(dz_pix, dz_cstride, d->Cout, &p.x_bytes) && buffer_extent(wrows, p.Kpad, p.Kpad + 128, &p.w_bytes);
+        p.fast = (kch % BK == 0) && buffer_extent(dz_pix, dz_cstride, kch, &p.x_bytes) && buffer_extent(wrows, p.Kpad, p.Kpad + 128, &p.w_bytes);
         if (!p.fast) p.x_bytes = p.w_bytes = 0;
         if (!p.fast && (d->stride != 1 || (d->ksize == 3 && p.cin_log2 < 0))) return RYOLO_EINVAL;
         p.no_persist = (d->tile & 0x200) ? 1 : 0;
@@ -428,12 +430,13 @@
     return RYOLO_OK;
 }
 
-static int dgrad_choice(const ryolo_conv_desc *d, const BnRed *bnred = nullptr, int mode = 0) {
+static int dgrad_choice(const ryolo_conv_desc *d, const BnRed *bnred = nullptr, int mode = 0, int dz_pad_zero = 0) {
     int choice = -1;
     ConvLaunch lc;
     lc.bnred = bnred; lc.bnred_mode = mode; lc.choice = &choice;
     void *fake = (void *)(uintptr_t)4096;
-    return conv_dgrad(d, fake, d ? d->Cout : 0, fake, (const float *)fake, (const float *)fake, fake, 1, lc) == RYOLO_OK ? choice : -1;
+    const int cs = !d ? 0 : (dz_pad_zero ? (d->Cout + BK - 1) / BK * BK : d->Cout);
+    return conv_dgrad(d, fake, cs, fake, (const float *)fake, (const float *)fake, fake, 1, lc, dz_pad_zero) == RYOLO_OK ? choice : -1;
 }
 
 static int bnreduce_plan_tiles(const ryolo_conv_desc *d) {
@@ -520,6 +523,17 @@
     return conv_dgrad(d, dz, dz_cstride, packed_dgrad, ones, zeros, dx, accumulate, lc);
 }
 
+int ryolo_conv2d_dgrad_zpad(const ryolo_conv_desc *d , const void *dz, int dz_cstride,
+                            const void *packed_dgrad, const float *ones, const float *zeros, void *dx, int accumulate,
+                            void *stream_) {
+    if (!dz || !packed_dgrad || !ones || !zeros || !dx) return RYOLO_EINVAL;
+    ConvLaunch lc;
+    lc.stream = (hipStream_t)stream_;
+    return conv_dgrad(d, dz, dz_cstride, packed_dgrad, ones, zeros, dx, accumulate, lc, 1);
+}
+
+int ryolo_conv_dgrad_zpad_kernel_choice(const ryolo_conv_desc *d) { return dgrad_choice(d, nullptr, 0, 1); }
+
 int ryolo_conv2d_dgrad_bnreduce(const ryolo_conv_desc *d, const void *dz, int dz_cstride, const void *packed_dgrad, const float *ones,
                                 const float *zeros, void *dx, int accumulate, const void *z, int z_cstride, const float *scale,
                                 const float *shift, const float *mean, const float *invstd, const float *slope, float *part,
diff --git a/rotate-yolov3_amd/csrc/conv_pw.hip b/rotate-yolov3_amd/csrc/conv_pw.hip
--- a/rotate-yolov3_amd/csrc/conv_pw.hip
+++ b/rotate-yolov3_amd/csrc/conv_pw.hip
@@ -66,6 +66,8 @@
     float stride, cf;
     int arc;
     int apb;
+    __bf16 *y;
+    int y_cs;
 };
 
 template <int KT, int NW, int CF, int PF, int RING, int MODE>
@@ -74,7 +76,7 @@
     constexpr int UNIT = BMS * 128;
     constexpr int LPU = (BMS / 8) / NW;
     constexpr int NCB = NW * CF * 16;
-    constexpr bool HAS_RES = MODE == 2 || MODE == 3, BNRED = MODE == 3, STATS = MODE == 1, DEC = MODE == 4;
+    constexpr bool HAS_RES = MODE == 2 || MODE == 3, BNRED = MODE == 3, STATS = MODE == 1, DEC = MODE == 4 || MODE == 5, DECY = MODE == 5;
     constexpr int TROW = NCB * 2 + 16;
     constexpr int NSTG = DEC ? 0 : (CF == 2 ? PF : PF / 2);
     constexpr int NREQ = (HAS_RES ? NSTG : 0) + (BNRED ? NSTG : 0);
@@ -302,6 +304,24 @@
                 const int a0 = nb * dc.apb, na_here = min(dc.apb, dc.na - a0);
                 const int nrows = BMS * na_here;
                 const long long hw = (long long)dc.ny * dc.nx;
+                if constexpr (DECY) {
+                    const int ncol = na_here * dc.no;
+                    if (((n0 | ncol) & 3) == 0) {
+                        const int ppr = ncol >> 2;
+                        for (int i = tid; i < BMS * ppr; i += NW * 64) {
+                            const int pxl = i / ppr, pc = i - pxl * ppr;
+                            if (m0 + pxl < p.M)
+                                *(uint2 *)(dc.y + (long long)(m0 + pxl) * dc.y_cs + n0 + pc * 4) = *(const uint2 *)(tile + pxl * TROW + pc * 8);
+                        }
+                    } else {
+                        const int ppr = ncol >> 1;
+                        for (int i = tid; i < BMS * ppr; i += NW * 64) {
+                            const int pxl = i / ppr, pc = i - pxl * ppr;
+                            if (m0 + pxl < p.M)
+                                *(unsigned *)(dc.y + (long long)(m0 + pxl) * dc.y_cs + n0 + pc * 2) = *(const unsigned *)(tile + pxl * TROW + pc * 4);
+                        }
+                    }
+                }
                 for (int rw = tid; rw < nrows; rw += NW * 64) {
                     const int al = rw / BMS, pxl = rw - al * BMS;
                     const int a = a0 + al;
@@ -318,6 +338,7 @@
                         if (k < dc.no) v[k] = (float)src[k];
                     const long long row = (long long)a * hw + (long long)y * dc.nx + x;
                     if (dc.p) store_row(dc.p + (((long long)n * dc.na * hw) + row) * dc.no, v, dc.no);
+                    if constexpr (DECY) continue;
                     const float aw = dc.anchors[a * 3 + 0] / dc.stride, ah = dc.anchors[a * 3 + 1] / dc.stride, aa = dc.anchors[a * 3 + 2];
                     decode_row<8>(v, dc.no, x, y, aw, ah, aa, dc.stride, dc.cf, dc.arc, dc.io + (((long long)n * dc.io_img_rows) + dc.io_row0 + row) * dc.no);
                 }
@@ -464,7 +485,7 @@
 
 template <int KT, int NW, int CF, int PF, int RING, int MODE>
 int pw_launch(ConvParams &p, const PwBnRed &br, int grid, hipStream_t stream) {
-    constexpr int LDS = RING * PF * 16 * 128 + (MODE == 4 ? PF * 16 * (NW * CF * 16 * 2 + 16) : 0);
+    constexpr int LDS = RING * PF * 16 * 128 + (MODE >= 4 ? PF * 16 * (NW * CF * 16 * 2 + 16) : 0);
     const PwDecode dc = g_pw_decode ? *g_pw_decode : PwDecode{};
     return launch_kernel<conv_pw_kernel<KT, NW, CF, PF, RING, MODE>>(dim3((unsigned)grid), dim3(NW * 64), LDS, stream, p, br, dc);
 }
@@ -472,7 +493,8 @@
 template <int KT, int NW, int CF, int PF, int RING, int MODES>
 int pw_launch_mode(ConvParams &p, const PwBnRed *br, int grid, hipStream_t stream) {
     PwBnRed none{};
-    const int mode = g_pw_decode ? 4 : (br ? 3 : (p.stat_part ? 1 : (p.res ? 2 : 0)));
+    const int mode = g_pw_decode ? (g_pw_decode->y ? 5 : 4) : (br ? 3 : (p.stat_part ? 1 : (p.res ? 2 : 0)));
+    if constexpr ((MODES & 32) != 0) if (mode == 5) return pw_launch<KT, NW, CF, PF, RING, 5>(p, none, grid, stream);
     if constexpr ((MODES & 16) != 0) if (mode == 4) return pw_launch<KT, NW, CF, PF, RING, 4>(p, none, grid, stream);
     if constexpr ((MODES & 8) != 0) if (mode == 3) return pw_launch<KT, NW, CF, PF, RING, 3>(p, *br, grid, stream);
     if constexpr ((MODES & 2) != 0) if (mode == 1) return pw_launch<KT, NW, CF, PF, RING, 1>(p, none, grid, stream);
@@ -552,14 +574,17 @@
 }
 
 int launch_conv_pw_decode(ConvParams &p, float *io, long long io_img_rows, long long io_row0, float *pout, const float *anchors, int na, int no,
-                          float stride, float cf, int arc, hipStream_t stream) {
-    if (!io || !anchors || na <= 0 || no < 7 || no > 8 || na * no != p.Cout || p.ups != 1 || p.res || p.stat_part) return RYOLO_EINVAL;
+                          float stride, float cf, int arc, hipStream_t stream, __bf16 *y, int y_cs) {
+    if (y ? (!pout || io || (y_cs & 7) || y_cs < p.Cout) : (!io || !anchors)) return RYOLO_EINVAL;
+    if (na <= 0 || no < 7 || no > 8 || na * no != p.Cout || p.ups != 1 || p.res || p.stat_part) return RYOLO_EINVAL;
     const long long dmax = p.Wo > p.Ho ? p.Wo : p.Ho;
     if (((long long)p.M + 64) * dmax >= 0x100000000ll) return RYOLO_EINVAL;
     PwDecode dc;
     dc.io = io; dc.p = pout; dc.anchors = anchors; dc.io_img_rows = io_img_rows; dc.io_row0 = io_row0;
     dc.na = na; dc.no = no; dc.ny = p.Ho; dc.nx = p.Wo; dc.stride = stride; dc.cf = cf; dc.arc = arc;
     dc.apb = pw_decode_apb(na, no, p.Cin == 1024 ? 128 : 256);
+    dc.y = y; dc.y_cs = y_cs;
+    if (y && dc.apb < na && ((dc.apb * no) & 1)) return RYOLO_EINVAL;
     g_pw_decode = &dc;
     ConvLaunch lc;
     lc.stream = stream;
@@ -568,11 +593,12 @@
     return rc;
 }
 
-bool conv_pw_decode_supported(const ConvParams &p, int na, int no) {
+bool conv_pw_decode_supported(const ConvParams &p, int na, int no, bool with_y) {
     if (no < 7 || no > 8 || na * no != p.Cout || p.Kpad != p.Cin || (p.Cin != 256 && p.Cin != 512 && p.Cin != 1024)) return false;
     const int ncb = p.Cin == 1024 ? 128 : 256;
     const int apb = pw_decode_apb(na, no, ncb);
     const int nb = apb > 0 ? (na + apb - 1) / apb : 0;
+    if (with_y && nb > 1 && ((apb * no) & 1)) return false;
     if (!(apb > 0 && (nb == 1 || nb == 2 || nb == 4) && (nb - 1) * apb * no + ncb <= ((p.Cout + 127) / 128) * 128)) return false;
     PwDecode dc{};
     dc.na = na; dc.no = no; dc.apb = apb;
@@ -629,12 +655,12 @@
     PW_CASE(4, 4, 2, 8, 4, 3)
     PW_CASE(6, 4, 2, 4, 8, 7)
     PW_CASE(2, 8, 2, 4, 12, 15)
-    PW_CASE(4, 8, 2, 4, 12, 23)
+    PW_CASE(4, 8, 2, 4, 12, 55)
     PW_CASE(4, 8, 1, 4, 12, 8)
-    PW_CASE(8, 8, 2, 4, 12, 23)
+    PW_CASE(8, 8, 2, 4, 12, 55)
     PW_CASE(8, 8, 1, 4, 12, 8)
     PW_CASE(12, 8, 1, 4, 12, 7)
-    PW_CASE(16, 8, 1, 4, 12, 23)
+    PW_CASE(16, 8, 1, 4, 12, 55)
 #undef PW_CASE
     return RYOLO_EINVAL;
 }
diff --git a/rotate-yolov3_amd/csrc/train.hip b/rotate-yolov3_amd/csrc/train.hip
--- a/rotate-yolov3_amd/csrc/train.hip
+++ b/rotate-yolov3_amd/csrc/train.hip
@@ -126,7 +126,7 @@
     return s < BWD_SLAB_MIN ? BWD_SLAB_MIN : s;
 }
 #endif
-template <int ACT, bool NTL = false>
+template <int ACT, bool NTL = false, bool NOZ = false>
 __global__ void __launch_bounds__(256)
 bn_act_bwd_reduce_kernel(const __bf16 *__restrict__ z, int z_cs, const __bf16 *__restrict__ dy, int dy_cs,
                          const float *__restrict__ scale, const float *__restrict__ shift,
@@ -164,7 +164,23 @@
             }
         };
         long long pix = p0 + pl;
-        for (; pix + 3 * npl < p1; pix += 4 * npl) {
+        if constexpr (NOZ) {
+            for (; pix + 7 * npl < p1; pix += 8 * npl) {
+                bf16x8 gv[8];
+#pragma unroll
+                for (int k = 0; k < 8; k++) gv[k] = ld8<NTL>(dy + (pix + k * npl) * dy_cs + c);
+#pragma unroll
+                for (int k = 0; k < 8; k++)
+#pragma unroll
+                    for (int e = 0; e < 8; e++) s1[e] += (float)gv[k][e];
+            }
+            for (; pix < p1; pix += npl) {
+                const bf16x8 gv = *(const bf16x8 *)(dy + pix * dy_cs + c);
+#pragma unroll
+                for (int e = 0; e < 8; e++) s1[e] += (float)gv[e];
+            }
+        }
+        for (; !NOZ && pix + 3 * npl < p1; pix += 4 * npl) {
             bf16x8 zv[4], gv[4];
 #pragma unroll
             for (int k = 0; k < 4; k++) {
@@ -174,7 +190,7 @@
 #pragma unroll
             for (int k = 0; k < 4; k++) accum(zv[k], gv[k]);
         }
-        for (; pix < p1; pix += npl) accum(*(const bf16x8 *)(z + pix * z_cs + c), *(const bf16x8 *)(dy + pix * dy_cs + c));
+        for (; !NOZ && pix < p1; pix += npl) accum(*(const bf16x8 *)(z + pix * z_cs + c), *(const bf16x8 *)(dy + pix * dy_cs + c));
 #pragma unroll
         for (int e = 0; e < 8; e++) s2[e] *= is[e];
     }
@@ -496,6 +512,10 @@
                        (const __bf16 *)z, z_cstride, (const __bf16 *)dy, dy_cstride, scale, shift, mean, invstd, slope,   \
                        npix, C, CT, part, bwd_slab(npix))
     if (pre_part) {  }
+    else if (!scale)
+        hipLaunchKernelGGL((nt_red ? bn_act_bwd_reduce_kernel<0, true, true> : bn_act_bwd_reduce_kernel<0, false, true>),
+                           dim3((C / 8 + CT - 1) / CT, nslab), dim3(256), 0, stream, (const __bf16 *)z, z_cstride, (const __bf16 *)dy, dy_cstride,
+                           scale, shift, mean, invstd, slope, npix, C, CT, part, bwd_slab(npix));
     else if (act == 0) RYOLO_BN_RED(0); else if (act == 1) RYOLO_BN_RED(1); else RYOLO_BN_RED(2);
 #undef RYOLO_BN_RED
     hipLaunchKernelGGL(bn_act_bwd_finalize_kernel, dim3((C + 31) / 32), dim3(1024), 0, stream, part, nslab, C, s1, s2,
diff --git a/rotate-yolov3_amd/model/hip_train_ops.py b/rotate-yolov3_amd/model/hip_train_ops.py
--- a/rotate-yolov3_amd/model/hip_train_ops.py
+++ b/rotate-yolov3_amd/model/hip_train_ops.py
@@ -20,6 +20,9 @@
 _lib.declare("ryolo_conv_pack_weights_dgrad", C.c_int, [_vp, C.c_int, C.c_int, C.c_int, C.c_int, _vp, _vp, _vp])
 _lib.declare("ryolo_conv_dgrad_tap_table", C.c_int, [C.c_int, C.c_int, _vp])
 _lib.declare("ryolo_conv2d_dgrad", C.c_int, [_P, _vp, C.c_int, _vp, _vp, _vp, _vp, C.c_int, _vp])
+_lib.declare("ryolo_conv2d_dgrad_zpad", C.c_int, [_P, _vp, C.c_int, _vp, _vp, _vp, _vp, C.c_int, _vp])
+_lib.declare("ryolo_conv_dgrad_zpad_kernel_choice", C.c_int, [_P])
+_lib.declare("ryolo_conv_head_train", C.c_int, [_P, _vp, _vp, _vp, _vp, C.c_int, C.c_int, _vp, _vp, _vp])
 _lib.declare("ryolo_conv2d_dgrad_bnreduce", C.c_int, [_P, _vp, C.c_int, _vp, _vp, _vp, _vp, C.c_int, _vp, C.c_int, _vp, _vp, _vp, _vp, _vp,
                                                       _vp, _vp])
 _lib.declare("ryolo_bn_act_bwd_reduced", C.c_int, [_vp, C.c_int, _vp, C.c_int, _vp, _vp, _vp, _vp, C.c_int, _vp, _vp, C.c_int,
@@ -240,6 +243,12 @@
                                               None, z.data_ptr(), _s(x.device)), "ryolo_conv2d_bn_act")
 
 
+def conv_head_train(d, x, packed_w, ones, shift, na, no, y, p):
+    d.out_cstride = _check_nhwc(y, "y")
+    _lib.check(_lib.lib().ryolo_conv_head_train(C.byref(d), x.data_ptr(), packed_w.data_ptr(), ones.data_ptr(), shift.data_ptr(),
+                                                int(na), int(no), y.data_ptr(), p.data_ptr(), _s(x.device)), "ryolo_conv_head_train")
+
+
 def bn_finalize(part, C_, count, gamma, beta, eps=1e-5, momentum=0.1, running_mean=None, running_var=None, out=None):
     dev = part.device
     if out is None:
@@ -304,10 +313,10 @@
     return out
 
 
-def conv_dgrad(d, dz, packed_dgrad, ones, zeros, dx, accumulate):
-    _lib.check(_lib.lib().ryolo_conv2d_dgrad(C.byref(d), dz.data_ptr(), dz.stride(2), packed_dgrad.data_ptr(), ones.data_ptr(),
-                                             zeros.data_ptr(), dx.data_ptr(), 1 if accumulate else 0, _s(dz.device)),
-               "ryolo_conv2d_dgrad")
+def conv_dgrad(d, dz, packed_dgrad, ones, zeros, dx, accumulate, zpad=False):
+    name = "ryolo_conv2d_dgrad_zpad" if zpad else "ryolo_conv2d_dgrad"
+    _lib.check(getattr(_lib.lib(), name)(C.byref(d), dz.data_ptr(), dz.stride(2), packed_dgrad.data_ptr(), ones.data_ptr(),
+                                         zeros.data_ptr(), dx.data_ptr(), 1 if accumulate else 0, _s(dz.device)), name)
 
 
 def dgrad_bnreduce_rows(d):
diff --git a/rotate-yolov3_amd/model/plan.py b/rotate-yolov3_amd/model/plan.py
--- a/rotate-yolov3_amd/model/plan.py
+++ b/rotate-yolov3_amd/model/plan.py
@@ -221,7 +221,11 @@
     return EvalPlan(shp, buffers, x, views, ops)
 
 
-def plan_train(defs, convs, N, H, W, conv0_recompute=True, conv0_one_pass=True, cin=3):
+def _head_stride(c):
+    return (c + 63) // 64 * 64
+
+
+def plan_train(defs, convs, N, H, W, conv0_recompute=True, conv0_one_pass=True, cin=3, yolos=None, head_pad=True, head_fuse=True):
     n = len(defs)
     shp = _shapes(defs, convs, cin, H, W)
     for i, d in enumerate(defs):
@@ -261,6 +265,14 @@
     def pair_for(i):
         return home[i] if i in home else new_pair(*shp[i])
 
+    def is_head(i):
+        return (i + 1 < n and defs[i + 1]['type'] == 'yolo' and readers[i] == [i + 1] and i not in home and i not in conv_res
+                and not convs[i]['bn'] and convs[i]['k'] == 1 and convs[i]['s'] == 1)
+
+    def head_pair(c, h, w):
+        cs = _head_stride(c)
+        return tuple(_slice(_new(buffers, cs, h, w), 0, c) for _ in range(2))
+
     forward, blocks = [], []
     for i, d in enumerate(defs):
         t = d['type']
@@ -273,7 +285,8 @@
                 raise Refused(cv['refuse'])
             xin, xin_g = (x, None) if i == 0 else (act[i - 1], grd[i - 1])
             final = i + 1 if i in conv_res else i
-            y, dy = pair_for(final)
+            padded = head_pad and is_head(i) and shp[i][0] % 64 != 0
+            y, dy = head_pair(*shp[i]) if padded else pair_for(final)
             res_alias = False
             if i in conv_res and final not in home:
                 rg = grd[conv_res[i]]
@@ -286,7 +299,11 @@
                              and _query('ryolo_conv0_recompute_supported', desc))
             blk = dict(layer=i, desc=desc, xin=xin, xin_g=xin_g, y=y, dy=dy, res=act[conv_res[i]] if i in conv_res else None,
                        res_g=grd[conv_res[i]] if i in conv_res else None, res_alias=res_alias, bn=cv['bn'], act=cv['act'], shape=shp[i],
-                       recompute=recompute, one_pass=bool(recompute and xin_g is None and conv0_one_pass))
+                       recompute=recompute, one_pass=bool(recompute and xin_g is None and conv0_one_pass), head_padded=padded, head_fused=None)
+            if head_fuse and yolos is not None and is_head(i) and cv['act'] in (None, ACT_LINEAR):
+                na, no = yolos[i + 1]
+                if _query('ryolo_conv_head_train_supported', desc, int(na), int(no)):
+                    blk['head_fused'] = (int(na), int(no))
             blocks.append(blk)
             forward.append(('conv', i, blk))
         elif t == 'shortcut':
diff --git a/rotate-yolov3_amd/model/train_engine.py b/rotate-yolov3_amd/model/train_engine.py
--- a/rotate-yolov3_amd/model/train_engine.py
+++ b/rotate-yolov3_amd/model/train_engine.py
@@ -45,15 +45,22 @@
         self.defs, self.mods = defs, mods
 
         convs = {i: self._conv_attrs(mods[i]) for i, d in enumerate(defs) if d['type'] == 'convolutional'}
+        yolos = {i: (int(mods[i].na), int(model.nc) + 6) for i, d in enumerate(defs) if d['type'] == 'yolo'}
         tp = self._tplan = plan.plan_train(defs, convs, self.bs, self.H, self.W,
                                            conv0_recompute=os.environ.get('RYOLO_CONV0_RECOMPUTE', '1') != '0',
-                                           conv0_one_pass=os.environ.get('RYOLO_CONV0_ONE_PASS', '1') != '0', cin=cin)
+                                           conv0_one_pass=os.environ.get('RYOLO_CONV0_ONE_PASS', '1') != '0', cin=cin, yolos=yolos,
+                                           head_pad=os.environ.get('RYOLO_HEAD_PAD', '1') != '0',
+                                           head_fuse=os.environ.get('RYOLO_HEAD_FUSE', '1') != '0')
         self.shp = tp.shapes
 
         def new_buf(c, h, w):
             return torch.empty((self.bs, h, w, c), dtype=torch.bfloat16, device=device)
 
         bufs = [new_buf(*b) for b in tp.buffers]
+        for b in tp.blocks:
+            if b['head_padded']:
+                bufs[b['y'].buf].zero_()
+                bufs[b['dy'].buf].zero_()
         tensors = {None: None}
 
         def tv(v):
@@ -89,7 +96,7 @@
                 blk = dict(i=i, conv=conv, bn=bn, act=actmod[-1] if actmod else None, mish=any(type(s_).__name__ == 'Mish' for s_ in mods[i]),
                            xin=xin, xin_g=tv(rec['xin_g']), z=z, dz=dz, y=y, dy=dy, desc=desc, res=tv(rec['res']), res_g=tv(rec['res_g']),
                            res_alias=rec['res_alias'], cin_k=xin.shape[-1], k=desc.ksize, s=desc.stride, pad=desc.pad,
-                           npix=self.bs * h * w, C=c, recompute=rec['recompute'])
+                           npix=self.bs * h * w, C=c, recompute=rec['recompute'], zpad=rec['head_padded'], head_fused=rec['head_fused'])
                 wgrad_ws = max(wgrad_ws, tr.wgrad_ws_bytes(desc))
                 bn_ws = max(bn_ws, tr.bn_bwd_ws_bytes(blk['npix'], c))
                 self.blocks.append(blk)
@@ -105,7 +112,11 @@
                 if model.nc + 6 > 96 or m.na * (model.nc + 6) > 1024:
                     io = torch.empty((self.bs, m.na * h * w, model.nc + 6), dtype=torch.float32, device=device)
                 self.p.append(pbuf)
-                fwd.append(('yolo', i, (tv(rec[0]), tv(rec[1]), m, anchors, pbuf, io, h, w)))
+                hb = self.blocks[-1] if self.blocks and self.blocks[-1]['y'] is tv(rec[0]) else None
+                fused = hb is not None and hb['head_fused'] == (int(m.na), model.nc + 6)
+                if fused:
+                    hb['pbuf'] = pbuf
+                fwd.append(('yolo', i, (tv(rec[0]), tv(rec[1]), m, anchors, pbuf, io, h, w, fused)))
         self.head_pairs = [(pl[0], pl[1]) for kind, _, pl in fwd if kind == 'yolo']
         self.fused_nhwc = False
         self.head_g_ready = False
@@ -358,7 +369,11 @@
                         bias = b['bias_pad']
                     else:
                         bias = self.zeros
-                    tr.conv_fwd_plain(b['desc'], b['xin'], b['packed'], self.ones, bias, b['z'])
+                    if b.get('pbuf') is not None:
+                        tr.conv_head_train(b['desc'], b['xin'], b['packed'], self.ones, bias, b['head_fused'][0], b['head_fused'][1], b['z'],
+                                           b['pbuf'])
+                    else:
+                        tr.conv_fwd_plain(b['desc'], b['xin'], b['packed'], self.ones, bias, b['z'])
                     b['stats'] = None
             elif kind == 'add':
                 a, bb, y = pl[0], pl[1], pl[2]
@@ -371,11 +386,12 @@
                 _lib.check(L.ryolo_upsample_nhwc(xin.data_ptr(), xin.stride(2), y.data_ptr(), y.stride(2), nn_, hh, ww, cc, 2,
                                                  _lib.stream_ptr(dev)), "ryolo_upsample_nhwc")
             elif kind == 'yolo':
-                head, _, m, anchors, pbuf, io, hh, ww = pl
+                head, _, m, anchors, pbuf, io, hh, ww, fused = pl
                 stride = float(max(self.H, self.W)) / float(max(hh, ww))
-                _lib.check(L.ryolo_yolo_decode(head.data_ptr(), head.stride(2), self.bs, hh, ww, m.na, self.model.nc + 6,
-                                               anchors.data_ptr(), stride, 1.0, 0, io.data_ptr() if io is not None else None, m.na * hh * ww, 0,
-                                               pbuf.data_ptr(), _lib.stream_ptr(dev)), "ryolo_yolo_decode")
+                if not fused:
+                    _lib.check(L.ryolo_yolo_decode(head.data_ptr(), head.stride(2), self.bs, hh, ww, m.na, self.model.nc + 6,
+                                                   anchors.data_ptr(), stride, 1.0, 0, io.data_ptr() if io is not None else None, m.na * hh * ww, 0,
+                                                   pbuf.data_ptr(), _lib.stream_ptr(dev)), "ryolo_yolo_decode")
                 if (m.nx, m.ny) != (ww, hh):
                     from .models import create_grids
                     create_grids(m, (self.H, self.W), (ww, hh), dev)
@@ -467,7 +483,7 @@
                         tr.conv_dgrad_bnreduce(b['desc'], b['dz'], b['packed_d'], self.ones, self.zeros, b['xin_g'], not in_first,
                                                y['z'], y['stats'], y['slope'], y['red_part'])
                     else:
-                        tr.conv_dgrad(b['desc'], b['dz'], b['packed_d'], self.ones, self.zeros, b['xin_g'], not in_first)
+                        tr.conv_dgrad(b['desc'], b['dz'], b['packed_d'], self.ones, self.zeros, b['xin_g'], not in_first, zpad=b['zpad'])
             elif kind == 'add':
                 dyv = pl[5]
                 self._passthrough(dyv, pl[3], flags[0])
```

Result: no change. 1347 images/s (-0.2%).
